# mobeets/classifying-vae-lstm

Hardware: AMD Instinct MI355X
Metric: piano-roll timesteps/sec (train) (higher is better)
Workload: dtype f32; 1 GPU; cfg3: cl_vrnn batch 256/GPU x seq_len 128, latent 2, 10 classes, 88-dim piano-roll, Adam-WN, hipGraph=True; global_batch=256, seq_len=128, parallelism=dp1

## Files before the change

### classifying-vae-lstm_amd/_lib.py

```python
import ctypes as C
import os

_HERE = os.path.dirname(os.path.abspath(__file__))
LIB_PATH = os.environ.get("CLV_LIB") or os.path.join(_HERE, "libclvae_hip.so")

ABI_VERSION = 600
ACT_NONE, ACT_RELU, ACT_SIGMOID, ACT_MASKPOS = 0, 1, 2, 3
GATE_HARD_SIGMOID, GATE_SIGMOID = 0, 1

_f = C.c_float
_i = C.c_int
_p = C.c_void_p
_sz = C.c_size_t
_i64 = C.c_int64
_u64 = C.c_uint64
_u32 = C.c_uint32
_d = C.c_double


class VaeStepOpts(C.Structure):
    _fields_ = [("draw", _i), ("stream_w", _u32), ("stream_z", _u32), ("step", _u32),
                ("noise_seed", _u64), ("first_w", _u64), ("first_z", _u64),
                ("step_dev", _p), ("loss_means", _p), ("bump_iterations", _p), ("bf16", _i)]



class NoiseDraw(C.Structure):
    _fields_ = [("seed", _u64), ("first", _u64), ("stream", _u32), ("step", _u32), ("step_dev", _p)]


class PairPackSrc(C.Structure):
    _fields_ = [("H", _i), ("L", _i), ("U_enc", _p), ("U_dec", _p), ("Kz", _p), ("Wz", _p), ("pack", _p)]


class AdamKnownSums(C.Structure):
    _fields_ = [("tensor", _i), ("use", _i), ("gdot", _p), ("vnorm2", _p)]


class BatchCursor(C.Structure):
    _fields_ = [("step_dev", _p), ("step0", C.c_int32), ("period", C.c_int32), ("stride", _i64), ("offset", _i64)]


class LabelStage(C.Structure):
    _fields_ = [("cur", _p), ("hist", _p),
                ("cur_stride", _i64), ("cur_offset", _i64), ("hist_stride", _i64), ("hist_offset", _i64), ("row0", _i64),
                ("cur_table", _p), ("hist_table", _p), ("idx", _p),
                ("cursor", BatchCursor),
                ("X", _p), ("Xh", _p), ("hist_chunk", C.c_int32), ("hist_ld", _i64),
                ("w_src", _p), ("w_out", _p), ("X8", _p), ("Xh8", _p)]


class FrameProj(C.Structure):
    _fields_ = [("T", C.c_int32), ("N", C.c_int32), ("ldo", C.c_int32), ("K_cur", _p), ("out_cur", _p), ("K_hist", _p), ("out_hist", _p)]


class WgradProblem(C.Structure):
    _fields_ = [("K", C.c_int32), ("N", C.c_int32),
                ("X", _p), ("ldx", C.c_int32), ("nx", C.c_int32), ("x_exact_bf16", C.c_int32),
                ("H", _p), ("ldh", C.c_int32), ("nh", C.c_int32), ("h_shift", C.c_int32), ("h_zero_period", C.c_int32),
                ("Z", _p), ("ldz", C.c_int32), ("nz", C.c_int32),
                ("dz", _p), ("lddz", C.c_int32),
                ("dKx", _p), ("ld_kx", C.c_int32),
                ("dU", _p), ("ld_u", C.c_int32),
                ("dKz", _p), ("ld_kz", C.c_int32),
                ("beta", C.c_float),
                ("ws", _p), ("ws_bytes", C.c_size_t)]


class ParamDesc(C.Structure):
    _fields_ = [("offset", C.c_int64), ("rows", C.c_int32), ("cols", C.c_int32),
                ("col_offset", C.c_int64), ("is_matrix", C.c_int32), ("pad_", C.c_int32)]


class GemmProb(C.Structure):
    _fields_ = [("A", C.c_void_p), ("lda", C.c_int32), ("M", C.c_int32), ("C", C.c_void_p), ("ldc", C.c_int32),
                ("a_shift", C.c_int32), ("a_zero_period", C.c_int32), ("ones", C.c_int32)]


class ReduceJob(C.Structure):
    _fields_ = [("opaque", C.c_ubyte * 160)]


class SkinnyProduct(C.Structure):
    _fields_ = [("A", C.c_void_p), ("lda", C.c_int), ("rows", C.c_int), ("B", C.c_void_p), ("ldb", C.c_int),
                ("N", C.c_int), ("K", C.c_int), ("C", C.c_void_p), ("ldc", C.c_int), ("bias_row", C.c_void_p)]


class LabelBwdRider(C.Structure):
    _fields_ = [("D", C.c_int), ("C", C.c_int), ("Kenc_w", C.c_void_p), ("Kdec_w", C.c_void_p), ("wargs", C.c_void_p),
                ("eps", C.c_void_p), ("onehot", C.c_void_p), ("W", C.c_void_p), ("hW", C.c_void_p), ("Ka", C.c_void_p),
                ("prior_logvar", C.c_float), ("class_weight", C.c_float), ("w_kl_weight", C.c_float), ("inv_b", C.c_float),
                ("dwargs", C.c_void_p), ("dhW", C.c_void_p), ("dKa", C.c_void_p), ("dba", C.c_void_p),
                ("ws", C.c_void_p), ("ws_bytes", C.c_size_t), ("job", C.c_void_p)]


class ProfRecord(C.Structure):
    _fields_ = [("name", C.c_char * 48), ("launches", C.c_int32), ("total_ms", C.c_float)]


def _args(kind, names):
    return [kind] * len(names.split())


_VRNN_GENERATE = _args(_i, "N S nsteps D H L C gate_act z_prior") + [_u64] + _args(_p, "x_seed w")
_VAE_GENERATE = _args(_i, "N nsteps D H L C use_x_prev z_prior") + [_u64] + _args(_p, "x_seed w")
_VARY = _args(_i, "N T D H L C gate_act|use_x_prev hist_source") + [_u64] + _args(_p, "sources x0 w_enc w_dec")
_DECODE = _args(_i, "N T D H L C gate_act|use_x_prev") + [_u64] + _args(_p, "z_in x0 history w_dec noise_rows")
_VRNN_ENC, _VRNN_DEC = _args(_p, "Kx_enc Kw_enc b_enc U_enc Wz bz"), _args(_p, "Kx_dec Kz Kw_dec b_dec U_dec Wo bo")
_VAE_ENC, _VAE_DEC = _args(_p, "Kh bh Kz bz"), _args(_p, "Kd bd Ko bo")
_TEMPER = [_p, _f, _f]
_OUT, _OUT_Z = _args(_p, "Xs xhat stream"), _args(_p, "Xs xhat zout stream")
_RESUME = [_u32] + _args(_p, "state_in state_out")

SIGNATURES = {
    "clv_version": (_i, []),
    "clv_device_count": (_i, []),
    "clv_error_string": (C.c_char_p, [_i]),
    "clv_gemm_auto_split": (_i, [_i, _i, _i]),
    "clv_gemm_workspace_bytes": (_sz, [_i, _i, _i]),
    "clv_gemm_f32": (_i, [_i, _i, _i, _i, _i, _f, _p, _i, _p, _i, _f, _p, _i, _p, _i, _p, _i, _p, _sz, _p, _p]),
    "clv_gemm_grouped_tn": (_i, [_p, _i, _i, _i, _p, _i, _f, _i, _p, _sz, _p, _p]),
    "clv_splitk_reduce_multi": (_i, [_p, _i, _p, _p, _p, _i, _p, _p, _i, _p]),
    "clv_splitk_reduce_multi_outer_supported": (_i, [_i, _i, _i, _i, _i]),
    "clv_splitk_reduce_multi_outer": (_i, [_p, _i, _p, _p, _p, _i, _p, _p, _i,
                                           _i, _i, _i, _p, _i, _i, _p, _i, _p, _i, _p, _p, _i, _p, _p, _p]),
    "clv_lstm_wgrad_supported": (_i, [_i, _i, _i, _i, _i]),
    "clv_lstm_wgrad_workspace_bytes": (_sz, [_i, _i, _i, _i, _i, _i]),
    "clv_lstm_wgrad_pair_supported": (_i, [_p, _p]),
    "clv_lstm_wgrad_pair_workspace_bytes": (_sz, [_i, _i, _i, _i, _i, _i]),
    "clv_lstm_wgrad_pair": (_i, [_p, _p, _i, _p, _p, _p]),
    "clv_lstm_wgrad": (_i, [_i, _i, _p, _i, _i, _i, _p, _i, _i, _i, _i, _p, _i, _i, _p, _i, _p, _i, _p, _i, _p, _i, _f,
                               _i, _p, _sz, _p, _p]),
    "clv_gemm_grouped_tn_small2": (_i, [_p, _i, _p, _p, _i, _p, _i, _i, _i, _p]),
    "clv_gemm_grouped_auto_split": (_i, [_p, _i, _i, _i]),
    "clv_gemm_grouped_workspace_bytes": (_sz, [_p, _i, _i, _i]),
    "clv_colsum_workspace_bytes": (_sz, [_i, _i]),
    "clv_colsum_f32": (_i, [_i, _i, _p, _i, _f, _p, _p, _sz, _p]),
    "clv_lstm_seq_fwd": (_i, [_i, _i, _i, _i, _p, _p, _p, _p, _p, _p, _p, _p, _p, _p, _p]),
    "clv_lstm_seq_bwd_z": (_i, [_i, _i, _i, _i, _p, _p, _p, _p, _p, _p, _p, _i, _p, _i, _p]),
    "clv_lstm_seq_bwd": (_i, [_i, _i, _i, _i, _p, _p, _p, _p, _p, _p, _p]),
    "clv_lstm_mx_supported": (_i, [_i, _i, _i, _i]),
    "clv_lstm_mx_fwd": (_i, [_i, _i, _i, _i, _p, _i, _i, _i, _p, _p, _i, _i, _p, _p, _p, _p, _p, _p, _p]),
    "clv_lstm_mx_bwd": (_i, [_i, _i, _i, _p, _p, _p, _p, _p, _p, _i, _p, _i, _p]),
    "clv_lstm_pair_supported": (_i, [_i, _i]),
    "clv_lstm_pair_pack_floats": (_sz, []),
    "clv_lstm_pair_pack": (_i, [_i, _i, _p, _p, _p, _p, _p, _p]),
    "clv_lstm_pair_fwd": (_i, [_i, _i, _i, _i, _i, _p, _p, _p, _i, _p, _p, _p, _p, _p, _p, _p, _p, _p, _p, _i, _p, _p, _p, _p, _p,
                               _p, _p]),
    "clv_lstm_pair_bwd": (_i, [_i, _i, _i, _i, _i, _f] + [_p] * 12 + [_p, _p, _p, _p, _sz, _p, _p, _p]),
    "clv_lstm_pair_bwd_workspace_bytes": (_sz, [_i, _i, _i]),
    "clv_sparse_proj_supported": (_i, [_i, _i]),
    "clv_sparse_proj_lds_bytes": (_sz, [_i, _i]),
    "clv_sparse_proj": (_i, [_i, _i, _i, _p, _i, _i, _p, _p, _i, _p]),
    "clv_sparse_proj2": (_i, [_i, _i, _i, _i, _i, _p, _i, _p, _p, _i, _p, _i, _p, _p, _p]),
    "clv_sparse_dense_supported": (_i, [_i]),
    "clv_sparse_dense": (_i, [_i, _i, _i, _p, _i, _p, _p, _i, _p, _i, _p]),
    "clv_sparse_outer": (_i, [_i, _i, _i, _p, _i, _p, _i, _p, _i, _p, _p, _i, _p, _p, _p]),
    "clv_dense_outer_bf16_supported": (_i, [_i, _i, _i, _i, _i]),
    "clv_dense_outer_bf16": (_i, [_i, _i, _i, _p, _i, _i, _p, _i, _p, _i, _p, _p, _i, _p, _p, _p]),
    "clv_gemm_bce_f32": (_i, [_i, _i, _i, _p, _i, _p, _i, _p, _p, _i, _f, _p, _p, _i, _p, _p]),
    "clv_out_head_train_supported": (_i, [_i, _i]),
    "clv_out_head_train_workspace_bytes": (_sz, [_i]),
    "clv_out_head_train": (_i, [_i, _i, _i, _p, _p, _p, _p, _i, _i, _f, _p, _p, _p, _p, _p, _p, _p, _sz, _p, _p]),
    "clv_latent_head_supported": (_i, [_i, _i]),
    "clv_latent_head_bwd_workspace_bytes": (_sz, [_i, _i]),
    "clv_latent_head_fwd": (_i, [_i, _i, _i, _p, _p, _p, _p, _p, _p, _i, _p, _p, _p]),
    "clv_latent_head_bwd": (_i, [_i, _i, _i, _p, _p, _p, _p, _p, _i, _f, _p, _p, _p, _p, _p, _sz, _p, _p]),
    "clv_vrnn_generate_supported": (_i, [_i, _i, _i, _i]),
    "clv_vrnn_generate": (_i, _VRNN_GENERATE + _VRNN_ENC + _VRNN_DEC + _OUT),
    "clv_vae_generate_supported": (_i, [_i, _i, _i, _i]),
    "clv_vae_generate": (_i, _VAE_GENERATE + _VAE_ENC + _VAE_DEC + _OUT),
    "clv_vrnn_generate_clamped": (_i, _VRNN_GENERATE + _VRNN_ENC + _VRNN_DEC + _args(_p, "clamp") + _OUT),
    "clv_vae_generate_clamped": (_i, _VAE_GENERATE + _VAE_ENC + _VAE_DEC + _args(_p, "clamp") + _OUT),
    "clv_vrnn_generate_tempered": (_i, _VRNN_GENERATE + _VRNN_ENC + _VRNN_DEC + _TEMPER + _OUT),
    "clv_vae_generate_tempered": (_i, _VAE_GENERATE + _VAE_ENC + _VAE_DEC + _TEMPER + _OUT),
    "clv_vrnn_vary": (_i, _VARY + _VRNN_ENC + _VRNN_DEC + _TEMPER + _OUT),
    "clv_vae_vary": (_i, _VARY + _VAE_ENC + _VAE_DEC + _TEMPER + _OUT),
    "clv_take_frame": (_i, [_i64, _i, _i, _p, _p, _p, _p]),
    "clv_vrnn_vary_latents": (_i, _VARY + _VRNN_ENC + _VRNN_DEC + _TEMPER + _OUT_Z),
    "clv_vae_vary_latents": (_i, _VARY + _VAE_ENC + _VAE_DEC + _TEMPER + _OUT_Z),
    "clv_vrnn_decode": (_i, _DECODE + _VRNN_DEC + _TEMPER[:2] + _OUT),
    "clv_vae_decode": (_i, _DECODE + _VAE_DEC + _TEMPER[:2] + _OUT),
    "clv_vrnn_generate_resume": (_i, _VRNN_GENERATE + _VRNN_ENC + _VRNN_DEC + _TEMPER + _RESUME + _OUT),
    "clv_vae_generate_resume": (_i, _VAE_GENERATE[:-2] + _args(_p, "w") + _VAE_ENC + _VAE_DEC + _TEMPER + _RESUME + _OUT),
    "clv_lerp_rows": (_i, [_i64, _i64] + [_p] * 7),
    "clv_sigmoid_temper": (_i, [_i64, _p, _f, _p]),
    "clv_scale_temper": (_i, [_i64, _p, _f, _p]),
    "clv_label_fwd": (_i, [_i, _i, _p, _p, _i, _p, _p, _f, _p, _p, _p]),
    "clv_label_bwd": (_i, [_i, _i, _p, _p, _i, _p, _p, _p, _p, _f, _f, _f, _f, _p, _p, _i, _p]),
    "clv_vae_fused_supported": (_i, [_i, _i, _i, _i, _i]),
    "clv_vae_fused_workspace_bytes": (_sz, [_i, _i, _i, _i, _i, _i, _i]),
    "clv_vae_fused_step": (_i, [_i, _i, _i, _i, _i, _i, _i, _p, _p, _p, _p, _p, _p, _p, _p, _p, C.c_long, _f, _f, _f, _f, _i,
                                _p, _p, _sz, _p, _p, _p, _p, _p, _p, _p, _p, _p]),
    "clv_vrnn_label_fwd": (_i, [_i, _i, _i, _i, _p, _p, _p, _p, _p, _f, _p, _p, _p, _p, _p, _p, _p, _p, _p, _p]),
    "clv_vrnn_label_fwd_x": (_i, [_i, _i, _i, _i, _p, _i, _i, _p, _p, _p, _p, _p, _p, _p, _p, _f, _p, _p, _p, _p, _p, _p, _p, _p, _p,
                                  _p, _p, _p, _p]),
    "clv_vrnn_label_fwd_x_proj_supported": (_i, [_i, _i, _i, _i, _i]),
    "clv_vrnn_label_fwd_parts": (_i, [_i, _i, _i, _i, _p, _i, _p, _p, _p, _p, _p, _p, _f, _p, _p, _p, _p, _p, _p, _p, _p, _p,
                                  _p, _p, _p]),
    "clv_dense_window_fwd_bf16_supported": (_i, [_i, _i, _i, _i, _i]),
    "clv_dense_window_fwd_bf16_splits": (_i, [_i, _i]),
    "clv_dense_window_fwd_bf16_workspace_bytes": (_sz, [_i, _i, _i]),
    "clv_dense_window_fwd_bf16": (_i, [_i, _i, _i, _p, _i, _i, _p, _i, _p, _sz, _p]),
    "clv_vrnn_label_bwd_workspace_bytes": (_sz, [_i, _i, _i]),
    "clv_vrnn_label_bwd": (_i, [_i, _i, _i, _i, _p, _p, _p, _p, _p, _p, _p, _p, _p, _p, _f, _f, _f, _f, _p, _p, _p, _p, _p, _sz,
                                   _p, _p]),
    "clv_gauss_fwd": (_i, [_i, _i, _p, _p, _p, _i, _p, _p]),
    "clv_gauss_bwd": (_i, [_i, _i, _p, _p, _p, _i, _f, _p, _p]),
    "clv_bernoulli_nll": (_i, [_i, _i, _p, _p, _i, _f, _p, _p, _p]),
    "clv_loss_sums": (_i, [_p, _i, _i, _p, _i, _i, _p, _i, _i, _p, _i, _i, _p, _i, _i, _p, _p]),
    "clv_sum_strided": (_i, [_i, _p, _i, _f, _p, _p]),
    "clv_act_grad": (_i, [_i64, _i, _p, _p, _p, _p]),
    "clv_axpy": (_i, [_i64, _f, _p, _p, _p]),
    "clv_gather_rows": (_i, [_i64, _i64, _p, _p, _p, _i64, _i64, _p]),
    "clv_adam_wn_plan_bytes": (_sz, [_p, _i]),
    "clv_adam_wn_plan_build": (_i, [_p, _i, _p]),
    "clv_adam_wn_workspace_bytes": (_sz, [_p, _i]),
    "clv_adam_wn_step": (_i, [_p, _i, _p, _p, _p, _p, _p, _p, _p, _p, _p, _i, _f, _f, _f, _f, _i, _p, _p, _sz, _p]),
    "clv_philox_normal2": (_i, [_p, _i64, _u32, _u64, _p, _i64, _u32, _u64, _u64, _u32, _p, _p]),
    "clv_gather_rows_multi": (_i, [_i64, _p, _i64, _i, _p, _p, _p, _p, _p, _p, _p, _p, _p, _p, _p, _p]),
    "clv_philox_normal": (_i, [_p, _i64, _u64, _u32, _p, _u32, _u64, _p]),
    "clv_philox_uniform": (_i, [_p, _i64, _u64, _u32, _p, _u32, _u64, _p]),
    "clv_i32_add": (_i, [_p, C.c_int32, _p]),
    "clv_iw_accumulate": (_i, [_i, _i, _i, _i, _p, _p, _p, _p, _p, _f, _i, _p, _p, _p]),
    "clv_iw_finish": (_i, [_i, _i, _i, _p, _p, _p, _p, _p]),
    "clv_smc_sample": (_i, [_i, _i, _i, _i, _i, _p, _p, _p, _p, _p, _p, _p, _p]),
    "clv_smc_resample": (_i, [_i, _i, _i, _i, _u64, _i64, _d] + [_p] * 9),
    "clv_smc_gather": (_i, [_i, _i, _i, _i, _i, _p, _p, _p, _p, _p, _p, _p]),
    "clv_smc_backtrack": (_i, [_i, _i, _i, _i, _i, _u64, _i64, _i, _p, _p, _p, _p, _p, _p]),
    "clv_smc_init_w": (_i, [_i, _i, _i, _i, _u64, _i64, _p, _p, _p, _p, _p]),
    "clv_smc_w_posterior": (_i, [_i, _i, _i, _i, _i, _p, _p, _p, _p, _p]),
    "clv_smc_take_w": (_i, [_i, _i, _i, _i, _p, _p, _p, _p]),
    "clv_key_track_windows": (_i, [_i, _i, _i, _i, _i, _i, _i, _p, _p, _p, _p, _p, _p, _p, _u64, _i64, _p, _p, _p]),
    "clv_key_track_smooth": (_i, [_i, _i, _p, _p, _p, _p, _d, _p, _p, _p, _p, _p]),
    "clv_bernoulli_sample": (_i, [_i64, _p, _p, _p, _p]),
    "clv_bernoulli_sample_clamped": (_i, [_i64, _i, _i, _i, _p, _p, _p, _p, _p, _p]),
    "clv_dropout_rows": (_i, [_i, _i, _i, _p, _i, _p, _i, _f, _f, _p, _i, _p]),
    "clv_graph_begin_capture": (_i, [_p]),
    "clv_graph_end_capture": (_i, [_p, C.POINTER(_p)]),
    "clv_graph_launch": (_i, [_p, _p]),
    "clv_graph_destroy": (_i, [_p]),
    "clv_prof_enable": (_i, [_i]),
    "clv_prof_collect": (_i, [C.POINTER(ProfRecord), _i]),
    "clv_prof_empty_scope": (_i, [_p]),
}

_lib = None


class ClvError(RuntimeError):
    pass


def lib():
    global _lib
    if _lib is None:
        if not os.path.exists(LIB_PATH):
            raise ClvError(
                "libclvae_hip.so is not built (%s). Run `python __graft_entry__.py` or "
                "`make -C classifying-vae-lstm_amd/csrc`. There is no CPU fallback." % LIB_PATH)
        import torch
        h = C.CDLL(LIB_PATH)
        for name, (res, args) in SIGNATURES.items():
            fn = getattr(h, name)
            fn.restype = res
            fn.argtypes = args
        if h.clv_version() != ABI_VERSION:
            raise ClvError("libclvae_hip.so has ABI version %d, this binding was written for %d (include/clvae.h: "
                           "CLV_ABI_VERSION); rebuild with `make -C classifying-vae-lstm_amd/csrc`"
                           % (h.clv_version(), ABI_VERSION))
        _lib = h
    return _lib


def require_gpu():
    n = lib().clv_device_count()
    if n <= 0:
        raise ClvError("no gfx950 (MI355X) device visible; the HIP path has no CPU fallback")
    return n


def check(code, what=""):
    if code != 0:
        msg = lib().clv_error_string(int(code))
        raise ClvError("%s failed: %s (%d)" % (what or "clv call", msg.decode() if msg else "?", code))
```

### classifying-vae-lstm_amd/csrc/optim.hip

```cpp
#include "common.h"

namespace clv {

#ifndef CLV_ADAM_UNIT_ROWS
#define CLV_ADAM_UNIT_ROWS 16
#endif
constexpr int UNIT_ROWS = CLV_ADAM_UNIT_ROWS;
constexpr int SM_RL = 16, SM_RMAX = 9;
constexpr int SM_ROWS = SM_RL * SM_RMAX;

struct AdamUnit {
  int64_t offset;
  int64_t col_offset;
  int32_t row0, nrows, cols;
  int32_t is_matrix;
  int32_t part_off;
  int32_t small;
};
struct AdamCol {
  int64_t col_global;
  int32_t part_base;
  int32_t nunits;
  int32_t cols;
  int32_t col_local;
};
struct AdamHyper {
  float lr, b1, b2, eps;
  int weightnorm;
  int step_t;
  const int32_t* iterations;
};

__device__ __forceinline__ float adam_lr_t(const AdamHyper& h) {
  const int t = h.iterations ? (*h.iterations + (h.step_t == CLV_STEP_ADVANCED ? 0 : 1)) : h.step_t;
  return h.lr * sqrtf(1.f - powf(h.b2, (float)t)) / (1.f - powf(h.b1, (float)t));
}

__global__ __launch_bounds__(256) void wn_stats_kernel(const AdamUnit* units, const float* params, const float* grads,
                                                       const float* s, float* partA, float* partB) {
  const AdamUnit un = units[blockIdx.x];
  if (!un.is_matrix || un.small) return;
  __shared__ float ra[4][64], rbb[4][64];
  const int cx = threadIdx.x & 63, ry = threadIdx.x >> 6;
  for (int c0 = 0; c0 < un.cols; c0 += 64) {
    const int col = c0 + cx;
    float a = 0.f, b = 0.f;
    if (col < un.cols) {
      const float inv_s = 1.f / s[un.col_offset + col];
      float pv[UNIT_ROWS / 4], gv[UNIT_ROWS / 4];
#pragma unroll
      for (int i = 0; i < UNIT_ROWS / 4; ++i) {
        const int r = ry + 4 * i;
        const size_t o = un.offset + (size_t)(un.row0 + min(r, un.nrows - 1)) * un.cols + col;
        pv[i] = params[o]; gv[i] = grads[o];
      }
#pragma unroll
      for (int i = 0; i < UNIT_ROWS / 4; ++i) {
        if (ry + 4 * i < un.nrows) {
          const float V = pv[i] * inv_s;
          a += V * V;
          b += gv[i] * V;
        }
      }
    }
    ra[ry][cx] = a; rbb[ry][cx] = b;
    __syncthreads();
    if (ry == 0 && col < un.cols) {
      partA[un.part_off + col] = ra[0][cx] + ra[1][cx] + ra[2][cx] + ra[3][cx];
      partB[un.part_off + col] = rbb[0][cx] + rbb[1][cx] + rbb[2][cx] + rbb[3][cx];
    }
    __syncthreads();
  }
}

constexpr int CL = 64;
constexpr int CPB = 4;
__device__ __forceinline__ void col_partial_sums(const AdamCol& c, const float* pa, const float* pb, int zy,
                                                 float& a, float& b) {
  const float* qa = pa + c.part_base + c.col_local;
  const float* qb = pb ? pb + c.part_base + c.col_local : nullptr;
  float a0 = 0.f, a1 = 0.f, a2 = 0.f, a3 = 0.f, b0 = 0.f, b1 = 0.f, b2 = 0.f, b3 = 0.f;
  int k = zy;
  for (; k + 11 * CL < c.nunits; k += 12 * CL) {
    float ta[12], tb[12];
#pragma unroll
    for (int i = 0; i < 12; ++i) {
      ta[i] = qa[(size_t)(k + i * CL) * c.cols];
      tb[i] = qb ? qb[(size_t)(k + i * CL) * c.cols] : 0.f;
    }
#pragma unroll
    for (int i = 0; i < 12; i += 4) {
      a0 += ta[i]; a1 += ta[i + 1]; a2 += ta[i + 2]; a3 += ta[i + 3];
      b0 += tb[i]; b1 += tb[i + 1]; b2 += tb[i + 2]; b3 += tb[i + 3];
    }
  }
  {
    float ta[12], tb[12];
    const int last = c.nunits - 1;
#pragma unroll
    for (int i = 0; i < 12; ++i) {
      const int kk = min(k + i * CL, last);
      ta[i] = qa[(size_t)kk * c.cols];
      tb[i] = qb ? qb[(size_t)kk * c.cols] : 0.f;
    }
#pragma unroll
    for (int i = 0; i < 12; i += 4) {
      a0 += (k + i * CL < c.nunits) ? ta[i] : 0.f;             a1 += (k + (i + 1) * CL < c.nunits) ? ta[i + 1] : 0.f;
      a2 += (k + (i + 2) * CL < c.nunits) ? ta[i + 2] : 0.f;   a3 += (k + (i + 3) * CL < c.nunits) ? ta[i + 3] : 0.f;
      b0 += (k + i * CL < c.nunits) ? tb[i] : 0.f;             b1 += (k + (i + 1) * CL < c.nunits) ? tb[i + 1] : 0.f;
      b2 += (k + (i + 2) * CL < c.nunits) ? tb[i + 2] : 0.f;   b3 += (k + (i + 3) * CL < c.nunits) ? tb[i + 3] : 0.f;
    }
  }
  a0 += a2; a1 += a3; b0 += b2; b1 += b3;
  a = a0 + a1; b = b0 + b1;
}
__device__ __forceinline__ float lanes16_sum(float (*red)[CPB], int zy, int cx, float v) {
  red[zy][cx] = v;
  __syncthreads();
  float t = 0.f;
  if (zy == 0)
#pragma unroll
    for (int i = 0; i < CL; ++i) t += red[i][cx];
  __syncthreads();
  return t;
}

__global__ __launch_bounds__(256) void wn_cols_kernel(int n_cols, const AdamCol* cols, const float* partA,
                                                      const float* partB, const float* s, float* mg, float* vg,
                                                      float* colscal, AdamHyper h) {
  __shared__ float red[CL][CPB];
  const int cx = threadIdx.x & (CPB - 1), zy = threadIdx.x / CPB;
  const int j = blockIdx.x * CPB + cx;
  float a = 0.f, b = 0.f;
  AdamCol c;
  bool skip = true;
  if (j < n_cols) { c = cols[j]; skip = c.nunits < 0; if (!skip) col_partial_sums(c, partA, partB, zy, a, b); }
  a = lanes16_sum(red, zy, cx, a);
  b = lanes16_sum(red, zy, cx, b);
  if (zy != 0 || j >= n_cols || skip) return;
  const float lr_t = adam_lr_t(h);
  const float sc = s[c.col_global];
  const float Vn = sqrtf(a);
  const float gparam = sc * Vn;
  const float grad_g = b / Vn;
  const float mgn = h.b1 * mg[c.col_global] + (1.f - h.b1) * grad_g;
  const float vgn = h.b2 * vg[c.col_global] + (1.f - h.b2) * grad_g * grad_g;
  mg[c.col_global] = mgn;
  vg[c.col_global] = vgn;
  colscal[4 * j + 0] = 1.f / sc;
  colscal[4 * j + 1] = grad_g / Vn;
  colscal[4 * j + 2] = sc;
  colscal[4 * j + 3] = gparam - lr_t * mgn / (sqrtf(vgn) + h.eps);
}

__global__ __launch_bounds__(256) void wn_cols2_kernel(int n_cols, const AdamCol* cols, const float* partC, float* s,
                                                       float* colscal, int32_t* iterations, float* vn2) {
  __shared__ float red[CL][CPB];
  if (blockIdx.x == 0 && threadIdx.x == 0 && iterations) *iterations += 1;
  const int cx = threadIdx.x & (CPB - 1), zy = threadIdx.x / CPB;
  const int j = blockIdx.x * CPB + cx;
  float a = 0.f, b = 0.f;
  AdamCol c;
  bool skip = true;
  if (j < n_cols) { c = cols[j]; skip = c.nunits < 0; if (!skip) col_partial_sums(c, partC, nullptr, zy, a, b); }
  a = lanes16_sum(red, zy, cx, a);
  if (zy != 0 || j >= n_cols || skip) return;
  const float snew = colscal[4 * j + 3] / sqrtf(a);
  colscal[4 * j + 0] = snew;
  s[c.col_global] = snew;
  if (vn2) vn2[c.col_global] = a;
}

__device__ __forceinline__ void wn_update_body(const AdamUnit& un, int unit_idx, float* params, const float* grads,
                                               float* m, float* v, const float* colscal,
                                               const int32_t* colidx0, float* partC, const AdamHyper& h) {
  if (un.small && h.weightnorm == CLV_OPT_ADAM_WN) return;
  const float lr_t = adam_lr_t(h);
  if (h.weightnorm == CLV_OPT_RMSPROP) {
    const int n = un.nrows * un.cols;
    const size_t base = un.offset + (size_t)un.row0 * un.cols;
    for (int i = threadIdx.x; i < n; i += 256) {
      const float g = grads[base + i];
      const float an = h.b2 * v[base + i] + (1.f - h.b2) * g * g;
      v[base + i] = an;
      params[base + i] -= h.lr * g / (sqrtf(an) + h.eps);
    }
    return;
  }
  if (!un.is_matrix || !h.weightnorm) {
    const int n = un.nrows * un.cols;
// ... 16 lines not shown
    if (col < un.cols) {
      const float inv_s = colscal[4 * (cbase + col) + 0], gov = colscal[4 * (cbase + col) + 1];
      const float sc = colscal[4 * (cbase + col) + 2];
      float pv[UNIT_ROWS / 4], gv[UNIT_ROWS / 4], mv[UNIT_ROWS / 4], vv[UNIT_ROWS / 4];
#pragma unroll
      for (int i = 0; i < UNIT_ROWS / 4; ++i) {
        const int r = ry + 4 * i;
        const size_t o = un.offset + (size_t)(un.row0 + min(r, un.nrows - 1)) * un.cols + col;
        pv[i] = params[o]; gv[i] = grads[o]; mv[i] = m[o]; vv[i] = v[o];
      }
#pragma unroll
      for (int i = 0; i < UNIT_ROWS / 4; ++i) {
        const int r = ry + 4 * i;
        if (r < un.nrows) {
          const size_t o = un.offset + (size_t)(un.row0 + r) * un.cols + col;
          const float V = pv[i] * inv_s;
          const float gV = sc * (gv[i] - gov * V);
          const float mn = h.b1 * mv[i] + (1.f - h.b1) * gV;
          const float vn = h.b2 * vv[i] + (1.f - h.b2) * gV * gV;
          m[o] = mn; v[o] = vn;
          const float Vp = V - lr_t * mn / (sqrtf(vn) + h.eps);
          params[o] = Vp;
          acc += Vp * Vp;
        }
      }
    }
    rc[ry][cx] = acc;
    __syncthreads();
    if (ry == 0 && col < un.cols) partC[un.part_off + col] = rc[0][cx] + rc[1][cx] + rc[2][cx] + rc[3][cx];
    __syncthreads();
  }
}

__global__ __launch_bounds__(256) void wn_rescale_kernel(const AdamUnit* units, float* params, const float* colscal,
                                                         const int32_t* colidx0) {
  const AdamUnit un = units[blockIdx.x];
  if (!un.is_matrix || un.small) return;
  const int cx = threadIdx.x & 63, ry = threadIdx.x >> 6;
  const int cbase = colidx0[blockIdx.x];
  for (int c0 = 0; c0 < un.cols; c0 += 64) {
    const int col = c0 + cx;
    if (col >= un.cols) continue;
    const float snew = colscal[4 * (cbase + col) + 0];
    for (int r = ry; r < un.nrows; r += 4) {
      const size_t o = un.offset + (size_t)(un.row0 + r) * un.cols + col;
      params[o] *= snew;
    }
  }
}

struct SmallItem {
  int64_t offset;
  int64_t col_offset;
  int32_t rows, cols, col0, is_matrix;
};
__device__ __forceinline__ void wn_small_body(const SmallItem& it, float* params, const float* grads, float* m,
                                              float* v, float* mg, float* vg, float* s, const AdamHyper& h) {
  const float lr_t = adam_lr_t(h);
  if (!it.is_matrix) {
    const int n = it.rows * it.cols;
    for (int i = threadIdx.x; i < n; i += 256) {
      const size_t o = it.offset + i;
      const float g = grads[o];
      const float mn = h.b1 * m[o] + (1.f - h.b1) * g;
      const float vn = h.b2 * v[o] + (1.f - h.b2) * g * g;
      m[o] = mn; v[o] = vn;
      params[o] -= lr_t * mn / (sqrtf(vn) + h.eps);
    }
    return;
  }
  __shared__ float red[SM_RL][16], tot[2][16];
  const int cx = threadIdx.x & 15, ry = threadIdx.x >> 4;
  const int col = it.col0 + cx;
  const bool live = col < it.cols;
  const int cc = min(col, it.cols - 1);
  const float sc = s[it.col_offset + cc];
  const float inv_s = 1.f / sc;
  float pv[SM_RMAX], gv[SM_RMAX], mv[SM_RMAX], vv[SM_RMAX];
#pragma unroll
  for (int i = 0; i < SM_RMAX; ++i) {
    const size_t o = it.offset + (size_t)min(ry + SM_RL * i, it.rows - 1) * it.cols + cc;
    pv[i] = params[o]; gv[i] = grads[o]; mv[i] = m[o]; vv[i] = v[o];
  }
  float a = 0.f, b = 0.f;
#pragma unroll
  for (int i = 0; i < SM_RMAX; ++i)
    if (ry + SM_RL * i < it.rows) {
      const float V = pv[i] * inv_s;
      pv[i] = V;
      a += V * V;
      b += gv[i] * V;
    }
  auto colsum = [&](float x, int slot) {
    red[ry][cx] = x;
    __syncthreads();
    if (ry == 0) {
      float t = 0.f;
#pragma unroll
      for (int i = 0; i < SM_RL; ++i) t += red[i][cx];
      tot[slot][cx] = t;
    }
    __syncthreads();
    return tot[slot][cx];
  };
  a = colsum(a, 0);
  b = colsum(b, 1);
  const float Vn = sqrtf(a);
  const float gparam = sc * Vn;
  const float grad_g = b / Vn;
  const size_t cg = it.col_offset + cc;
  const float mgn = h.b1 * mg[cg] + (1.f - h.b1) * grad_g;
  const float vgn = h.b2 * vg[cg] + (1.f - h.b2) * grad_g * grad_g;
  const float gnew = gparam - lr_t * mgn / (sqrtf(vgn) + h.eps);
  const float gov = grad_g / Vn;
  float c2 = 0.f;
#pragma unroll
  for (int i = 0; i < SM_RMAX; ++i)
    if (ry + SM_RL * i < it.rows) {
      const float gV = sc * (gv[i] - gov * pv[i]);
      const float mn = h.b1 * mv[i] + (1.f - h.b1) * gV;
      const float vn = h.b2 * vv[i] + (1.f - h.b2) * gV * gV;
      mv[i] = mn; vv[i] = vn;
      const float Vp = pv[i] - lr_t * mn / (sqrtf(vn) + h.eps);
      pv[i] = Vp;
      c2 += Vp * Vp;
    }
  c2 = colsum(c2, 0);
  const float snew = gnew / sqrtf(c2);
  if (live) {
#pragma unroll
    for (int i = 0; i < SM_RMAX; ++i)
      if (ry + SM_RL * i < it.rows) {
        const size_t o = it.offset + (size_t)(ry + SM_RL * i) * it.cols + col;
        m[o] = mv[i]; v[o] = vv[i];
        params[o] = snew * pv[i];
      }
    if (ry == 0) { mg[cg] = mgn; vg[cg] = vgn; s[cg] = snew; }
  }
}

__global__ __launch_bounds__(256) void wn_update_kernel(int n_units, const AdamUnit* units, const SmallItem* items,
                                                        float* params, const float* grads, float* m, float* v,
                                                        float* mg, float* vg, float* s, const float* colscal,
                                                        const int32_t* colidx0, float* partC, AdamHyper h) {
  if ((int)blockIdx.x >= n_units) {
    wn_small_body(items[blockIdx.x - n_units], params, grads, m, v, mg, vg, s, h);
    return;
  }
  wn_update_body(units[blockIdx.x], (int)blockIdx.x, params, grads, m, v, colscal, colidx0, partC, h);
}

__global__ void adam_bump_kernel(int32_t* iterations) { *iterations += 1; }

#ifndef CLV_FAST_ROWS
#define CLV_FAST_ROWS 64
#endif
constexpr int FAST_ROWS = CLV_FAST_ROWS;
constexpr int FAST_NT = 1024;
struct AdamFast {
  int64_t offset, col_offset;
  int rows, cols, nunits;
  const float* gdot;
  float* vn2;
  float* gnew;
  float* partC;
};

__device__ __forceinline__ void wn_fast_update_body(const AdamFast& f, int unit, float* params, const float* grads, float* m,
                                                    float* v, float* mg, float* vg, const float* s, const AdamHyper& h) {
  __shared__ float cs[3][128];
  __shared__ float2 red[16][64];
  const int tid = threadIdx.x, cx = tid & 63, ry = tid >> 6;
  const float lr_t = adam_lr_t(h);
  for (int c = tid; c < f.cols; c += FAST_NT) {
    const size_t cg = f.col_offset + c;
    const float sc = s[cg], a = f.vn2[cg];
    const float Vn = sqrtf(a), inv_s = 1.f / sc;
    const float grad_g = f.gdot[c] * inv_s / Vn;
    cs[0][c] = inv_s; cs[1][c] = grad_g / Vn; cs[2][c] = sc;
    if (unit == 0) {
      const float mgn = h.b1 * mg[cg] + (1.f - h.b1) * grad_g;
      const float vgn = h.b2 * vg[cg] + (1.f - h.b2) * grad_g * grad_g;
      mg[cg] = mgn; vg[cg] = vgn;
      f.gnew[c] = sc * Vn - lr_t * mgn / (sqrtf(vgn) + h.eps);
    }
  }
  __syncthreads();
  const int row0 = unit * FAST_ROWS, nrows = min(FAST_ROWS, f.rows - row0), n2 = f.cols / 2;
  float2 acc = make_float2(0.f, 0.f);
  if (cx < n2) {
    const float2 inv_s = make_float2(cs[0][2 * cx], cs[0][2 * cx + 1]), gov = make_float2(cs[1][2 * cx], cs[1][2 * cx + 1]);
    const float2 sc = make_float2(cs[2][2 * cx], cs[2][2 * cx + 1]);
    float2 pv[FAST_ROWS / 16], gv[FAST_ROWS / 16], mv[FAST_ROWS / 16], vv[FAST_ROWS / 16];
#pragma unroll
    for (int i = 0; i < FAST_ROWS / 16; ++i) {
      const size_t o = f.offset + (size_t)(row0 + min(ry + 16 * i, nrows - 1)) * f.cols + 2 * cx;
      pv[i] = *reinterpret_cast<const float2*>(params + o); gv[i] = *reinterpret_cast<const float2*>(grads + o);
      mv[i] = *reinterpret_cast<const float2*>(m + o); vv[i] = *reinterpret_cast<const float2*>(v + o);
    }
    auto one = [&](float p, float g, float m0, float v0, float is, float go, float s0, float& mo, float& vo, float& a2) {
      const float V = p * is;
      const float gV = s0 * (g - go * V);
      mo = h.b1 * m0 + (1.f - h.b1) * gV;
      vo = h.b2 * v0 + (1.f - h.b2) * gV * gV;
      const float Vp = V - lr_t * mo / (sqrtf(vo) + h.eps);
      a2 += Vp * Vp;
      return Vp;
    };
#pragma unroll
    for (int i = 0; i < FAST_ROWS / 16; ++i) {
      const int r = ry + 16 * i;
      if (r < nrows) {
        const size_t o = f.offset + (size_t)(row0 + r) * f.cols + 2 * cx;
        float2 mo, vo, po;
        po.x = one(pv[i].x, gv[i].x, mv[i].x, vv[i].x, inv_s.x, gov.x, sc.x, mo.x, vo.x, acc.x);
        po.y = one(pv[i].y, gv[i].y, mv[i].y, vv[i].y, inv_s.y, gov.y, sc.y, mo.y, vo.y, acc.y);
        *reinterpret_cast<float2*>(m + o) = mo;
        *reinterpret_cast<float2*>(v + o) = vo;
        *reinterpret_cast<float2*>(params + o) = po;
      }
    }
  }
  red[ry][cx] = acc;
  __syncthreads();
  if (ry == 0 && cx < n2) {
    float2 t = make_float2(0.f, 0.f);
#pragma unroll
    for (int w = 0; w < 16; ++w) { t.x += red[w][cx].x; t.y += red[w][cx].y; }
    *reinterpret_cast<float2*>(f.partC + (size_t)unit * f.cols + 2 * cx) = t;
  }
}

#ifndef CLV_ADAM_FLAT
#define CLV_ADAM_FLAT 1
#endif
__device__ __forceinline__ void wn_fast_update_body_flat(const AdamFast& f, int unit, float* params, const float* grads, float* m,
                                                         float* v, float* mg, float* vg, const float* s, const AdamHyper& h) {
  __shared__ __attribute__((aligned(16))) float cs[3][128];
  __shared__ __attribute__((aligned(16))) float sq[FAST_ROWS * 128];
  const int tid = threadIdx.x;
  const float lr_t = adam_lr_t(h);
  for (int c = tid; c < f.cols; c += FAST_NT) {
    const size_t cg = f.col_offset + c;
    const float sc = s[cg], a = f.vn2[cg];
    const float Vn = sqrtf(a), inv_s = 1.f / sc;
    const float grad_g = f.gdot[c] * inv_s / Vn;
    cs[0][c] = inv_s; cs[1][c] = grad_g / Vn; cs[2][c] = sc;
    if (unit == 0) {
      const float mgn = h.b1 * mg[cg] + (1.f - h.b1) * grad_g;
      const float vgn = h.b2 * vg[cg] + (1.f - h.b2) * grad_g * grad_g;
      mg[cg] = mgn; vg[cg] = vgn;
      f.gnew[c] = sc * Vn - lr_t * mgn / (sqrtf(vgn) + h.eps);
    }
  }
  const int row0 = unit * FAST_ROWS, nrows = min(FAST_ROWS, f.rows - row0);
  const int n4 = nrows * f.cols / 4;
  const size_t o0 = f.offset + (size_t)row0 * f.cols;
#ifndef CLV_ADAM_FLAT_PT
#define CLV_ADAM_FLAT_PT 2
#endif
  constexpr int PT = CLV_ADAM_FLAT_PT;
  constexpr int NTA = (FAST_ROWS * 128 / 4 + PT - 1) / PT < FAST_NT ? (FAST_ROWS * 128 / 4 + PT - 1) / PT : FAST_NT;
  float4 pv[PT], gv[PT], mv[PT], vv[PT];
#pragma unroll
  for (int k = 0; k < PT; ++k) {
    const size_t o = o0 + 4 * (size_t)min(tid + NTA * k, n4 - 1);
    pv[k] = *reinterpret_cast<const float4*>(params + o); gv[k] = *reinterpret_cast<const float4*>(grads + o);
    mv[k] = *reinterpret_cast<const float4*>(m + o); vv[k] = *reinterpret_cast<const float4*>(v + o);
  }
  __syncthreads();
#pragma unroll
  for (int k = 0; k < PT; ++k) {
    const int i = tid + NTA * k;
    if (tid < NTA && i < n4) {
      const int c0 = (4 * i) % f.cols;
      const float pin[4] = {pv[k].x, pv[k].y, pv[k].z, pv[k].w}, gin[4] = {gv[k].x, gv[k].y, gv[k].z, gv[k].w};
      const float min_[4] = {mv[k].x, mv[k].y, mv[k].z, mv[k].w}, vin[4] = {vv[k].x, vv[k].y, vv[k].z, vv[k].w};
      const float4 c_is = *reinterpret_cast<const float4*>(&cs[0][c0]), c_gg = *reinterpret_cast<const float4*>(&cs[1][c0]),
                   c_sc = *reinterpret_cast<const float4*>(&cs[2][c0]);
      const float is4[4] = {c_is.x, c_is.y, c_is.z, c_is.w}, gg4[4] = {c_gg.x, c_gg.y, c_gg.z, c_gg.w}, sc4[4] = {c_sc.x, c_sc.y, c_sc.z, c_sc.w};
      float po[4], mo[4], vo[4];
#pragma unroll
      for (int c = 0; c < 4; ++c) {
        const float V = pin[c] * is4[c];
        const float gV = sc4[c] * (gin[c] - gg4[c] * V);
        mo[c] = h.b1 * min_[c] + (1.f - h.b1) * gV;
        vo[c] = h.b2 * vin[c] + (1.f - h.b2) * gV * gV;
        po[c] = V - lr_t * mo[c] / (sqrtf(vo[c]) + h.eps);
      }
      const size_t o = o0 + 4 * (size_t)i;
      *reinterpret_cast<float4*>(m + o) = make_float4(mo[0], mo[1], mo[2], mo[3]);
      *reinterpret_cast<float4*>(v + o) = make_float4(vo[0], vo[1], vo[2], vo[3]);
      *reinterpret_cast<float4*>(params + o) = make_float4(po[0], po[1], po[2], po[3]);
      *reinterpret_cast<float4*>(sq + 4 * i) = make_float4(po[0] * po[0], po[1] * po[1], po[2] * po[2], po[3] * po[3]);
    }
  }
  __syncthreads();
  const int cx = tid % f.cols, rl = tid / f.cols;
  float part = 0.f;
  if (rl < 8)
    for (int r = rl; r < nrows; r += 8) part += sq[r * f.cols + cx];
  __syncthreads();
  if (rl < 8) sq[rl * f.cols + cx] = part;
  __syncthreads();
  if (tid < f.cols) {
    float t = 0.f;
#pragma unroll
    for (int w = 0; w < 8; ++w) t += sq[w * f.cols + tid];
    f.partC[(size_t)unit * f.cols + tid] = t;
  }
}

__global__ __launch_bounds__(FAST_NT) void wn_fast_update_kernel(AdamFast f, const SmallItem* items, float* params,
                                                                 const float* grads, float* m, float* v, float* mg, float* vg,
                                                                 float* s, AdamHyper h) {
  if ((int)blockIdx.x >= f.nunits) {
    if (threadIdx.x >= 256) return;
    wn_small_body(items[blockIdx.x - f.nunits], params, grads, m, v, mg, vg, s, h);
    return;
  }
#if CLV_ADAM_FLAT
  if (f.cols % 4 == 0 && f.offset % 4 == 0 && 8 * f.cols <= FAST_NT) {
    wn_fast_update_body_flat(f, (int)blockIdx.x, params, grads, m, v, mg, vg, s, h);
    return;
  }
#endif
  wn_fast_update_body(f, (int)blockIdx.x, params, grads, m, v, mg, vg, s, h);
}

__global__ __launch_bounds__(FAST_NT) void wn_fast_rescale_kernel(AdamFast f, float* params, float* s, int32_t* iterations) {
  __shared__ __attribute__((aligned(16))) float2 red[16][64], snew[64];
  const int tid = threadIdx.x, cx = tid & 63, ry = tid >> 6, unit = blockIdx.x, n2 = f.cols / 2;
  if (unit == 0 && tid == 0 && iterations) *iterations += 1;
#if CLV_ADAM_FLAT
  const bool flat = f.cols % 4 == 0 && f.offset % 4 == 0;
  const int frow0 = unit * FAST_ROWS, fn4 = min(FAST_ROWS, f.rows - frow0) * f.cols / 4;
  float* ftile = params + f.offset + (size_t)frow0 * f.cols;
  float4 fpv[2];
  if (flat) {
#pragma unroll
    for (int k = 0; k < 2; ++k) fpv[k] = *reinterpret_cast<const float4*>(ftile + 4 * (size_t)min(tid + FAST_NT * k, fn4 - 1));
  }
#endif
  float2 a = make_float2(0.f, 0.f);
  if (cx < n2)
    for (int k = ry; k < f.nunits; k += 16) {
      const float2 t = *reinterpret_cast<const float2*>(f.partC + (size_t)k * f.cols + 2 * cx);
      a.x += t.x; a.y += t.y;
    }
  red[ry][cx] = a;
  __syncthreads();
  if (ry == 0 && cx < n2) {
    float2 t = make_float2(0.f, 0.f);
#pragma unroll
    for (int w = 0; w < 16; ++w) { t.x += red[w][cx].x; t.y += red[w][cx].y; }
    const float2 sn = make_float2(f.gnew[2 * cx] / sqrtf(t.x), f.gnew[2 * cx + 1] / sqrtf(t.y));
    snew[cx] = sn;
    if (unit == 0) {
      *reinterpret_cast<float2*>(s + f.col_offset + 2 * cx) = sn;
      *reinterpret_cast<float2*>(f.vn2 + f.col_offset + 2 * cx) = t;
    }
  }
  __syncthreads();
#if CLV_ADAM_FLAT
  if (flat) {
    const float* sf = reinterpret_cast<const float*>(snew);
#pragma unroll
    for (int k = 0; k < 2; ++k) {
      const int i = tid + FAST_NT * k;
      if (i < fn4) {
        const int c0 = (4 * i) % f.cols;
        const float4 sn4 = *reinterpret_cast<const float4*>(sf + c0);
        *reinterpret_cast<float4*>(ftile + 4 * (size_t)i) = make_float4(fpv[k].x * sn4.x, fpv[k].y * sn4.y, fpv[k].z * sn4.z, fpv[k].w * sn4.w);
      }
    }
    return;
  }
#endif
  const int row0 = unit * FAST_ROWS, nrows = min(FAST_ROWS, f.rows - row0);
  if (cx < n2) {
    const float2 sn = snew[cx];
    float2 pv[FAST_ROWS / 16];
#pragma unroll
    for (int i = 0; i < FAST_ROWS / 16; ++i)
      pv[i] = *reinterpret_cast<const float2*>(params + f.offset + (size_t)(row0 + min(ry + 16 * i, nrows - 1)) * f.cols + 2 * cx);
#pragma unroll
    for (int i = 0; i < FAST_ROWS / 16; ++i)
      if (ry + 16 * i < nrows)
        *reinterpret_cast<float2*>(params + f.offset + (size_t)(row0 + ry + 16 * i) * f.cols + 2 * cx) =
            make_float2(pv[i].x * sn.x, pv[i].y * sn.y);
  }
}

struct PlanCounts { int n_units, n_cols, n_part, n_small, n_big; };

static bool is_small(const clv_param_desc& t) { return !t.is_matrix || t.rows <= SM_ROWS; }
static PlanCounts plan_counts(const clv_param_desc* t, int n) {
  PlanCounts c{0, 0, 0, 0, 0};
  for (int i = 0; i < n; ++i) {
    const int units = (t[i].rows + UNIT_ROWS - 1) / UNIT_ROWS;
    c.n_units += units;
    if (t[i].is_matrix) { c.n_cols += t[i].cols; c.n_part += units * t[i].cols; }
    if (is_small(t[i])) c.n_small += t[i].is_matrix ? (t[i].cols + 15) / 16 : 1;
    else c.n_big += 1;
  }
  return c;
}

}

using namespace clv;

extern "C" size_t clv_adam_wn_plan_bytes(const clv_param_desc* host_table, int n_tensors) {
  if (!host_table || n_tensors <= 0) return 0;
  PlanCounts c = plan_counts(host_table, n_tensors);
  return align_up(sizeof(AdamUnit) * c.n_units, 16) + align_up(sizeof(AdamCol) * (c.n_cols > 0 ? c.n_cols : 1), 16) +
         align_up(sizeof(int32_t) * c.n_units, 16) + align_up(sizeof(SmallItem) * (c.n_small > 0 ? c.n_small : 1), 16);
}

extern "C" int clv_adam_wn_plan_build(const clv_param_desc* host_table, int n_tensors, void* host_blob) {
  if (!host_table || n_tensors <= 0 || !host_blob) return CLV_EINVAL;
  PlanCounts c = plan_counts(host_table, n_tensors);
  char* p = (char*)host_blob;
  AdamUnit* units = (AdamUnit*)p;
  p += align_up(sizeof(AdamUnit) * c.n_units, 16);
  AdamCol* cols = (AdamCol*)p;
  p += align_up(sizeof(AdamCol) * (c.n_cols > 0 ? c.n_cols : 1), 16);
  int32_t* colidx0 = (int32_t*)p;
  p += align_up(sizeof(int32_t) * c.n_units, 16);
  SmallItem* small = (SmallItem*)p;
  int ui = 0, ci = 0, part = 0, si = 0;
  for (int i = 0; i < n_tensors; ++i) {
    const clv_param_desc& t = host_table[i];
    if (t.rows <= 0 || t.cols <= 0) return CLV_EINVAL;
    if (is_small(t)) {
      if (t.is_matrix)
        for (int c0 = 0; c0 < t.cols; c0 += 16) small[si++] = SmallItem{t.offset, t.col_offset, t.rows, t.cols, c0, 1};
      else small[si++] = SmallItem{t.offset, 0, t.rows, t.cols, 0, 0};
    }
    const int nun = (t.rows + UNIT_ROWS - 1) / UNIT_ROWS;
    const int part_base = part;
    for (int k = 0; k < nun; ++k) {
      AdamUnit& u = units[ui];
      u.offset = t.offset; u.col_offset = t.col_offset;
      u.row0 = k * UNIT_ROWS;
      u.nrows = (t.rows - u.row0) < UNIT_ROWS ? (t.rows - u.row0) : UNIT_ROWS;
      u.cols = t.cols; u.is_matrix = t.is_matrix;
      u.part_off = t.is_matrix ? part : 0;
      u.small = is_small(t) ? 1 : 0;
      colidx0[ui] = t.is_matrix ? ci : 0;
      if (t.is_matrix) part += t.cols;
      ++ui;
    }
    if (t.is_matrix) {
      for (int cidx = 0; cidx < t.cols; ++cidx) {
        AdamCol& c2 = cols[ci + cidx];
        c2.col_global = t.col_offset + cidx;
        c2.part_base = part_base; c2.nunits = is_small(t) ? -1 : nun; c2.cols = t.cols; c2.col_local = cidx;
      }
      ci += t.cols;
    }
  }
  return CLV_OK;
}

extern "C" size_t clv_adam_wn_workspace_bytes(const clv_param_desc* host_table, int n_tensors) {
  if (!host_table || n_tensors <= 0) return 0;
  PlanCounts c = plan_counts(host_table, n_tensors);
  return (size_t)(3 * c.n_part + 4 * c.n_cols + 16) * sizeof(float);
}

extern "C" int clv_adam_wn_step(const clv_param_desc* host_table, int n_tensors, const void* plan_dev,
                                   float* params, const float* grads, float* m, float* v,
                                   float* mg, float* vg, float* s,
                                   int32_t* iterations_dev, int step_t, float lr, float beta1, float beta2, float eps,
                                   int weightnorm, const clv_adam_known_sums* known, void* ws, size_t ws_bytes, void* stream) {
  if (!host_table || n_tensors <= 0 || !plan_dev || !params || !grads || !m || !v) return CLV_EINVAL;
  float* vn2 = known ? known->vnorm2 : nullptr;
  if (weightnorm < 0 || weightnorm > CLV_OPT_RMSPROP) return CLV_EINVAL;
  if (weightnorm == CLV_OPT_ADAM_WN && (!mg || !vg || !s)) return CLV_EINVAL;
  PlanCounts c = plan_counts(host_table, n_tensors);
  if (!ws || ws_bytes < clv_adam_wn_workspace_bytes(host_table, n_tensors)) return CLV_EWORKSPACE;
  hipStream_t st = (hipStream_t)stream;
  const char* p = (const char*)plan_dev;
  const AdamUnit* units = (const AdamUnit*)p;
  p += align_up(sizeof(AdamUnit) * c.n_units, 16);
  const AdamCol* cols = (const AdamCol*)p;
  p += align_up(sizeof(AdamCol) * (c.n_cols > 0 ? c.n_cols : 1), 16);
  const int32_t* colidx0 = (const int32_t*)p;
  p += align_up(sizeof(int32_t) * c.n_units, 16);
  const SmallItem* small = (const SmallItem*)p;
  float* partA = (float*)ws;
  float* partB = partA + c.n_part;
  float* partC = partB + c.n_part;
  float* colscal = partC + c.n_part;
  AdamHyper h{lr, beta1, beta2, eps, weightnorm, step_t, iterations_dev};
  int32_t* bump = (iterations_dev && (step_t == -1 || step_t == CLV_STEP_ADVANCED)) ? nullptr : iterations_dev;
  const bool wn = weightnorm == CLV_OPT_ADAM_WN && c.n_cols > 0;
  const bool fast = known && known->use && wn;
  int nunits = 0;
  if (fast) {
    const int ti = known->tensor;
    if (ti < 0 || ti >= n_tensors || c.n_big != 1 || is_small(host_table[ti]) || !known->gdot || !vn2) return CLV_EINVAL;
    const clv_param_desc& t = host_table[ti];
    if (t.cols > 128 || t.cols % 2 || t.offset % 2 || t.col_offset % 2) return CLV_EINVAL;
    nunits = (t.rows + FAST_ROWS - 1) / FAST_ROWS;
    if ((size_t)nunits * t.cols > (size_t)c.n_part) return CLV_EWORKSPACE;
  }
  ProfScope pr("adam_wn_step", st);
  if (fast) {
    const clv_param_desc& t = host_table[known->tensor];
    AdamFast f{t.offset, t.col_offset, t.rows, t.cols, nunits, known->gdot, vn2, colscal, partC};
    hipLaunchKernelGGL(wn_fast_update_kernel, dim3(nunits + c.n_small), dim3(FAST_NT), 0, st, f, small, params, grads, m, v, mg,
                       vg, s, h);
    hipLaunchKernelGGL(wn_fast_rescale_kernel, dim3(nunits), dim3(FAST_NT), 0, st, f, params, s, bump);
    return launch_status();
  }
  const bool chain = !wn || c.n_big > 0;
  const int n_small = wn ? c.n_small : 0;
  if (wn && chain) {
    hipLaunchKernelGGL(wn_stats_kernel, dim3(c.n_units), dim3(256), 0, st, units, params, grads, s, partA, partB);
    hipLaunchKernelGGL(wn_cols_kernel, dim3((c.n_cols + CPB - 1) / CPB), dim3(256), 0, st, c.n_cols, cols, partA, partB, s,
                       mg, vg, colscal, h);
  }
  {
    const int n_units = chain ? c.n_units : 0;
    if (n_units + n_small > 0)
      hipLaunchKernelGGL(wn_update_kernel, dim3(n_units + n_small), dim3(256), 0, st, n_units, units, small, params, grads, m,
                         v, mg, vg, s, colscal, colidx0, partC, h);
  }
  if (wn && chain) {
    hipLaunchKernelGGL(wn_cols2_kernel, dim3((c.n_cols + CPB - 1) / CPB), dim3(256), 0, st, c.n_cols, cols, partC, s, colscal,
                       bump, vn2);
    hipLaunchKernelGGL(wn_rescale_kernel, dim3(c.n_units), dim3(256), 0, st, units, params, colscal, colidx0);
  } else if (bump) {
    hipLaunchKernelGGL(adam_bump_kernel, dim3(1), dim3(1), 0, st, bump);
  }
  return launch_status();
}
```

### classifying-vae-lstm_amd/csrc/outer_bf16_body.h

```cpp
#pragma once
#include "bf16_images.h"

namespace clv {


typedef float od_f32x4 __attribute__((ext_vector_type(4)));
typedef unsigned od_u32x4 __attribute__((ext_vector_type(4)));

constexpr int OD_KS = 32;
constexpr int OD_P = 192;
constexpr int OD_IMG = OD_KS * OD_P;
constexpr int OD_BUF = 4 * OD_IMG;
constexpr int OD_LDS = 2 * OD_BUF;

struct OuterBf16Args {
  int Bn, nx, N, ldx, ldg, ldo;
  const void* X;
  const float* G;
  float* out;
  float* colsum;
  const float* Hact; const float* hbias; float* gdot; int ldh;
};

typedef __amdgpu_buffer_rsrc_t od_rsrc_t;
constexpr unsigned OD_OOB = 0x80000000u;
__device__ __forceinline__ float od_u2f(unsigned u) { return __builtin_bit_cast(float, u); }
__device__ __forceinline__ float4 od_load4(od_rsrc_t r, unsigned voff) {
  const od_u32x4 x = __builtin_amdgcn_raw_buffer_load_b128(r, (int)voff, 0, 0);
  return make_float4(od_u2f(x[0]), od_u2f(x[1]), od_u2f(x[2]), od_u2f(x[3]));
}
__device__ __forceinline__ float4 od_load_u8x4(od_rsrc_t r, unsigned voff) {
  return make_float4(od_u2f((unsigned)__builtin_amdgcn_raw_buffer_load_b32(r, (int)voff, 0, 0)), 0.f, 0.f, 0.f);
}
__device__ __forceinline__ float4 od_widen(const float4& raw) {
  const float r0 = raw.x;
  const unsigned v = __builtin_bit_cast(unsigned, r0);
  return make_float4((float)(v & 0xffu), (float)((v >> 8) & 0xffu), (float)((v >> 16) & 0xffu), (float)(v >> 24));
}

inline int od_own_launch_waves(int nx) { return (nx + 95) / 96 >= 100 ? 6 : 3; }

template <int OD_NW, bool XU8>
__device__ __forceinline__ void dense_outer_block(const OuterBf16Args& a, char* od_lds, int blk, int vw) {
  constexpr int OD_NT = 64 * OD_NW, OD_JT = 16 * OD_NW;
  const int tid = threadIdx.x, lane = tid & 63;
  const int wave = __builtin_amdgcn_readfirstlane(tid >> 6);
  const int ntile = (a.nx + OD_JT - 1) / OD_JT;
  if (blk >= ntile) {
    float2* red = reinterpret_cast<float2*>(od_lds);
    const int n2 = a.N / 2;
    for (int w = wave; w < vw; w += OD_NW) {
      float2 cs = make_float2(0.f, 0.f), gd = make_float2(0.f, 0.f);
      if (lane < n2) {
        const float2 hb = a.gdot ? make_float2(a.hbias[2 * lane], a.hbias[2 * lane + 1]) : make_float2(0.f, 0.f);
        for (int b0 = w; b0 < a.Bn; b0 += 8 * vw) {
          float2 hv[8], gv[8];
#pragma unroll
          for (int i = 0; i < 8; ++i) {
            const int bb = min(b0 + i * vw, a.Bn - 1);
            gv[i] = *reinterpret_cast<const float2*>(a.G + (size_t)bb * a.ldg + 2 * lane);
            hv[i] = a.gdot ? *reinterpret_cast<const float2*>(a.Hact + (size_t)bb * a.ldh + 2 * lane) : make_float2(0.f, 0.f);
          }
#pragma unroll
          for (int i = 0; i < 8; ++i) {
            const float mk = b0 + i * vw < a.Bn ? 1.f : 0.f;
            cs.x += gv[i].x * mk; cs.y += gv[i].y * mk;
            gd.x = fmaf((hv[i].x - hb.x) * mk, gv[i].x, gd.x);
            gd.y = fmaf((hv[i].y - hb.y) * mk, gv[i].y, gd.y);
          }
        }
      }
      red[w * 64 + lane] = cs;
      red[(vw + w) * 64 + lane] = gd;
    }
    __syncthreads();
    if (wave == 0 && lane < n2) {
      float2 t = make_float2(0.f, 0.f), u = make_float2(0.f, 0.f);
      for (int w = 0; w < vw; ++w) {
        t.x += red[w * 64 + lane].x; t.y += red[w * 64 + lane].y;
        u.x += red[(vw + w) * 64 + lane].x; u.y += red[(vw + w) * 64 + lane].y;
      }
      if (a.colsum) { a.colsum[2 * lane] = t.x; a.colsum[2 * lane + 1] = t.y; }
      if (a.gdot) { a.gdot[2 * lane] = u.x; a.gdot[2 * lane + 1] = u.y; }
    }
    return;
  }

  for (int i = tid; i < OD_LDS / 16; i += OD_NT) reinterpret_cast<float4*>(od_lds)[i] = make_float4(0.f, 0.f, 0.f, 0.f);
  const int j0 = blk * OD_JT;
  const int n4 = a.N / 4;
  constexpr unsigned XE = XU8 ? 1u : 4u;
  const od_rsrc_t r_x = (od_rsrc_t)__builtin_amdgcn_make_buffer_rsrc(const_cast<void*>(a.X), 0, (int)(unsigned)((size_t)a.Bn * a.ldx * XE), 0x00020000);
  const od_rsrc_t r_g = (od_rsrc_t)__builtin_amdgcn_make_buffer_rsrc(const_cast<float*>(a.G), 0, (int)(unsigned)((size_t)a.Bn * a.ldg * 4), 0x00020000);
  constexpr int XC4 = OD_JT / 4;
  constexpr int XS = OD_KS * XC4 / OD_NT, GS = (OD_KS * 24 + OD_NT - 1) / OD_NT;
  static_assert(XS * OD_NT == OD_KS * XC4, "X slots");
  unsigned xg[XS], gg[GS];
  int xl[XS], gl[GS];
  bool gok[GS];
#pragma unroll
  for (int i = 0; i < XS; ++i) {
    const int e = tid + OD_NT * i;
    const int rx = e / XC4, cx = e - XC4 * rx;
    xg[i] = j0 + 4 * cx < a.nx ? XE * (unsigned)(rx * a.ldx + j0 + 4 * cx) : OD_OOB;
    xl[i] = rx * OD_P + 8 * cx;
  }
#pragma unroll
  for (int i = 0; i < GS; ++i) {
    const int e = tid + OD_NT * i;
    gok[i] = e < OD_KS * n4;
    const int eg = gok[i] ? e : 0, rg = eg / n4, cg = eg - n4 * rg;
    gg[i] = gok[i] ? 4u * (unsigned)(rg * a.ldg + 4 * cg) : OD_OOB;
    gl[i] = rg * OD_P + 8 * cg;
  }
  const int nst = (a.Bn + OD_KS - 1) / OD_KS;
  constexpr int DEPTH = 4;
  float4 xr[DEPTH][XS], gr[DEPTH][GS];
  auto load_stage = [&](float4 (&xq)[XS], float4 (&gq)[GS], int s) {
    const unsigned kx = XE * (unsigned)(s * OD_KS * a.ldx), kg = 4u * (unsigned)(s * OD_KS * a.ldg);
#pragma unroll
    for (int i = 0; i < XS; ++i) {
      const unsigned xo = xg[i] == OD_OOB ? OD_OOB : xg[i] + kx;
      xq[i] = XU8 ? od_load_u8x4(r_x, xo) : od_load4(r_x, xo);
    }
#pragma unroll
    for (int i = 0; i < GS; ++i) gq[i] = od_load4(r_g, gg[i] == OD_OOB ? OD_OOB : gg[i] + kg);
  };
  auto store_stage = [&](const float4 (&xq)[XS], const float4 (&gq)[GS], int s) {
    char* buf = od_lds + (s & 1) * OD_BUF;
#pragma unroll
    for (int i = 0; i < XS; ++i) img_put4<1>(buf + xl[i], 0, XU8 ? od_widen(xq[i]) : xq[i]);
#pragma unroll
    for (int i = 0; i < GS; ++i)
      if (gok[i]) img_put4<3>(buf + OD_IMG + gl[i], OD_IMG, gq[i]);
  };
  __syncthreads();
#pragma unroll
  for (int d = 0; d < DEPTH; ++d) load_stage(xr[d], gr[d], d);
  store_stage(xr[0], gr[0], 0);
  load_stage(xr[0], gr[0], DEPTH);
  asm volatile("s_waitcnt lgkmcnt(0)\n\ts_barrier" ::: "memory");

  od_f32x4 acc[6];
#pragma unroll
  for (int n = 0; n < 6; ++n) acc[n] = od_f32x4{0.f, 0.f, 0.f, 0.f};
  const int fo = img_frag_lane_offset(OD_P, lane);
  auto stage = [&](int s, float4 (&xq)[XS], float4 (&gq)[GS]) {
    const char* buf = od_lds + (s & 1) * OD_BUF;
    const img_bf16x8 ax = img_frag(buf, OD_P, 16 * wave, fo);
#pragma unroll
    for (int n = 0; n < 6; ++n) {
      img_bf16x8 b[3];
#pragma unroll
      for (int p = 0; p < 3; ++p) b[p] = img_frag(buf + (1 + p) * OD_IMG, OD_P, 16 * n, fo);
#pragma unroll
      for (int p = 2; p >= 0; --p) acc[n] = __builtin_amdgcn_mfma_f32_16x16x32_bf16(ax, b[p], acc[n], 0, 0, 0);
    }
    store_stage(xq, gq, s + 1);
    load_stage(xq, gq, s + 1 + DEPTH);
    asm volatile("s_waitcnt lgkmcnt(0)\n\ts_barrier" ::: "memory");
  };
  for (int s = 0; s < nst; s += DEPTH) {
    stage(s, xr[1], gr[1]);
    stage(s + 1, xr[2], gr[2]);
    stage(s + 2, xr[3], gr[3]);
    stage(s + 3, xr[0], gr[0]);
  }
#pragma unroll
  for (int n = 0; n < 6; ++n)
#pragma unroll
    for (int r = 0; r < 4; ++r) {
      const int j = j0 + 16 * wave + 4 * (lane >> 4) + r, c = 16 * n + (lane & 15);
      if (j < a.nx && c < a.N) a.out[(size_t)j * a.ldo + c] = acc[n][r];
    }
}

}
```

### classifying-vae-lstm_amd/csrc/tail_launch.hip

```cpp
#include "outer_bf16_body.h"
#include "reduce_body.h"

namespace clv {

constexpr int TL_NW = 4;
static_assert(SR_LDS_FLOATS * 4 <= OD_LDS, "the reduce roles' scratch overlays the product's images");

template <bool XU8>
__global__ __launch_bounds__(64 * TL_NW, XU8 ? 4 : 3) void tail_launch_kernel(ReduceTable t, MeanTerms m, SkinnyRider sr, OuterBf16Args a,
                                                                unsigned n_outer, int vw) {
  extern __shared__ __attribute__((aligned(16))) char tl_lds[];
  if (blockIdx.x < n_outer) { dense_outer_block<TL_NW, XU8>(a, tl_lds, (int)blockIdx.x, vw); return; }
  reduce_launch_block<true>(t, m, sr, blockIdx.x - n_outer, reinterpret_cast<float*>(tl_lds));
}

}

extern "C" int clv_splitk_reduce_multi_outer_supported(int Bn, int nx, int N, int ldx, int ldg) {
  return clv_dense_outer_bf16_supported(Bn, nx, N, ldx, ldg);
}

extern "C" int clv_splitk_reduce_multi_outer(const clv_reduce_job* jobs, int njobs, const float* const* x, const int* n,
                                             const int* stride, int n_terms, float* means_out,
                                             const clv_skinny_product* riders, int n_riders,
                                             int Bn, int nx, int N, const void* X, int x_u8, int ldx, const float* G, int ldg,
                                             float* out, int ldo, float* colsum, const float* Hact, int ldh, const float* hbias,
                                             float* gdot, void* stream) {
  using namespace clv;
  ReduceTable t;
  MeanTerms m;
  SkinnyRider sr;
  unsigned blocks = 0;
  if (int e = reduce_launch_tables(jobs, njobs, x, n, stride, n_terms, means_out, riders, n_riders, t, m, sr, &blocks)) return e;
  const bool product = Bn != 0 || nx != 0 || N != 0 || X || G || out;
  OuterBf16Args a{};
  unsigned n_outer = 0;
  if (product) {
    if (!clv_dense_outer_bf16_supported(Bn, nx, N, ldx, ldg) || !X || !G || !out || ldo < N) return CLV_EINVAL;
    if (((uintptr_t)X) % (x_u8 ? 4 : 16) != 0 || ((uintptr_t)G) % 16 != 0) return CLV_EINVAL;
    if (gdot && (!Hact || !hbias || ldh < N || ldh % 2 != 0 || ((uintptr_t)Hact) % 8 != 0)) return CLV_EINVAL;
    a = OuterBf16Args{Bn, nx, N, ldx, ldg, ldo, X, G, out, colsum, Hact, hbias, gdot, ldh};
    n_outer = (unsigned)((nx + 16 * TL_NW - 1) / (16 * TL_NW)) + ((colsum || gdot) ? 1u : 0u);
  }
  if (blocks + n_outer == 0) return CLV_OK;
  hipStream_t s = (hipStream_t)stream;
  const int lds = product ? OD_LDS : SR_LDS_FLOATS * 4 + reduce_pad_lds();
  ProfScope p("tail_launch", s);
  auto go = [&](auto kern) -> int {
    if (int e = allow_dynamic_lds(reinterpret_cast<const void*>(kern), OD_LDS)) return e;
    hipLaunchKernelGGL(kern, dim3(n_outer + blocks), dim3(64 * TL_NW), lds, s, t, m, sr, a, n_outer, od_own_launch_waves(nx));
    return launch_status();
  };
  return x_u8 ? go(tail_launch_kernel<true>) : go(tail_launch_kernel<false>);
}
```

### classifying-vae-lstm_amd/engine.py

```python
import contextlib
import ctypes as C
import os
import warnings

import numpy as np
import torch

from . import _lib, ops
from .engine_dropout import VrnnDropout
from .engine_generate import VaeGenerate, VrnnGenerate
from .ops import ACT_MASKPOS, ACT_NONE, ACT_RELU, ACT_SIGMOID
from .params import FlatParams, fuse_heads


def vae_param_shapes(cfg):
    D, H, L, Hc, Cn = cfg['D'], cfg['H'], cfg['L'], cfg['Hc'], cfg['C']
    dec_in = Cn + (D if cfg['use_x_prev'] else 0) + L
    head = [('h_w/kernel', (D, Hc)), ('h_w/bias', (Hc,)),
            ('w_mean/kernel', (Hc, Cn - 1)), ('w_mean/bias', (Cn - 1,)),
            ('w_log_var/kernel', (Hc, Cn - 1)), ('w_log_var/bias', (Cn - 1,))]
    if H > 0:
        return head + [('h/kernel', (D + Cn, H)), ('h/bias', (H,)),
                       ('z_mean/kernel', (H, L)), ('z_mean/bias', (L,)),
                       ('z_log_var/kernel', (H, L)), ('z_log_var/bias', (L,)),
                       ('decoder_h/kernel', (dec_in, H)), ('decoder_h/bias', (H,)),
                       ('x_decoded_mean/kernel', (H, D)), ('x_decoded_mean/bias', (D,))]
    return head + [('z_mean/kernel', (D + Cn, L)), ('z_mean/bias', (L,)),
                   ('z_log_var/kernel', (D + Cn, L)), ('z_log_var/bias', (L,)),
                   ('x_decoded_mean/kernel', (dec_in, D)), ('x_decoded_mean/bias', (D,))]


def vrnn_param_shapes(cfg):
    D, H, L, T, Cn = cfg['D'], cfg['H'], cfg['L'], cfg['T'], cfg['C']
    dec_in = (D if cfg['use_x_prev'] else 0) + L + Cn
    return [('hW/kernel', (T * D, D)), ('hW/bias', (D,)),
            ('Wargs/kernel', (D, 2 * (Cn - 1))), ('Wargs/bias', (2 * (Cn - 1),)),
            ('encoder_h/kernel', (D + Cn, 4 * H)), ('encoder_h/recurrent_kernel', (H, 4 * H)),
            ('encoder_h/bias', (4 * H,)),
            ('Z_mean/kernel', (H, L)), ('Z_mean/bias', (L,)),
            ('Z_log_var/kernel', (H, L)), ('Z_log_var/bias', (L,)),
            ('decoder_h/kernel', (dec_in, 4 * H)), ('decoder_h/recurrent_kernel', (H, 4 * H)),
            ('decoder_h/bias', (4 * H,)),
            ('X_decoded_mean/kernel', (H, D)), ('X_decoded_mean/bias', (D,))]


SWITCHES = {
    'fuse_pair':      (None,                   True,  "the separate sequence kernels (csrc/lstm.hip) instead of encoder + latent head + decoder as one launch"),
    'sparse_inputs':  (None,                   True,  "dense GEMM input projections instead of row gathers of the notes that are on"),
    'keep_logits':    (None,                   True,  "the fused output head does not store its logits (what a replayed training step does: 11.5 / 92 MB per step)"),
    'fuse_head':      ('CLV_FUSE_HEAD',        True,  "output head as GEMM + NLL + three backward GEMMs instead of one launch"),
    'bf16_wgrad':     ('CLV_BF16_WGRAD',       True,  "the LSTM kernel gradients on the f32 MFMA GEMM instead of split-bf16 products"),
    'wgrad_pair':     ('CLV_WGRAD_PAIR',       True,  "one kernel-gradient launch per LSTM instead of both in one"),
    'dense_hw_grad':  ('CLV_DENSE_HW_GRAD',    True,  "the hW kernel gradient by walking the notes instead of dense on the bf16 matrix cores"),
    'dense_hw_fwd':   ('CLV_DENSE_HW_FWD',     True,  "the hW forward product by walking the notes at every batch size"),
    'label_in_pair':  ('CLV_LABEL_IN_PAIR',    True,  "the label path's backward as a launch of its own instead of the pair backward kernel's epilogue"),
    'fuse_latent':    ('CLV_FUSE_LATENT',      True,  "the latent head as GEMM + pointwise launches instead of csrc/latent_head.hip"),
    'lstm_mx':        ('CLV_USE_MX',           True,  "large batches on the generic chain instead of csrc/lstm_mx.hip"),
    'frames_u8':      ('CLV_FRAMES_U8',        True,  "the large-batch step widens its byte batch to float (rounds 4-5) instead of reading bytes"),
    'front_fused':    ('CLV_FRONT_FUSED',      True,  "the frame projections as a launch of their own behind the label launch instead of workgroups of it (csrc/label_head.hip: vrnn_front_kernel)"),
    'tail_launch':    ('CLV_TAIL_LAUNCH',      True,  "the hW kernel gradient as a launch of its own in front of grads_tail() instead of workgroups of the reduction launch that ends it (csrc/tail_launch.hip)"),
    'fine_grid':      ('CLV_FINE_GRID',        False, "twice the workgroups, half the rows each, for the LSTM kernel gradients (what tune_dp_schedule may pick next to an all-reduce)"),
    'fuse_notes':     ('CLV_FUSE_NOTES',       False, "input projections gathered inside the pair forward from note lists (+48 us on MI355X: profiles/r03_notes_fusion_ab.txt)"),
}


def switch(cfg, key):
    env, default, _ = SWITCHES[key]
    if key in cfg:
        return bool(cfg[key])
    if env is not None and env in os.environ:
        return os.environ[env] != '0'
    return default


def _f(device, *shape):
    return torch.empty(*shape, dtype=torch.float32, device=device)


class _EngineBase:
    def __init__(self, cfg, batch_size, shapes, device, head_pairs=(), grads_pre=0):
        _lib.require_gpu()
        self.cfg = dict(cfg)
        self.B = int(batch_size)
        self.device = torch.device(device)
        phys, aliases = fuse_heads(shapes, head_pairs)
        self.P = FlatParams(shapes, self.device, phys, aliases, pre=grads_pre)
        self.ws = ops.Workspace(self.device, 8 << 20)
        self.ws2 = ops.Workspace(self.device, 8 << 20)
        self.rq = ops.ReduceQueue(self.device)
        self.side = torch.cuda.Stream(device=self.device) if cfg.get('two_streams', False) else None
        self.scal = torch.zeros(8, dtype=torch.float32, device=self.device)
        self.kl_weight = float(cfg.get('kl_weight', 1.0))
        self.w_kl_weight = float(cfg.get('w_kl_weight', 1.0))
        self.class_weight = float(cfg.get('class_weight', 1.0))

    def losses(self):
        s = self.scal.detach().cpu().numpy().astype(np.float64)
        out = dict(vae=s[0], kl_z=s[1], kl_w=s[2], w_rec=s[3], acc=s[4])
        out['total'] = (out['vae'] + self.w_kl_weight * out['kl_w'] + self.class_weight * out['w_rec']
                        + self.kl_weight * out['kl_z'])
        out['elbo'] = -(out['vae'] + out['kl_z'] + out['kl_w'] + out['w_rec'])
        return out

    def _mean_into(self, n, x, stride, slot):
        ops.sum_strided(n, x, stride, 1.0 / n, self.scal[slot:])

    def _side(self):
        if self.side is None:
            return contextlib.nullcontext()
        self.side.wait_stream(torch.cuda.current_stream())
        return torch.cuda.stream(self.side)

    def _side_more(self):
        return contextlib.nullcontext() if self.side is None else torch.cuda.stream(self.side)

    def _join(self):
        if self.side is not None:
            torch.cuda.current_stream().wait_stream(self.side)


class VaeEngine(VaeGenerate, _EngineBase):

    def __init__(self, cfg, batch_size, device='cuda:0'):
        super().__init__(cfg, batch_size, vae_param_shapes(cfg), device,
                         head_pairs=[('w_mean', 'w_log_var', 'wargs'), ('z_mean', 'z_log_var', 'zargs')])
        B, D, H, L, Hc, Cn = self.B, cfg['D'], cfg['H'], cfg['L'], cfg['Hc'], cfg['C']
        d = self.device
        self.xoff = D if cfg['use_x_prev'] else 0
        L_ = _lib.lib()
        self.fused = H > 0 and bool(cfg.get('fused_step', True)) and bool(L_.clv_vae_fused_supported(D, H, Hc, Cn, L))
        self.stage_spec = None
        names = ['h_w', 'wargs', 'h', 'zargs', 'decoder_h', 'x_decoded_mean']
        self._offs = (C.c_int64 * 12)(*[self.P.offsets.get('%s/%s' % (n, w), 0) for n in names for w in ('kernel', 'bias')])
        ws_bytes = L_.clv_vae_fused_workspace_bytes(B, D, H, Hc, Cn, L, int(cfg['use_x_prev'])) if self.fused else 0
        self._fused_ws = torch.empty(max(ws_bytes, 16), dtype=torch.uint8, device=self.device) if self.fused else None
        self.h_w = _f(d, B, Hc)
        self.wargs = _f(d, B, 2 * (Cn - 1))
        self.w = _f(d, B, Cn)
        self.rowloss = _f(d, B, 3)
        self.h = _f(d, B, max(H, 1))
        self.zargs = _f(d, B, 2 * L)
        self.z = _f(d, B, L)
        self.h_dec = _f(d, B, max(H, 1))
        self.logits = _f(d, B, D)
        self.dlogits = _f(d, B, D)
        self.rownll = _f(d, B)
        self.rowkl = _f(d, B)
        self.d_hdec = _f(d, B, max(H, 1))
        self.dz = _f(d, B, L)
        self.dzargs = _f(d, B, 2 * L)
        self.d_h = _f(d, B, max(H, 1))
        self.dw = _f(d, B, Cn)
        self.dwargs = _f(d, B, 2 * (Cn - 1))
        self.d_hw = _f(d, B, Hc)

    def encode_w(self, x, B=None):
        cfg, P = self.cfg, self.P
        B = self.B if B is None else B
        D, Hc, C1 = cfg['D'], cfg['Hc'], cfg['C'] - 1
        g = ops.gemm
        g(x, P.p('h_w/kernel'), self.h_w, B, Hc, D, bias=P.p('h_w/bias'), act=ACT_RELU, ws=self.ws)
        g(self.h_w, P.p('wargs/kernel'), self.wargs, B, 2 * C1, Hc, bias=P.p('wargs/bias'), ws=self.ws)

    def encode_z(self, x, w, B=None):
        cfg, P = self.cfg, self.P
        B = self.B if B is None else B
        D, H, L, Cn = cfg['D'], cfg['H'], cfg['L'], cfg['C']
        g = ops.gemm
        if H == 0:
            g(x, P.p('zargs/kernel'), self.zargs, B, 2 * L, D, ws=self.ws)
            g(w, P.rows(P.params, 'zargs/kernel', D), self.zargs, B, 2 * L, Cn, beta=1.0, bias=P.p('zargs/bias'), ws=self.ws)
            return
        g(x, P.p('h/kernel'), self.h, B, H, D, ws=self.ws)
        g(w, P.rows(P.params, 'h/kernel', D), self.h, B, H, Cn, beta=1.0, bias=P.p('h/bias'), act=ACT_RELU,
          ws=self.ws)
        g(self.h, P.p('zargs/kernel'), self.zargs, B, 2 * L, H, bias=P.p('zargs/bias'), ws=self.ws)

    def decode(self, w, z, xp, B=None, act=ACT_NONE):
        cfg, P = self.cfg, self.P
        B = self.B if B is None else B
        D, H, L, Cn = cfg['D'], cfg['H'], cfg['L'], cfg['C']
        g = ops.gemm
        if H == 0:
            K = 'x_decoded_mean/kernel'
            g(w, P.p(K), self.logits, B, D, Cn, ws=self.ws)
            if cfg['use_x_prev']:
                g(xp, P.rows(P.params, K, Cn), self.logits, B, D, D, beta=1.0, ws=self.ws)
            g(z, P.rows(P.params, K, Cn + self.xoff), self.logits, B, D, L, beta=1.0, bias=P.p('x_decoded_mean/bias'),
              act=act, ws=self.ws)
            return
        g(w, P.p('decoder_h/kernel'), self.h_dec, B, H, Cn, ws=self.ws)
        if cfg['use_x_prev']:
            g(xp, P.rows(P.params, 'decoder_h/kernel', Cn), self.h_dec, B, H, D, beta=1.0, ws=self.ws)
        g(z, P.rows(P.params, 'decoder_h/kernel', Cn + self.xoff), self.h_dec, B, H, L, beta=1.0,
          bias=P.p('decoder_h/bias'), act=ACT_RELU, ws=self.ws)
        g(self.h_dec, P.p('x_decoded_mean/kernel'), self.logits, B, D, H, bias=P.p('x_decoded_mean/bias'), act=act,
          ws=self.ws)

    def x_hat(self):
        cfg, P, B = self.cfg, self.P, self.B
        if cfg['H'] == 0:
            self.decode(self.w, self.z, self._last_xp, act=ACT_SIGMOID)
            return self.logits
        ops.gemm(self.h_dec, P.p('x_decoded_mean/kernel'), self.dlogits, B, cfg['D'], cfg['H'],
                 bias=P.p('x_decoded_mean/bias'), act=ACT_SIGMOID, ws=self.ws)
        return self.dlogits

    def forward(self, x, xp, eps_w, eps_z, w_true=None):
        cfg, B = self.cfg, self.B
        self._last_xp = xp
        L, Cn = cfg['L'], cfg['C']
        C1 = Cn - 1
        self.encode_w(x)
        ops.label_fwd(B, Cn, self.wargs, self.wargs[:, C1:], 2 * C1, eps_w, w_true, cfg['w_log_var_prior'],
                      self.w, self.rowloss)
        self.encode_z(x, self.w)
        ops.gauss_fwd(B, L, self.zargs, eps_z, self.z, L, self.rowkl)
        self.decode(self.w, self.z, xp)

    def _fused_step(self, x, xp, w_true, eps_w, eps_z, need_grads, target=None, noise=None, bump=False):
        cfg, P, B = self.cfg, self.P, self.B
        p_ = ops._ptr
        opts = _lib.VaeStepOpts()
        opts.loss_means = p_(self.scal)
        opts.bf16 = int(bool(cfg.get('bf16', False)))
        if noise is not None:
            (opts.noise_seed, opts.stream_w, opts.stream_z, opts.first_w, opts.first_z, opts.step), step_dev = noise[:6], noise[6]
            opts.draw, opts.step_dev = 1, p_(step_dev)
        if bump and need_grads:
            opts.bump_iterations = p_(P.iterations)
        tail = (p_(eps_w), p_(eps_z), p_(P.params), self._offs, P.n, float(cfg['w_log_var_prior']), self.class_weight,
                self.kl_weight, self.w_kl_weight, int(need_grads), p_(P.grads), p_(self._fused_ws), self._fused_ws.numel(),
                p_(self.logits), p_(self.w), p_(self.wargs), p_(self.zargs), p_(self.rownll), p_(self.rowkl),
                p_(self.rowloss), C.byref(opts), ops._stream())
        stage, self.stage_spec = self.stage_spec, None
        staged = stage is not None and target is None
        _lib.check(_lib.lib().clv_vae_fused_step(
            B, cfg['D'], cfg['H'], cfg['Hc'], cfg['C'], cfg['L'], int(cfg['use_x_prev']), p_(x), p_(xp), p_(target), p_(w_true),
            C.byref(stage) if staged else None, *tail), "clv_vae_fused_step")

    def can_stage_in_label(self):
        return bool(self.fused)

    def folds_step(self, w_true):
        return bool(self.fused and w_true is not None)

    def loss_and_grads(self, x, xp, w_true, eps_w, eps_z, need_grads=True, target=None, noise=None, bump=False):
        cfg, P, B = self.cfg, self.P, self.B
        D, H, L, Hc, Cn = cfg['D'], cfg['H'], cfg['L'], cfg['Hc'], cfg['C']
        C1 = Cn - 1
        inv = 1.0 / B
        if self.fused and w_true is not None:
            return self._fused_step(x, xp, w_true, eps_w, eps_z, need_grads, target, noise, bump)
        if noise is not None:
            ops.philox_normal2(eps_w, B * C1, noise[1], noise[3], eps_z, B * L, noise[2], noise[4], noise[0], noise[5],
                               step_dev=noise[6])
        self.forward(x, xp, eps_w, eps_z, w_true)
        ops.bernoulli_nll(B, D, self.logits, x if target is None else target, D, inv, self.rownll,
                          self.dlogits if need_grads else None)
        ops.loss_sums([(self.rownll, B, 1), (self.rowkl, B, 1), (self.rowloss, B, 3), (self.rowloss[:, 1:], B, 3),
                       (self.rowloss[:, 2:], B, 3)], self.scal)
        if not need_grads:
            return
        g, ws, xo = ops.gemm, self.ws, self.xoff
        if H == 0:
            return self._grads_without_hidden_layers(x, xp, w_true, eps_w, eps_z, inv)
        g(self.h_dec, self.dlogits, P.g('x_decoded_mean/kernel'), H, D, B, ta=True, ws=ws)
        ops.colsum(self.dlogits, B, D, P.g('x_decoded_mean/bias'), ws)
        g(self.dlogits, P.p('x_decoded_mean/kernel'), self.d_hdec, B, H, D, tb=True, act=ACT_MASKPOS, aux=self.h_dec,
          ws=ws)
        g(self.w, self.d_hdec, P.g('decoder_h/kernel'), Cn, H, B, ta=True, ws=ws)
        if cfg['use_x_prev']:
            g(xp, self.d_hdec, P.rows(P.grads, 'decoder_h/kernel', Cn), D, H, B, ta=True, ws=ws)
        g(self.z, self.d_hdec, P.rows(P.grads, 'decoder_h/kernel', Cn + xo), L, H, B, ta=True, ws=ws)
        ops.colsum(self.d_hdec, B, H, P.g('decoder_h/bias'), ws)
        g(self.d_hdec, P.p('decoder_h/kernel'), self.dw, B, Cn, H, tb=True, ws=ws)
        g(self.d_hdec, P.rows(P.params, 'decoder_h/kernel', Cn + xo), self.dz, B, L, H, tb=True, ws=ws)
        ops.gauss_bwd(B, L, self.zargs, eps_z, self.dz, L, self.kl_weight * inv, self.dzargs)
        g(self.h, self.dzargs, P.g('zargs/kernel'), H, 2 * L, B, ta=True, ws=ws)
        ops.colsum(self.dzargs, B, 2 * L, P.g('zargs/bias'), ws)
        g(self.dzargs, P.p('zargs/kernel'), self.d_h, B, H, 2 * L, tb=True, act=ACT_MASKPOS, aux=self.h, ws=ws)
        g(x, self.d_h, P.g('h/kernel'), D, H, B, ta=True, ws=ws)
        g(self.w, self.d_h, P.rows(P.grads, 'h/kernel', D), Cn, H, B, ta=True, ws=ws)
        ops.colsum(self.d_h, B, H, P.g('h/bias'), ws)
        g(self.d_h, P.rows(P.params, 'h/kernel', D), self.dw, B, Cn, H, tb=True, beta=1.0, ws=ws)
        self._label_head_grads(x, w_true, eps_w, inv)


    def _label_head_grads(self, x, w_true, eps_w, inv):
        cfg, P, B = self.cfg, self.P, self.B
        D, Hc, Cn = cfg['D'], cfg['Hc'], cfg['C']
        C1, g, ws = Cn - 1, ops.gemm, self.ws
        ops.label_bwd(B, Cn, self.wargs, self.wargs[:, C1:], 2 * C1, eps_w, w_true, self.w, self.dw,
                      cfg['w_log_var_prior'], self.class_weight, self.w_kl_weight, inv,
                      self.dwargs, self.dwargs[:, C1:], 2 * C1)
        g(self.h_w, self.dwargs, P.g('wargs/kernel'), Hc, 2 * C1, B, ta=True, ws=ws)
        ops.colsum(self.dwargs, B, 2 * C1, P.g('wargs/bias'), ws)
        g(self.dwargs, P.p('wargs/kernel'), self.d_hw, B, Hc, 2 * C1, tb=True, act=ACT_MASKPOS, aux=self.h_w, ws=ws)
        g(x, self.d_hw, P.g('h_w/kernel'), D, Hc, B, ta=True, ws=ws)
        ops.colsum(self.d_hw, B, Hc, P.g('h_w/bias'), ws)

    def _grads_without_hidden_layers(self, x, xp, w_true, eps_w, eps_z, inv):
        cfg, P, B = self.cfg, self.P, self.B
        D, L, Cn = cfg['D'], cfg['L'], cfg['C']
        g, ws, xo, K = ops.gemm, self.ws, self.xoff, 'x_decoded_mean/kernel'
        g(self.w, self.dlogits, P.g(K), Cn, D, B, ta=True, ws=ws)
        if cfg['use_x_prev']:
            g(xp, self.dlogits, P.rows(P.grads, K, Cn), D, D, B, ta=True, ws=ws)
        g(self.z, self.dlogits, P.rows(P.grads, K, Cn + xo), L, D, B, ta=True, ws=ws)
        ops.colsum(self.dlogits, B, D, P.g('x_decoded_mean/bias'), ws)
        g(self.dlogits, P.p(K), self.dw, B, Cn, D, tb=True, ws=ws)
        g(self.dlogits, P.rows(P.params, K, Cn + xo), self.dz, B, L, D, tb=True, ws=ws)
        ops.gauss_bwd(B, L, self.zargs, eps_z, self.dz, L, self.kl_weight * inv, self.dzargs)
        g(x, self.dzargs, P.g('zargs/kernel'), D, 2 * L, B, ta=True, ws=ws)
        g(self.w, self.dzargs, P.rows(P.grads, 'zargs/kernel', D), Cn, 2 * L, B, ta=True, ws=ws)
        ops.colsum(self.dzargs, B, 2 * L, P.g('zargs/bias'), ws)
        g(self.dzargs, P.rows(P.params, 'zargs/kernel', D), self.dw, B, Cn, 2 * L, tb=True, beta=1.0, ws=ws)
        self._label_head_grads(x, w_true, eps_w, inv)


class VrnnEngine(VrnnDropout, VrnnGenerate, _EngineBase):

    def __init__(self, cfg, batch_size, device='cuda:0'):
        super().__init__(cfg, batch_size, vrnn_param_shapes(cfg), device,
                         head_pairs=[('Z_mean', 'Z_log_var', 'Zargs')], grads_pre=cfg['D'])
        B, D, H, L, T, Cn = self.B, cfg['D'], cfg['H'], cfg['L'], cfg['T'], cfg['C']
        d = self.device
        BT = B * T
        if H != 88:
            warnings.warn("cl_vrnn with %d LSTM units runs on the generic kernels (csrc/lstm_any.hip, GEMM heads): several times "
                          "slower per step than the default 88 units, which the fused kernels are laid out for" % H, stacklevel=2)
        self.gate_act = _lib.GATE_HARD_SIGMOID if cfg.get('gate_act', 'hard_sigmoid') == 'hard_sigmoid' \
            else _lib.GATE_SIGMOID
        self.off = D if cfg['use_x_prev'] else 0
        self.dropout = float(cfg.get('dropout', 0.0) or 0.0)
        if not 0.0 <= self.dropout < 1.0:
            raise ValueError("dropout must be in [0, 1)")
        self._train_pass = False
        sw = lambda key: switch(cfg, key)
        self.fuse_pair = sw('fuse_pair') and ops.lstm_pair_supported(L, H) and not self.dropout
        self.fine_grid = sw('fine_grid')
        self.pair_pack = _f(d, ops.lstm_pair_pack_floats()) if self.fuse_pair else None
        self.sparse_inputs = sw('sparse_inputs') and ops.sparse_proj_supported(D, 4 * H)
        self.fuse_head = sw('fuse_head') and ops.out_head_train_supported(H, D)
        self._head_done = False
        self.keep_logits = sw('keep_logits')
        self.bf16_wgrad = sw('bf16_wgrad')
        self.frames_exact_bf16 = bool(cfg.get('frames_exact_bf16', False))
        self.wgrad_pair = sw('wgrad_pair')
        self.dense_hw_grad = sw('dense_hw_grad')
        self.dense_hw_fwd = sw('dense_hw_fwd') and B >= int(os.environ.get('CLV_DENSE_HW_FWD_ROWS', '512'))
        self.ws_hw = None
        self.stage_spec = None
        self._f8 = None
        self.ws_b = None
        self.label_in_pair = sw('label_in_pair') and self.fuse_pair
        self.fuse_latent = sw('fuse_latent') and ops.latent_head_supported(H, L)
        self.use_mx = sw('lstm_mx') and not self.fuse_pair and not self.dropout and self.sparse_inputs \
            and ops.lstm_mx_supported(B, D, L, H)
        self.frames_u8 = sw('frames_u8')
        self.front_fused = sw('front_fused')
        self.tail_launch = sw('tail_launch')
        self.halves_adjacent = False
        self._hw_outer = None
        self.fuse_notes = sw('fuse_notes') and self.fuse_pair and self.sparse_inputs and D == ops.NOTE_NONE
        self.notes_valid = False
        if self.fuse_notes:
            self.notes_enc = torch.full((BT, ops.NOTE_ROW), ops.NOTE_NONE, dtype=torch.uint8, device=d)
            self.notes_dec = torch.full((BT, ops.NOTE_ROW), ops.NOTE_NONE, dtype=torch.uint8, device=d)
        self.hW = _f(d, B, D)
        self.wargs = _f(d, B, 2 * (Cn - 1))
        self.W = _f(d, B, Cn)
        self.rowloss = _f(d, B, 3)
        self.wk_enc = _f(d, B, 4 * H)
        self.wk_dec = _f(d, B, 4 * H)
        self.gates_enc = _f(d, BT, 4 * H)
        self.gates_dec = _f(d, BT, 4 * H)
        aux2 = self.fuse_pair or self.use_mx
        self.hs_enc, self.cs_enc = _f(d, BT, H), _f(d, BT, 2 * H if aux2 else H)
        self.hs_dec, self.cs_dec = _f(d, BT, H), _f(d, BT, 2 * H if aux2 else H)
        self.zargs = _f(d, BT, 2 * L)
        self.xz_ld = (self.off + L + 3) // 4 * 4
        self.XZ = torch.zeros(BT, self.xz_ld, dtype=torch.float32, device=d)
        self.Z = self.XZ[:, self.off:self.off + L]
        self.rowkl = _f(d, BT)
        self.klterm = _f(d, BT, L)
        self.logits = _f(d, BT, D)
        self.dlogits = _f(d, BT, D)
        self.rownll = _f(d, BT)
        self.dhs = _f(d, BT, H)
        self.dzsum_enc, self.dzsum_dec = _f(d, B, 4 * H), _f(d, B, 4 * H)
        self.dZ = _f(d, BT, L)
        self.dzargs = _f(d, BT, 2 * L)
        self.dW = _f(d, B, Cn)
        self.dwargs = _f(d, B, 2 * (Cn - 1))
        self.dhW = _f(d, B, D)
        self.gdot = self.P.grads_pre[:D] if (self.P.grads_pre.numel() >= D and self.P.offsets['hW/kernel'] == 0) else _f(d, D)
        self.gdot_fresh = False
        if self.dropout:
            in_e, in_d = D + Cn, self.off + L + Cn
            self.u_enc, self.u_dec = _f(d, B, 4, in_e), _f(d, B, 4, in_d)
            self._masks_given = False
            self.xm_e = _f(d, 4, BT, D)
            self.xm_d = torch.zeros(4, BT, self.xz_ld, dtype=torch.float32, device=d)
            self.wm_e, self.wm_d = _f(d, 4, B, Cn), _f(d, 4, B, Cn)
            self.dxg, self.dwg = _f(d, BT, self.xz_ld), _f(d, B, Cn)

    def folds_noise(self):
        return bool((self.fuse_pair or (self.use_mx and self.fuse_latent)) and self.sparse_inputs and self.cfg['D'] % 2 == 0)

    def frames_u8_route(self):
        cfg, B = self.cfg, self.B
        D, H, L, T = cfg['D'], cfg['H'], cfg['L'], cfg['T']
        if not (self.frames_u8 and self.fuse_head and self.bf16_wgrad and self.dense_hw_grad and D % 4 == 0 and self.sparse_inputs
                and ops.dense_outer_bf16_supported(B, T * D, D, T * D, D) and ops.sparse_dense_supported(D)
                and ops.lstm_wgrad_supported(4 * H, D, H, 0, 2) and (not self.off or ops.lstm_wgrad_supported(4 * H, D, H, L, 2))):
            return None
        if self.use_mx:
            return 'gather' if (self.dense_hw_fwd and ops.dense_window_fwd_bf16_supported(B, T * D, D, T * D, D)) else None
        if self.fuse_pair and self.can_stage_in_label():
            return 'label'
        return None

    def frames_u8_supported(self):
        return self.frames_u8_route() is not None

    def forward(self, X, Xp, eps_W, eps_Z, w_true=None, keep_gates=True, nll=None, target=None, noise=None, frames8=None):
        if frames8 is not None and (target is not None or not self.frames_exact_bf16 or not self.frames_u8_supported()):
            raise ValueError("frames8 needs the large-batch path (frames_u8_supported()), frames_exact_bf16 and the input frames as "
                             "the target")
        self._f8 = frames8
        target = X if target is None else target
        cfg, P, B = self.cfg, self.P, self.B
        self._nll_done = False
        self._noise = None
        if noise is not None:
            if self.folds_noise():
                seed, sw, sz, fw, fz, step, step_dev = noise
                self._noise = (ops.noise_draw(seed, sw, fw, step, step_dev), ops.noise_draw(seed, sz, fz, step, step_dev))
            else:
                ops.philox_normal2(eps_W, B * (cfg['C'] - 1), noise[1], noise[3], eps_Z, B * cfg['T'] * cfg['L'], noise[2],
                                   noise[4], noise[0], noise[5], step_dev=noise[6])
        D, H, L, T, Cn = cfg['D'], cfg['H'], cfg['L'], cfg['T'], cfg['C']
        C1, BT, G4 = Cn - 1, B * T, 4 * H
        g, ws = ops.gemm, self.ws
        if cfg['use_x_prev'] and frames8 is None and Xp.data_ptr() != self.XZ.data_ptr():
            self.XZ.view(B, T, self.xz_ld)[:, :, :D].copy_(Xp.view(B, T, D))
        if self.fuse_pair:
            return self._forward_pair(X, eps_W, eps_Z, w_true, nll, target)
        if self.use_mx:
            return self._forward_mx(X, eps_W, eps_Z, w_true, nll, target)
        if self.dropout and self._train_pass:
            if noise is not None:
                row0 = int(noise[3]) // max(cfg['C'] - 1, 1)
                for u, sid in ((self.u_enc, 2), (self.u_dec, 3)):
                    per_row = u.shape[1] * u.shape[2]
                    ops.philox_uniform(u, B * per_row, noise[0], noise[5], sid, row0 * per_row, step_dev=noise[6])
                self._masks_given = True
            elif not self._masks_given:
                raise RuntimeError("training pass with dropout=%g and neither noise=... nor set_dropout_uniforms(): the masks "
                                   "would come from uninitialised memory" % self.dropout)
            return self._forward_dropout(X, eps_W, eps_Z, w_true, nll, target)
        if self.sparse_inputs:
            ops.sparse_proj(BT, D, G4, X, D, P.p('encoder_h/kernel'), self.gates_enc)
        else:
            with self._side():
                g(X, P.p('encoder_h/kernel'), self.gates_enc, BT, G4, D, ws=self.ws2)
        off = self.off
        self._label_forward(X, eps_W, w_true)
        self._join()
        ops.lstm_seq_fwd(B, T, self.gates_enc, self.wk_enc, P.p('encoder_h/recurrent_kernel'), self.hs_enc,
                         self.cs_enc, self.gates_enc, gate_act=self.gate_act, H=H)
        if self.fuse_latent:
            ops.latent_head_fwd(BT, H, L, self.hs_enc, P.p('Zargs/kernel'), P.p('Zargs/bias'), eps_Z, self.zargs, self.Z,
                                self.xz_ld, self.rowkl)
        else:
            g(self.hs_enc, P.p('Zargs/kernel'), self.zargs, BT, 2 * L, H, bias=P.p('Zargs/bias'), ws=ws)
            ops.gauss_fwd(BT, L, self.zargs, eps_Z, self.Z, self.xz_ld, self.rowkl)
        self._join()
        g(self.XZ, P.p('decoder_h/kernel'), self.gates_dec, BT, G4, off + L, lda=self.xz_ld, ws=ws)
        ops.lstm_seq_fwd(B, T, self.gates_dec, self.wk_dec, P.p('decoder_h/recurrent_kernel'), self.hs_dec,
                         self.cs_dec, self.gates_dec, gate_act=self.gate_act, H=H)
        self._output_head(target, nll)

    def _forward_mx(self, X, eps_W, eps_Z, w_true, nll, target):
        cfg, P, B = self.cfg, self.P, self.B
        D, H, L, T = cfg['D'], cfg['H'], cfg['L'], cfg['T']
        BT, off = B * T, self.off
        f8 = self._f8
        if f8 is not None:
            X = f8[0]
        self._label_forward(X, eps_W, w_true)
        ops.lstm_mx_fwd(B, T, X, D, D, P.p('encoder_h/kernel'), None, 0, 0, None, self.wk_enc,
                        P.p('encoder_h/recurrent_kernel'), self.hs_enc, self.gates_enc, self.cs_enc, gate_act=self.gate_act)
        if self.fuse_latent:
            nz = getattr(self, '_noise', None)
            ops.latent_head_fwd(BT, H, L, self.hs_enc, P.p('Zargs/kernel'), P.p('Zargs/bias'), eps_Z, self.zargs, self.Z,
                                self.xz_ld, self.rowkl, noise=nz[1] if nz else None)
        else:
            ops.gemm(self.hs_enc, P.p('Zargs/kernel'), self.zargs, BT, 2 * L, H, bias=P.p('Zargs/bias'), ws=self.ws)
            ops.gauss_fwd(BT, L, self.zargs, eps_Z, self.Z, self.xz_ld, self.rowkl)
        hist, hist_ld = (f8[1], D) if (f8 is not None and off) else (self.XZ if off else None, self.xz_ld)
        ops.lstm_mx_fwd(B, T, hist, hist_ld, off, P.p('decoder_h/kernel') if off else None,
                        self.Z, self.xz_ld, L, P.rows(P.params, 'decoder_h/kernel', off), self.wk_dec,
                        P.p('decoder_h/recurrent_kernel'), self.hs_dec, self.gates_dec, self.cs_dec, gate_act=self.gate_act)
        self._output_head(X if f8 is not None else target, nll)

    def _dense_hw_fwd_now(self):
        cfg = self.cfg
        return self.dense_hw_fwd and self.frames_exact_bf16 and \
            ops.dense_window_fwd_bf16_supported(self.B, cfg['T'] * cfg['D'], cfg['D'], cfg['T'] * cfg['D'], cfg['D'])

    def can_stage_in_label(self):
        return self.fuse_pair and self.sparse_inputs and self.cfg['D'] % 2 == 0 and not self.fuse_notes and \
            not (self.dense_hw_fwd and ops.dense_window_fwd_bf16_supported(self.B, self.cfg['T'] * self.cfg['D'], self.cfg['D'],
                                                                         self.cfg['T'] * self.cfg['D'], self.cfg['D']))

# ... 32 lines not shown
            else:
                ops.gemm_bce(self.hs_dec, P.p('X_decoded_mean/kernel'), P.p('X_decoded_mean/bias'), X, scale, self.logits,
                             self.dlogits if need_grads else None, self.rownll, BT, D, H)
            self._nll_done = True
        else:
            ops.gemm(self.hs_dec, P.p('X_decoded_mean/kernel'), self.logits, BT, D, H, bias=P.p('X_decoded_mean/bias'),
                     ws=self.ws)

    def _forward_pair(self, X, eps_W, eps_Z, w_true, nll=None, target=None):
        cfg, P, B = self.cfg, self.P, self.B
        D, H, L, T, Cn = cfg['D'], cfg['H'], cfg['L'], cfg['T'], cfg['C']
        BT, G4, off = B * T, 4 * H, self.off
        g, ws = ops.gemm, self.ws
        pack = (L, P.p('encoder_h/recurrent_kernel'), P.p('decoder_h/recurrent_kernel'),
                P.rows(P.params, 'decoder_h/kernel', off), P.p('Zargs/kernel'), self.pair_pack)
        pack_in_label = self.sparse_inputs and D % 2 == 0
        if not pack_in_label:
            ops.lstm_pair_pack(*pack)
        stage = self.stage_spec if pack_in_label else None
        self.stage_spec = None
        f8 = self._f8
        if f8 is not None and stage is None:
            raise ValueError("frames8 on the pair path: the byte batch is what the label launch's own stage leaves (ops.label_stage)")
        proj = None
        if stage is not None and f8 is not None and self.front_fused and self.sparse_inputs and not self.fuse_notes and \
                ops.vrnn_label_fwd_x_proj_supported(B, D, T * D, T, G4):
            proj = (T, G4, P.p('encoder_h/kernel'), self.gates_enc, P.p('decoder_h/kernel') if off else None,
                    self.gates_dec if off else None)
        if stage is not None:
            self._label_forward(X, eps_W, w_true, pack=pack, stage=stage, proj=proj)
        notes = None
        if proj is not None:
            pass
        elif self.fuse_notes and self.notes_valid:
            notes = (self.notes_enc, P.p('encoder_h/kernel'), self.notes_dec if off else None,
                     P.p('decoder_h/kernel') if off else None)
        elif self.sparse_inputs:
            cur, hist, hist_ld = (X, self.XZ, self.xz_ld) if f8 is None else (f8[0], f8[1], D)
            if off:
                ops.sparse_proj2(BT, G4, (D, cur, D, P.p('encoder_h/kernel'), self.gates_enc),
                                 (off, hist, hist_ld, P.p('decoder_h/kernel'), self.gates_dec))
            else:
                ops.sparse_proj(BT, D, G4, cur, D, P.p('encoder_h/kernel'), self.gates_enc)
        else:
            g(X, P.p('encoder_h/kernel'), self.gates_enc, BT, G4, D, ws=ws)
            if off:
                g(self.XZ, P.p('decoder_h/kernel'), self.gates_dec, BT, G4, off, lda=self.xz_ld, ws=ws)
        if stage is None:
            self._label_forward(X, eps_W, w_true, pack=pack if pack_in_label else None)
        nz = getattr(self, '_noise', None)
        ops.lstm_pair_fwd(B, T, L, self.gates_enc, self.wk_enc, self.gates_dec, off > 0, self.wk_dec, self.pair_pack,
                          P.p('Zargs/bias'), eps_Z, self.hs_enc, self.cs_enc, self.hs_dec, self.cs_dec, self.zargs, self.Z,
                          self.xz_ld, self.klterm, gate_act=self.gate_act, noise=nz[1] if nz else None, notes=notes)
        self._output_head(f8[0] if f8 is not None else (X if target is None else target), nll)

    def xp_view(self):
        return self.XZ.view(self.B, self.cfg['T'], self.xz_ld)[:, :, :self.cfg['D']]

    def x_hat(self):
        cfg, P = self.cfg, self.P
        ops.gemm(self.hs_dec, P.p('X_decoded_mean/kernel'), self.dlogits, self.B * cfg['T'], cfg['D'], cfg['H'],
                 bias=P.p('X_decoded_mean/bias'), act=ACT_SIGMOID, ws=self.ws)
        return self.dlogits

    def _wgrad_args(self, name, X_in, x_ld, x_rows, hs, dz, x8=None):
        cfg, P = self.cfg, self.P
        H, T, L = cfg['H'], cfg['T'], cfg['L']
        nz = L if name == 'decoder_h' else 0
        nx = x_rows - nz
        if not (self.bf16_wgrad and nx > 0 and ops.lstm_wgrad_supported(4 * H, nx, H, nz, self.frames_exact_bf16)):
            return None
        xs, xs_ld = (X_in, x_ld) if (x8 is None or nx == 0) else (x8, nx)
        return (self.B * T, 4 * H, xs, xs_ld, nx, self.frames_exact_bf16, hs, H, H, T, X_in[:, nx:] if nz else None, x_ld, nz,
                dz, P.g(name + '/kernel'), P.g(name + '/recurrent_kernel'),
                P.rows(P.grads, name + '/kernel', nx) if nz else None)

    def _lstm_wgrads(self, name, X_in, x_ld, x_rows, hs, dz, dzsum, w_row, ws, products=True, x8=None):
        cfg, P, B = self.cfg, self.P, self.B
        H, Cn = cfg['H'], cfg['C']
        G4 = 4 * H
        rq = self._rq()
        if products:
            args = self._wgrad_args(name, X_in, x_ld, x_rows, hs, dz, x8)
            if args is None and x8 is not None:
                raise RuntimeError("frames8: the %s kernel gradients have no byte-reading kernel at these shapes" % name)
            if args is not None:
                ops.lstm_wgrad(*args, ws, defer=rq, split_scale=2 if self.fine_grid else 1)
            else:
                self._lstm_wgrads_f32(name, X_in, x_ld, x_rows, hs, dz, ws, rq)
        if not (Cn + 1 <= 16 and B <= 4096):
            ops.gemm_grouped_tn([dict(A=self.W, lda=Cn, M=Cn, C=P.rows(P.grads, name + '/kernel', w_row)),
                                 dict(A=None, M=1, C=P.g(name + '/bias'), ones=1)], G4, B, dzsum, ws, defer=rq)

    def _lstm_wgrads_f32(self, name, X_in, x_ld, x_rows, hs, dz, ws, rq):
        cfg, P = self.cfg, self.P
        H, T = cfg['H'], cfg['T']
        BT, G4 = self.B * T, 4 * H
        ops.gemm_grouped_tn([dict(A=X_in, lda=x_ld, M=x_rows, C=P.g(name + '/kernel')),
                             dict(A=hs, lda=H, M=H, C=P.g(name + '/recurrent_kernel'), shift=1, zero_period=T)],
                            G4, BT, dz, ws, defer=rq, split_scale=2 if self.fine_grid else 1)

    def _dense_wgrad(self, name, A, lda, rows, N, K, Bm, ws, rq):
        P = self.P
        gk, gb = P.g(name + '/kernel'), P.g(name + '/bias')
        if gb.data_ptr() == gk.data_ptr() + 4 * rows * N and lda % 4 == 0 and A.data_ptr() % 16 == 0:
            probs = [dict(A=A, lda=lda, M=rows + 1, C=gk, ldc=N, ones=2)]
        else:
            probs = [dict(A=A, lda=lda, M=rows, C=gk), dict(A=None, M=1, C=gb, ones=1)]
        ops.gemm_grouped_tn(probs, N, K, Bm, ws, defer=rq)

    def _rq(self):
        return self.rq if self.side is None else None

    def tail_range(self):
        D, T = self.cfg['D'], self.cfg['T']
        return self.P.offsets['hW/kernel'], T * D * D

    def _bptt_separate(self, eps_Z, ws):
        cfg, P, B = self.cfg, self.P, self.B
        H, L, T = cfg['H'], cfg['L'], cfg['T']
        BT, G4, off = B * T, 4 * H, self.off
        g = ops.gemm
        if self.use_mx:
            ops.lstm_mx_bwd(B, T, P.p('decoder_h/recurrent_kernel'), self.dhs, self.cs_dec, self.gates_dec, self.dzsum_dec,
                            Kz=P.rows(P.params, 'decoder_h/kernel', off), nz=L, dZ=self.dZ, lddz=L)
        elif H == 88 and L <= 40:
            ops.lstm_seq_bwd_z(B, T, P.p('decoder_h/recurrent_kernel'), self.dhs, self.cs_dec, self.gates_dec,
                               self.dzsum_dec, P.rows(P.params, 'decoder_h/kernel', off), L, self.dZ, L,
                               gate_act=self.gate_act)
        else:
            ops.lstm_seq_bwd(B, T, P.p('decoder_h/recurrent_kernel'), self.dhs, self.cs_dec, self.gates_dec,
                             self.dzsum_dec, gate_act=self.gate_act, H=H)
            g(self.gates_dec, P.rows(P.params, 'decoder_h/kernel', off), self.dZ, BT, L, G4, tb=True, ws=ws)
        if self.fuse_latent:
            ops.latent_head_bwd(BT, H, L, self.hs_enc, P.p('Zargs/kernel'), self.zargs, eps_Z, self.dZ, L,
                                self.kl_weight / BT, self.dhs, P.g('Zargs/kernel'), P.g('Zargs/bias'), ws, defer=self._rq())
            self._head_grad_done = True
        else:
            ops.gauss_bwd(BT, L, self.zargs, eps_Z, self.dZ, L, self.kl_weight / BT, self.dzargs)
            g(self.dzargs, P.p('Zargs/kernel'), self.dhs, BT, H, 2 * L, tb=True, ws=ws)
        if self.use_mx:
            ops.lstm_mx_bwd(B, T, P.p('encoder_h/recurrent_kernel'), self.dhs, self.cs_enc, self.gates_enc, self.dzsum_enc)
        else:
            ops.lstm_seq_bwd(B, T, P.p('encoder_h/recurrent_kernel'), self.dhs, self.cs_enc, self.gates_enc,
                             self.dzsum_enc, gate_act=self.gate_act, H=H)

    def loss_and_grads(self, X, Xp, w_true, eps_W, eps_Z, need_grads=True, do_tail=True, target=None, noise=None, frames8=None):
        cfg, P, B = self.cfg, self.P, self.B
        D, H, L, T, Cn = cfg['D'], cfg['H'], cfg['L'], cfg['T'], cfg['C']
        C1, BT, G4 = Cn - 1, B * T, 4 * H
        inv_bt, inv_b = 1.0 / BT, 1.0 / B
        g, ws, off = ops.gemm, self.ws, self.off
        adjacent, self.halves_adjacent = bool(do_tail or self.halves_adjacent), False
        self._hw_outer = None
        self._train_pass = bool(need_grads)
        try:
            self.forward(X, Xp, eps_W, eps_Z, w_true, nll=(inv_bt, need_grads), target=target, noise=noise, frames8=frames8)
        finally:
            self._train_pass = False
        if not self._nll_done:
            ops.bernoulli_nll(BT, D, self.logits, X if target is None else target, D, inv_bt, self.rownll,
                              self.dlogits if need_grads else None)
        kl = (self.klterm, BT * L, 1) if self.fuse_pair else (self.rowkl, BT, 1)
        terms = [(self.rownll, BT, 1), kl, (self.rowloss, B, 3), (self.rowloss[:, 1:], B, 3), (self.rowloss[:, 2:], B, 3)]
        self._loss_terms = terms if (need_grads and self._rq() is not None) else None
        if self._loss_terms is None:
            ops.loss_sums(terms, self.scal)
        if not need_grads:
            self._join()
            return
        if not self._head_done:
            g(self.dlogits, P.p('X_decoded_mean/kernel'), self.dhs, BT, H, D, tb=True, ws=ws)
        if self.dropout:
            self._backward_dropout(X, w_true, eps_W, eps_Z)
            return
        if self.fuse_pair:
            label = None
            if self.label_in_pair:
                label = dict(D=D, C=Cn, Kenc_w=P.rows(P.params, 'encoder_h/kernel', D),
                             Kdec_w=P.rows(P.params, 'decoder_h/kernel', off + L), wargs=self.wargs, eps=eps_W, onehot=w_true,
                             W=self.W, hW=self.hW, Ka=P.p('Wargs/kernel'), prior=cfg['w_log_var_prior'],
                             class_weight=self.class_weight, w_kl_weight=self.w_kl_weight, inv_b=inv_b, dwargs=self.dwargs,
                             dhW=self.dhW, layer_grad=(P.g('Wargs/kernel'), P.g('Wargs/bias')))
            ops.lstm_pair_bwd(B, T, L, self.kl_weight * inv_bt, self.pair_pack, P.p('Zargs/kernel'), self.dhs,
                              self.cs_dec, self.cs_enc, self.gates_dec, self.gates_enc, self.dzsum_dec, self.dzsum_enc,
                              self.zargs, eps_Z, self.dzargs, gate_act=self.gate_act,
                              head_grad=(self.hs_enc, P.g('Zargs/kernel'), P.g('Zargs/bias')), ws=ws, defer=self._rq(),
                              label=label)
            self._head_grad_done = True
        else:
            self._bptt_separate(eps_Z, ws)
        if not (self.fuse_pair and self.label_in_pair):
            ops.vrnn_label_bwd(B, D, Cn, G4, self.dzsum_enc, self.dzsum_dec, P.rows(P.params, 'encoder_h/kernel', D),
                               P.rows(P.params, 'decoder_h/kernel', off + L), self.wargs, eps_W, w_true, self.W, self.hW,
                               P.p('Wargs/kernel'), cfg['w_log_var_prior'], self.class_weight, self.w_kl_weight, inv_b,
                               self.dwargs, self.dhW, layer_grad=(P.g('Wargs/kernel'), P.g('Wargs/bias')), ws=ws,
                               defer=self._rq())
        if self.sparse_inputs and ops.sparse_dense_supported(D):
            outer = ops.dense_outer_bf16 if (self.dense_hw_grad and self.frames_exact_bf16 and
                                             ops.dense_outer_bf16_supported(B, T * D, D, T * D, D)) else ops.sparse_outer
            frames = X if frames8 is None else frames8[0]
            gdot = (self.hW, D, P.p('hW/bias'), self.gdot)
            if (outer is ops.dense_outer_bf16 and self.tail_launch and adjacent and self._rq() is not None
                    and ops.reduce_outer_supported(B, T * D, D, T * D, D)):
                self._hw_outer = dict(Bn=B, nx=T * D, N=D, X=frames, ldx=T * D, G=self.dhW, ldg=D, out=P.g('hW/kernel'),
                                      colsum=P.g('hW/bias'), gdot=gdot)
            else:
                outer(B, T * D, D, frames, T * D, self.dhW, D, P.g('hW/kernel'), colsum=P.g('hW/bias'), gdot=gdot)
            self.gdot_fresh = True
        else:
            g(X, self.dhW, P.g('hW/kernel'), T * D, D, B, ta=True, ws=ws)
            ops.colsum(self.dhW, B, D, P.g('hW/bias'), ws)
        if do_tail:
            self.grads_tail(X, frames8=frames8)

    def grads_tail(self, X, frames8=None):
        cfg, P, B = self.cfg, self.P, self.B
        D, H, L, T, Cn = cfg['D'], cfg['H'], cfg['L'], cfg['T'], cfg['C']
        C1, BT, off = Cn - 1, B * T, self.off
        ws, rq = self.ws, self._rq()
        if self.dropout:
            return
        if not self._head_done:
            self._dense_wgrad('X_decoded_mean', self.hs_dec, H, H, D, BT, self.dlogits, ws, rq)
        dec = ('decoder_h', self.XZ, self.xz_ld, off + L, self.hs_dec, self.gates_dec)
        enc = ('encoder_h', X, D, D, self.hs_enc, self.gates_enc)
        if frames8 is not None:
            dec, enc = dec + (frames8[1],), enc + (frames8[0],)
        paired = False
        if self.wgrad_pair:
            pd, pe = self._wgrad_args(*dec), self._wgrad_args(*enc)
            if pd is not None and pe is not None and ops.lstm_wgrad_pair_supported(pd, pe):
                if rq is None and self.ws_b is None:
                    self.ws_b = ops.Workspace(self.device)
                ops.lstm_wgrad_pair(pd, pe, (ws, self.ws_b), defer=rq, split_scale=2 if self.fine_grid else 1)
                paired = True
        self._lstm_wgrads(*dec[:6], self.dzsum_dec, off + L, ws, products=not paired, x8=dec[6] if len(dec) > 6 else None)
        if not getattr(self, '_head_grad_done', False):
            self._dense_wgrad('Zargs', self.hs_enc, H, H, 2 * L, BT, self.dzargs, ws, rq)
        self._head_grad_done = False
        self._lstm_wgrads(*enc[:6], self.dzsum_enc, D, ws, products=not paired, x8=enc[6] if len(enc) > 6 else None)
        skinny = None
        if Cn + 1 <= 16 and B <= 4096:
            if rq is not None:
                skinny = [dict(A=self.W, lda=Cn, rows=Cn, B=dzs, ldb=4 * H, N=4 * H, K=B,
                               C=P.rows(P.grads, name + '/kernel', w_row), ldc=4 * H, bias_row=P.g(name + '/bias'))
                          for name, w_row, dzs in (('encoder_h', D, self.dzsum_enc), ('decoder_h', off + L, self.dzsum_dec))]
            else:
                wprobs = lambda name, w_row: [dict(A=self.W, lda=Cn, M=Cn, C=P.rows(P.grads, name + '/kernel', w_row)),
                                              dict(A=None, M=1, C=P.g(name + '/bias'), ones=1)]
                ops.gemm_grouped_tn_small2(wprobs('encoder_h', D), self.dzsum_enc, wprobs('decoder_h', off + L),
                                           self.dzsum_dec, 4 * H, B)
        if rq is not None:
            rq.flush(means=getattr(self, '_loss_terms', None), out=self.scal, skinny=skinny, outer=self._hw_outer)
            self._loss_terms = None
            self._hw_outer = None
```

### classifying-vae-lstm_amd/ops.py

```python
import ctypes as C

import torch

from . import _lib
from ._lib import ACT_NONE, ACT_RELU, ACT_SIGMOID, ACT_MASKPOS, check


def _ptr(t):
    return None if t is None else C.c_void_p(t.data_ptr())


def _stream():
    return C.c_void_p(torch.cuda.current_stream().cuda_stream)


class Workspace:

    def __init__(self, device, nbytes=1 << 20):
        self.device = device
        self.buf = torch.empty(int(nbytes), dtype=torch.uint8, device=device)

    def ensure(self, nbytes):
        if self.buf.numel() < nbytes:
            self.buf = torch.empty(int(nbytes * 1.25) + 256, dtype=torch.uint8, device=self.device)
        return self.buf


class ReduceQueue:
    MAX_JOBS = 16

    def __init__(self, device):
        self.device = device
        self.jobs = (_lib.ReduceJob * self.MAX_JOBS)()
        self.slots = [None] * self.MAX_JOBS
        self.n = 0

    def scratch(self, nbytes):
        if self.n >= self.MAX_JOBS:
            raise _lib.ClvError("ReduceQueue: more than %d pending reductions" % self.MAX_JOBS)
        buf = self.slots[self.n]
        if buf is None or buf.numel() < nbytes:
            buf = self.slots[self.n] = torch.empty(int(nbytes) + 256, dtype=torch.uint8, device=self.device)
        return buf

    def next_job(self):
        j = C.byref(self.jobs, self.n * C.sizeof(_lib.ReduceJob))
        self.n += 1
        return j

    def next_job_addr(self):
        a = C.addressof(self.jobs) + self.n * C.sizeof(_lib.ReduceJob)
        self.n += 1
        return a

    def flush(self, means=None, out=None, skinny=None, outer=None):
        if means or skinny or self.n or outer is not None:
            means = means or []
            k = len(means)
            xs = (C.c_void_p * max(k, 1))(*[_ptr(t) for t, _, _ in means])
            ns = (C.c_int * max(k, 1))(*[int(n) for _, n, _ in means])
            st = (C.c_int * max(k, 1))(*[int(s) for _, _, s in means])
            skinny = skinny or []
            riders = (_lib.SkinnyProduct * max(len(skinny), 1))()
            for i, p in enumerate(skinny):
                riders[i] = _lib.SkinnyProduct(_ptr(p['A']), p['lda'], p['rows'], _ptr(p['B']), p['ldb'], p['N'], p['K'],
                                               _ptr(p['C']), p['ldc'], _ptr(p.get('bias_row')))
            args = (self.jobs, self.n, xs if k else None, ns if k else None, st if k else None, k,
                    _ptr(out) if k else None, riders if skinny else None, len(skinny))
            if outer is None:
                check(_lib.lib().clv_splitk_reduce_multi(*args, _stream()), "clv_splitk_reduce_multi")
            else:
                o = outer
                h, ldh, hb, go = o['gdot'] if o.get('gdot') is not None else (None, 0, None, None)
                ldo = o['ldo'] if o.get('ldo') is not None else o['N']
                check(_lib.lib().clv_splitk_reduce_multi_outer(
                    *args, o['Bn'], o['nx'], o['N'], _ptr(o['X']), _is_u8(o['X']), o['ldx'], _ptr(o['G']), o['ldg'], _ptr(o['out']),
                    ldo, _ptr(o.get('colsum')), _ptr(h), int(ldh), _ptr(hb), _ptr(go), _stream()), "clv_splitk_reduce_multi_outer")
        self.n = 0


def reduce_outer_supported(Bn, nx, N, ldx, ldg):
    return bool(_lib.lib().clv_splitk_reduce_multi_outer_supported(Bn, nx, N, ldx, ldg))


def gemm(A, B, C_out, M, N, K, ta=False, tb=False, lda=None, ldb=None, ldc=None, alpha=1.0, beta=0.0,
         bias=None, act=ACT_NONE, aux=None, split_k=None, ws=None, defer=None):
    L = _lib.lib()
    lda = lda if lda is not None else (M if ta else K)
    ldb = ldb if ldb is not None else (K if tb else N)
    ldc = ldc if ldc is not None else N
    if split_k is None:
        split_k = L.clv_gemm_auto_split(M, N, K)
    wsp, wsb, job = None, 0, None
    if split_k > 1:
        need = L.clv_gemm_workspace_bytes(M, N, split_k)
        buf = defer.scratch(need) if defer is not None else ws.ensure(need)
        wsp, wsb = _ptr(buf), buf.numel()
        job = defer.next_job() if defer is not None else None
    check(L.clv_gemm_f32(int(ta), int(tb), M, N, K, float(alpha), _ptr(A), lda, _ptr(B), ldb, float(beta),
                                  _ptr(C_out), ldc, _ptr(bias), act, _ptr(aux), split_k, wsp, wsb, job, _stream()),
          "clv_gemm_f32")


def gemm_grouped_tn(probs, N, K, B, ws, ldb=None, beta=0.0, split_k=None, defer=None, split_scale=1):
    L = _lib.lib()
    arr = (_lib.GemmProb * len(probs))()
    for i, p in enumerate(probs):
        A = p.get('A')
        arr[i] = _lib.GemmProb(A.data_ptr() if A is not None else None, p.get('lda', p['M']), p['M'],
                               p['C'].data_ptr(), p.get('ldc', N), p.get('shift', 0), p.get('zero_period', 0),
                               int(p.get('ones', 0)))
    n = len(probs)
    if split_k is None:
        split_k = L.clv_gemm_grouped_auto_split(arr, n, N, K)
        if split_k > 1:
            split_k *= int(split_scale)
    wsp, wsb, job = None, 0, None
    if split_k > 1:
        need = L.clv_gemm_grouped_workspace_bytes(arr, n, N, split_k)
        buf = defer.scratch(need) if defer is not None else ws.ensure(need)
        wsp, wsb = _ptr(buf), buf.numel()
        job = defer.next_job() if defer is not None else None
    check(L.clv_gemm_grouped_tn(arr, n, N, K, _ptr(B), ldb if ldb is not None else N, float(beta), split_k,
                                         wsp, wsb, job, _stream()), "clv_gemm_grouped_tn")


def lstm_wgrad_supported(N, nx, nh, nz, x_exact_bf16):
    return bool(_lib.lib().clv_lstm_wgrad_supported(N, nx, nh, nz, int(bool(x_exact_bf16))))


def lstm_wgrad(K, N, X, ldx, nx, x_exact_bf16, H, ldh, nh, T, Z, ldz, nz, dz, dKx, dU, dKz, ws, defer=None, beta=0.0,
               split_scale=1):
    L = _lib.lib()
    need = L.clv_lstm_wgrad_workspace_bytes(K, N, nx, nh, nz, int(split_scale))
    buf = defer.scratch(need) if defer is not None else ws.ensure(need)
    job = defer.next_job() if defer is not None else None
    check(L.clv_lstm_wgrad(K, N, _ptr(X), ldx, nx, _frames_mode(X, x_exact_bf16), _ptr(H), ldh, nh, 1, T,
                              _ptr(Z), ldz, nz, _ptr(dz), N, _ptr(dKx), N, _ptr(dU), N, _ptr(dKz), N, float(beta),
                              int(split_scale), _ptr(buf), buf.numel(), job, _stream()), "clv_lstm_wgrad")


def _wgrad_problem(K, N, X, ldx, nx, x_exact_bf16, H, ldh, nh, T, Z, ldz, nz, dz, dKx, dU, dKz, beta=0.0):
    w = _lib.WgradProblem()
    w.K, w.N = K, N
    w.X, w.ldx, w.nx, w.x_exact_bf16 = _ptr(X), ldx, nx, _frames_mode(X, x_exact_bf16)
    w.H, w.ldh, w.nh, w.h_shift, w.h_zero_period = _ptr(H), ldh, nh, 1, T
    w.Z, w.ldz, w.nz = _ptr(Z), ldz, nz
    w.dz, w.lddz = _ptr(dz), N
    w.dKx, w.ld_kx, w.dU, w.ld_u, w.dKz, w.ld_kz = _ptr(dKx), N, _ptr(dU), N, _ptr(dKz), N
    w.beta = float(beta)
    return w


def lstm_wgrad_pair_supported(p, q):
    a, b = _wgrad_problem(*p), _wgrad_problem(*q)
    return bool(_lib.lib().clv_lstm_wgrad_pair_supported(C.byref(a), C.byref(b)))


def lstm_wgrad_pair(p, q, ws, defer=None, split_scale=1):
    L = _lib.lib()
    probs, jobs = [], []
    for i, t in enumerate((p, q)):
        w = _wgrad_problem(*t)
        need = L.clv_lstm_wgrad_pair_workspace_bytes(w.K, w.N, w.nx, w.nh, w.nz, int(split_scale))
        buf = defer.scratch(need) if defer is not None else ws[i].ensure(need)
        jobs.append(defer.next_job() if defer is not None else None)
        w.ws, w.ws_bytes = _ptr(buf), buf.numel()
        probs.append(w)
    check(L.clv_lstm_wgrad_pair(C.byref(probs[0]), C.byref(probs[1]), int(split_scale), jobs[0], jobs[1], _stream()),
          "clv_lstm_wgrad_pair")


def gemm_bce(A, B, bias, Y, scale, logits, dlogits, rownll, M, N, K, lda=None, ldb=None, ldy=None, ldc=None):
    check(_lib.lib().clv_gemm_bce_f32(M, N, K, _ptr(A), lda if lda is not None else K, _ptr(B),
                                      ldb if ldb is not None else N, _ptr(bias), _ptr(Y), ldy if ldy is not None else N,
                                      float(scale), _ptr(logits), _ptr(dlogits), ldc if ldc is not None else N,
                                      _ptr(rownll), _stream()), "clv_gemm_bce_f32")


def out_head_train_supported(H, D):
    return bool(_lib.lib().clv_out_head_train_supported(H, D))


def out_head_train(R, H, D, hs, Wo, bo, Y, scale, rownll, dhs, dWo, dbo, ws, logits=None, dlogits=None, ldy=None,
                   defer=None):
    L = _lib.lib()
    need = L.clv_out_head_train_workspace_bytes(R)
    buf = defer.scratch(need) if defer is not None else ws.ensure(need)
    job = defer.next_job() if defer is not None else None
    check(L.clv_out_head_train(R, H, D, _ptr(hs), _ptr(Wo), _ptr(bo), _ptr(Y), _is_u8(Y), ldy if ldy is not None else D,
                               float(scale), _ptr(logits), _ptr(rownll), _ptr(dlogits), _ptr(dhs), _ptr(dWo), _ptr(dbo),
                               _ptr(buf), buf.numel(), job, _stream()), "clv_out_head_train")


def latent_head_supported(H, L):
    return bool(_lib.lib().clv_latent_head_supported(H, L))


def latent_head_fwd(R, H, L, hs, Wz, bz, eps, zargs, Z, ldz, rowkl=None, noise=None):
    check(_lib.lib().clv_latent_head_fwd(R, H, L, _ptr(hs), _ptr(Wz), _ptr(bz), _ptr(eps), _ptr(zargs), _ptr(Z), ldz,
                                         _ptr(rowkl), _noise_ref(noise), _stream()), "clv_latent_head_fwd")


def latent_head_bwd(R, H, L, hs, Wz, zargs, eps, dZ, lddz, kl_scale, dhs, dWz, dbz, ws, dzargs=None, defer=None):
    Lb = _lib.lib()
    need = Lb.clv_latent_head_bwd_workspace_bytes(R, L)
    buf = defer.scratch(need) if defer is not None else ws.ensure(need)
    job = defer.next_job() if defer is not None else None
    check(Lb.clv_latent_head_bwd(R, H, L, _ptr(hs), _ptr(Wz), _ptr(zargs), _ptr(eps), _ptr(dZ), lddz, float(kl_scale),
                                 _ptr(dzargs), _ptr(dhs), _ptr(dWz), _ptr(dbz), _ptr(buf), buf.numel(), job, _stream()),
          "clv_latent_head_bwd")


def _prob_array(probs, N):
    arr = (_lib.GemmProb * len(probs))()
    for i, p in enumerate(probs):
        A = p.get('A')
        arr[i] = _lib.GemmProb(A.data_ptr() if A is not None else None, p.get('lda', p['M']), p['M'],
                               p['C'].data_ptr(), p.get('ldc', N), p.get('shift', 0), p.get('zero_period', 0),
                               int(p.get('ones', 0)))
    return arr


def gemm_grouped_tn_small2(probs0, B0, probs1, B1, N, K, ldb=None):
    a0, a1 = _prob_array(probs0, N), _prob_array(probs1, N)
    check(_lib.lib().clv_gemm_grouped_tn_small2(a0, len(probs0), _ptr(B0), a1, len(probs1), _ptr(B1), N, K,
                                                ldb if ldb is not None else N, _stream()), "clv_gemm_grouped_tn_small2")


def loss_sums(terms, out):
    a = []
    for t, n, st in terms:
        a += [_ptr(t), n, st]
    check(_lib.lib().clv_loss_sums(*a, _ptr(out), _stream()), "clv_loss_sums")

# ... 580 lines not shown
```

### classifying-vae-lstm_amd/params.py

```python
import ctypes as C

import numpy as np
import torch

from . import _lib, ops


def fuse_heads(shapes, pairs):
    d = dict(shapes)
    phys, aliases, done = [], {}, set()
    for name, shp in shapes:
        layer, w = name.split('/')
        hit = [pr for pr in pairs if layer in pr[:2]]
        if not hit:
            phys.append((name, shp))
            continue
        a, b, fused = hit[0]
        na, nb = d[a + '/kernel'][1], d[b + '/kernel'][1]
        for wn in ('kernel', 'bias'):
            aliases[a + '/' + wn] = (fused + '/' + wn, 0, na)
            aliases[b + '/' + wn] = (fused + '/' + wn, na, nb)
        if fused not in done:
            done.add(fused)
            phys.append((fused + '/kernel', (d[a + '/kernel'][0], na + nb)))
            phys.append((fused + '/bias', (na + nb,)))
    return phys, aliases


class FlatParams:

    def __init__(self, shapes, device, phys=None, aliases=None, pre=0):
        self.logical = list(shapes)
        self.aliases = dict(aliases or {})
        self.shapes = list(phys) if phys is not None else list(shapes)
        self.device = device
        self.offsets, self.col_offsets = {}, {}
        off = col = 0
        table = (_lib.ParamDesc * len(self.shapes))()
        for i, (name, shp) in enumerate(self.shapes):
            n = int(np.prod(shp))
            self.offsets[name] = off
            is_mat = len(shp) > 1
            rows = int(np.prod(shp[:-1])) if is_mat else 1
            table[i] = _lib.ParamDesc(off, rows, int(shp[-1]), col if is_mat else 0, int(is_mat), 0)
            if is_mat:
                self.col_offsets[name] = col
                col += (int(shp[-1]) + 3) // 4 * 4
            off += (n + 3) // 4 * 4
        self.n, self.n_cols, self.table = off, max(col, 4), table
        self._subplans = {}
        f = dict(dtype=torch.float32, device=device)
        self.params = torch.zeros(self.n, **f)
        pre = (int(pre) + 3) // 4 * 4
        self.grads_store = torch.zeros(pre + self.n, **f)
        self.grads_pre, self.grads = self.grads_store[:pre], self.grads_store[pre:]
        self.m = torch.zeros(self.n, **f)
        self.v = torch.zeros(self.n, **f)
        self.mg = torch.zeros(self.n_cols, **f)
        self.vg = torch.zeros(self.n_cols, **f)
        self.s = torch.ones(self.n_cols, **f)
        self.vn2 = torch.zeros(self.n_cols, **f)
        self.norms_valid = False
        self.iterations = torch.zeros(1, dtype=torch.int32, device=device)
        L = _lib.lib()
        nb = L.clv_adam_wn_plan_bytes(table, len(self.shapes))
        blob = (C.c_uint8 * nb)()
        _lib.check(L.clv_adam_wn_plan_build(table, len(self.shapes), blob), "adam plan")
        self.plan = torch.from_numpy(np.frombuffer(blob, dtype=np.uint8).copy()).to(device)
        self.adam_ws = torch.empty(L.clv_adam_wn_workspace_bytes(table, len(self.shapes)), dtype=torch.uint8,
                                   device=device)

    def view(self, buf, name):
        if name in self.aliases:
            phys, c0, nc = self.aliases[name]
            return self.view(buf, phys)[..., c0:c0 + nc]
        shp = dict(self.shapes)[name]
        o = self.offsets[name]
        return buf[o:o + int(np.prod(shp))].view(*shp)

    def p(self, name):
        return self.view(self.params, name)

    def g(self, name):
        return self.view(self.grads, name)

    def rows(self, buf, name, r0):
        shp = dict(self.shapes)[name]
        o = self.offsets[name] + r0 * int(shp[-1])
        return buf[o:]

    def set_weights(self, weights):
        for name, _ in self.logical:
            self.p(name).copy_(torch.as_tensor(np.asarray(weights[name], dtype=np.float32)))
        self.norms_valid = False

    def get_weights(self, buf=None):
        buf = self.params if buf is None else buf
        return {name: self.view(buf, name).detach().cpu().numpy().copy() for name, _ in self.logical}

    def state_tensors(self):
        return [self.params, self.m, self.v, self.mg, self.vg, self.s, self.vn2, self.iterations]

    def reset_optimizer(self):
        for t in (self.m, self.v, self.mg, self.vg):
            t.zero_()
        self.s.fill_(1.0)
        self.iterations.zero_()
        self.norms_valid = False

    def _subplan(self, names):
        key = tuple(names)
        if key not in self._subplans:
            idx = [i for i, (name, _) in enumerate(self.shapes) if name in names]
            table = (_lib.ParamDesc * len(idx))(*[self.table[i] for i in idx])
            L = _lib.lib()
            blob = (C.c_uint8 * L.clv_adam_wn_plan_bytes(table, len(idx)))()
            _lib.check(L.clv_adam_wn_plan_build(table, len(idx), blob), "adam plan")
            plan = torch.from_numpy(np.frombuffer(blob, dtype=np.uint8).copy()).to(self.device)
            self._subplans[key] = (table, len(idx), plan)
        return self._subplans[key]

    def tall_tensor(self):
        tall = [(i, name) for i, (name, shp) in enumerate(self.shapes) if len(shp) > 1 and int(np.prod(shp[:-1])) > 144]
        return tall[0] if len(tall) == 1 else None

    def adam_step(self, lr=1e-3, b1=0.9, b2=0.999, eps=1e-8, weightnorm=True, only=None, advance=True, advanced=False,
                  gdot=None):
        table, n, plan = (self.table, len(self.shapes), self.plan) if only is None else self._subplan(only)
        known, tall = None, self.tall_tensor()
        if int(weightnorm) == 1 and tall is not None and (only is None or tall[1] in only):
            use = gdot is not None and self.norms_valid
            pos = tall[0] if only is None else [name for name, _ in self.shapes if name in only].index(tall[1])
            known = _lib.AdamKnownSums(pos, int(use), ops._ptr(gdot) if use else None, ops._ptr(self.vn2))
        _lib.check(_lib.lib().clv_adam_wn_step(
            table, n, ops._ptr(plan), ops._ptr(self.params), ops._ptr(self.grads),
            ops._ptr(self.m), ops._ptr(self.v), ops._ptr(self.mg), ops._ptr(self.vg), ops._ptr(self.s),
            ops._ptr(self.iterations), -2 if advanced else (0 if advance else -1), lr, b1, b2, eps, int(weightnorm),
            C.byref(known) if known is not None else None, ops._ptr(self.adam_ws),
            self.adam_ws.numel(), ops._stream()), "clv_adam_wn_step")
        self.norms_valid = known is not None or (self.norms_valid and tall is not None and only is not None
                                                 and tall[1] not in only)
```

### classifying-vae-lstm_amd/trainer.py

```python
import os

import numpy as np

import torch

from . import ops
from .parallel import GradAllReduce, eps_first_index, meta_device


IW_STREAM_W, IW_STREAM_Z = 0xFFFFFFFE, 0xFFFFFFFF
SMC_STREAM = 0xFFFFFFFD
SMC_W_STREAM = 0xFFFFFFFC
KEY_STREAM = 0xFFFFFFFB


class DevWindows:

    def __init__(self, store, starts, t0):
        self.store, self.starts, self.t0 = store, starts, int(t0)
        self.shape = (int(starts.shape[0]),)


class TrainStep:
    def __init__(self, engine, seed=1234, rank=0, world=1, group=None, optimizer='adam-wn',
# ... 21 lines not shown
            self.xp_ld = engine.xz_ld
        else:
            self.Xp = torch.zeros(*shp, **f)
        self.Y = None
        self.X8 = self.Xp8 = None
        self._f8 = None
        self.w_true = torch.zeros(B, cfg['C'], **f)
        self.eps_w = torch.zeros(B, C1, **f)
        self.eps_z = torch.zeros(B * T, L, **f)
        tail = engine.tail_range() if self.is_vrnn else (0, 0)
        force = os.environ.get('CLV_FORCE_DP_GRAPHS') == '1'
        P = engine.P
        self.pre_in_tail = bool(self.is_vrnn and tail[1] and tail[0] == 0 and P.grads_pre.numel() > 0
                                and getattr(engine, 'gdot', None) is not None
                                and engine.gdot.data_ptr() == P.grads_pre.data_ptr())
        real = os.environ.get('CLV_DP_REAL_COLLECTIVES') == '1'
        if self.pre_in_tail:
            self.ar = GradAllReduce(P.grads_store, 0, P.grads_pre.numel() + tail[1], group, always=real) \
                if (world > 1 or force) else None
        else:
            self.ar = GradAllReduce(P.grads, tail[0], tail[1], group, always=real) if (world > 1 or force) else None
        self.tail_names = [n for n, _ in engine.P.shapes if tail[1] and engine.P.offsets[n] == tail[0]
                           and int(np.prod(dict(engine.P.shapes)[n])) == tail[1]]
        self.rest_names = [n for n, _ in engine.P.shapes if n not in self.tail_names]
        self.split_update = self.ar is not None and len(self.tail_names) == 1
        self.dp_trials = None
        self.capture_collectives = os.environ.get('CLV_CAPTURE_COLLECTIVES', '1') != '0'
        self.capture_note = None
        self._graphs = None
        self._warm = False
        self._bound = None
        self.loss_acc = None

    def noise_spec(self, stream_offset=0, row0=None):
        eng, B = self.eng, self.eng.B
        C1, L = eng.cfg['C'] - 1, eng.cfg['L']
        T = eng.cfg['T'] if self.is_vrnn else 1
        row0 = self.rank * B if row0 is None else int(row0)
        return (self.seed, 2 * stream_offset, 2 * stream_offset + 1, eps_first_index(row0, C1),
                eps_first_index(row0, T * L), 0, eng.P.iterations)

    def draw_noise(self, stream_offset=0, row0=None):
        eng, B = self.eng, self.eng.B
        T = eng.cfg['T'] if self.is_vrnn else 1
        seed, sw, sz, fw, fz, step, it = self.noise_spec(stream_offset, row0)
        ops.philox_normal2(self.eps_w, B * (eng.cfg['C'] - 1), sw, fw, self.eps_z, B * T * eng.cfg['L'], sz, fz, seed, step,
                           step_dev=it)

    def _folded(self):
        return (not self.is_vrnn) and self.eng.folds_step(self.w_true)

    def set_target(self, on):
        if bool(on) != (self.Y is not None):
            self.Y = torch.zeros_like(self.X) if on else None
            self.recapture()

    def bind_batches(self, d_cur, d_hist, d_w, idx=None, period=1, stride=None, offset=0, d_target=None):
        self.set_target(d_target is not None)
        self._bound = dict(cur=d_cur, hist=d_hist, w=d_w, idx=idx, period=int(period),
                           stride=int(self.eng.B if stride is None else stride), offset=int(offset), target=d_target,
                           step0=int(self.eng.P.iterations.item()))
        self.recapture()

    def unbind_batches(self):
        if self._bound is not None:
            self._bound = None
            self.recapture()

    def _bytes_batch(self, b):
        eng = self.eng
        if not (self.is_vrnn and b['target'] is None and getattr(eng, 'frames_u8_route', lambda: None)() == 'gather'):
            return None
        need_hist = eng.off > 0
        if need_hist != (b['hist'] is not None):
            return None
        for x in ((b['cur'], b['hist']) if need_hist else (b['cur'],)):
            t = x.store if isinstance(x, DevWindows) else x
            if t.dtype != torch.uint8 or not t.is_contiguous():
                return None
        if self.X8 is None:
            shp = tuple(self.X.shape)
            self.X8 = torch.zeros(*shp, dtype=torch.uint8, device=self.X.device)
            self.Xp8 = torch.zeros(*shp, dtype=torch.uint8, device=self.X.device) if need_hist else None
        return (self.X8, self.Xp8)

    def _stage_bound(self):
        b = self._bound
        self._f8 = self._bytes_batch(b)
        segs = self._segments(b['cur'], b['hist'], b['w'], b['target'], bytes_out=self._f8)
        ops.gather_rows_multi(self.eng.B, b['idx'], segs, notes=self._note_outputs(b['cur'], b['hist'], len(segs)),
                              cursor=(self.eng.P.iterations, b['step0'], b['period'], b['stride'], b['offset']))

    def _label_stage(self):
        b, eng = self._bound, self.eng
        if os.environ.get('CLV_STAGE_IN_LABEL', '1') == '0' or b['target'] is not None:
            return None
        if not getattr(eng, 'can_stage_in_label', lambda: False)():
            return None
        if not self.is_vrnn and not (self._folded() and b['w'] is not None):
            return None
        need_hist = (eng.off > 0) if self.is_vrnn else bool(eng.cfg['use_x_prev'])
        if need_hist != (b['hist'] is not None):
            return None
        D, row = eng.cfg['D'], int(self.X[0].numel())

        def src(x):
            if isinstance(x, DevWindows):
                return (x.store, D, x.t0 * D, x.starts)
            return (x, row, 0, None)
        cur = src(b['cur'])
        hist = src(b['hist']) if need_hist else None
        if any(t is not None and (t[0].dtype != torch.uint8 or not t[0].is_contiguous()) for t in (cur, hist)):
            return None
        if b['w'].dtype != torch.float32 or not b['w'].is_contiguous():
            return None
        if hasattr(eng, 'frames_exact_bf16') and not eng.frames_exact_bf16:
            eng.frames_exact_bf16 = True
            self.recapture()
        hist_chunk, hist_ld = (D, self.xp_ld) if self.xp_ld else (row, row)
        f8 = None
        if self.is_vrnn and getattr(eng, 'frames_u8_route', lambda: None)() == 'label':
            if self.X8 is None:
                self.X8 = torch.zeros(tuple(self.X.shape), dtype=torch.uint8, device=self.X.device)
                self.Xp8 = torch.zeros(tuple(self.X.shape), dtype=torch.uint8, device=self.X.device) if need_hist else None
            f8 = (self.X8, self.Xp8)
        self._f8 = f8
        return ops.label_stage(cur, hist, b['idx'], 0, (eng.P.iterations, b['step0'], b['period'], b['stride'], b['offset']),
                               self.X, self.Xp if need_hist else None, hist_chunk, hist_ld, b['w'], self.w_true, bytes_out=f8)

    def _main(self):
        if not self._drop_logits:
            return self._main_pass()
        keep, self.eng.keep_logits = self.eng.keep_logits, False
        try:
            return self._main_pass()
        finally:
            self.eng.keep_logits = keep

    def _main_pass(self):
        self._f8 = None
        if self._bound is not None:
            st = self._label_stage()
            if st is None:
                self._stage_bound()
            elif hasattr(self.eng, 'stage_spec'):
                self.eng.stage_spec = st
        if self._folded():
            self.eng.loss_and_grads(self.X, self.Xp, self.w_true, self.eps_w, self.eps_z, target=self.Y,
                                    noise=self.noise_spec(), bump=True)
            return
        if self.is_vrnn:
            if hasattr(self.eng, 'halves_adjacent'):
                self.eng.halves_adjacent = self.ar is None
            self.eng.loss_and_grads(self.X, self.Xp, self.w_true, self.eps_w, self.eps_z, do_tail=False, target=self.Y,
                                    noise=self.noise_spec(), frames8=self._f8)
            return
        self.draw_noise()
        self.eng.loss_and_grads(self.X, self.Xp, self.w_true, self.eps_w, self.eps_z, target=self.Y)

    def _tail(self):
        if self.is_vrnn:
            self.eng.grads_tail(self.X, frames8=self._f8)

    def _update(self):
        eng = self.eng
        eng.P.adam_step(lr=self.lr, b2=self.b2, weightnorm=self.weightnorm, advanced=self._folded(), gdot=self._gdot())

    def _gdot(self):
        eng = self.eng
        ok = self.fast_adam and getattr(eng, 'gdot_fresh', False) and (self.ar is None or self.pre_in_tail)
        if hasattr(eng, 'gdot_fresh'):
            eng.gdot_fresh = False
        return eng.gdot if ok else None

    def _update_tail(self):
        self.eng.P.adam_step(lr=self.lr, b2=self.b2, weightnorm=self.weightnorm, only=self.tail_names, advance=False,
                             advanced=self._folded(), gdot=self._gdot())

    def _update_rest(self):
        self.eng.P.adam_step(lr=self.lr, b2=self.b2, weightnorm=self.weightnorm, only=self.rest_names,
                             advanced=self._folded())

    def _segments(self, cur, hist, w, target=None, bytes_out=None):
        row, D = int(self.X[0].numel()), self.eng.cfg['D']

        def src(x):
            return (x.store, (D, x.t0 * D, x.starts)) if isinstance(x, DevWindows) else (x, ())
        exact = all(src(x)[0].dtype == torch.uint8 for x in (cur, hist) if x is not None)
        if hasattr(self.eng, 'frames_exact_bf16') and self.eng.frames_exact_bf16 != exact:
            self.eng.frames_exact_bf16 = exact
            self.recapture()
        c, cx = src(cur)
        if bytes_out is not None:
            segs = [(c, bytes_out[0], row, D, D) + cx]
            if hist is not None:
                h, hx = src(hist)
                segs.append((h, bytes_out[1], row, D, D) + hx)
            segs.append((w, self.w_true, int(self.w_true.shape[1]), 0, 0))
            return segs
        segs = [(c, self.X, row, D, D) + cx]
        if hist is not None:
            h, hx = src(hist)
            if self.xp_ld:
                segs.append((h, self.Xp, row, D, self.xp_ld) + hx)
            else:
                segs.append((h, self.Xp, row, 0, 0) + hx)
        segs.append((w, self.w_true, int(self.w_true.shape[1]), 0, 0))
        if target is not None:
            t, tx = src(target)
            segs.append((t, self.Y, row, 0, 0) + tx)
        return segs

    def _note_outputs(self, cur, hist, nseg):
        eng = self.eng
        if not getattr(eng, 'fuse_notes', False):
            return None
        need = [cur, hist] if eng.off else [cur]
        ok = all(x is not None and self._is_binary_u8(x.store if isinstance(x, DevWindows) else x) for x in need)
        if eng.notes_valid != ok:
            eng.notes_valid = ok
            self.recapture()
        if not ok:
            return None
        out = [None] * nseg
        out[0] = eng.notes_enc
        if eng.off:
            out[1] = eng.notes_dec
        return out

    def _is_binary_u8(self, t):
        if t.dtype != torch.uint8:
            return False
        key = (t.untyped_storage().data_ptr(), t.untyped_storage().nbytes())
        cache = self.__dict__.setdefault('_binary_stores', {})
        if key not in cache:
            whole = torch.empty(0, dtype=torch.uint8, device=t.device).set_(t.untyped_storage())
            cache[key] = bool((whole <= 1).all().item())
        return cache[key]

    def stage_batch(self, X, Xp, w_true, target=None):
        self.set_target(target is not None)
        segs = self._segments(X, Xp, w_true, target)
        ops.gather_rows_multi(self.eng.B, None, segs, notes=self._note_outputs(X, Xp, len(segs)))

    def gather_batch(self, d_cur, d_hist, d_w, ib, row0=0, d_target=None):
        self.set_target(d_target is not None)
        segs = self._segments(d_cur, d_hist, d_w, d_target)
        ops.gather_rows_multi(self.eng.B, ib, segs, row0=row0, notes=self._note_outputs(d_cur, d_hist, len(segs)))

    def _accumulate(self):
        if self.loss_acc is not None:
            ops.axpy(5, 1.0, self.eng.scal, self.loss_acc)

    def _single(self):
        self._main()
        self._tail()
        self._update()
        self._accumulate()

    def _eager(self):
        if self.ar is None:
            return self._single()
        self._main()
        if self.ar is not None:
            self.ar.reduce_tail()
        self._tail()
        if self.ar is not None:
            self.ar.reduce_main()
            if self.split_update:
                self.ar.wait_tail()
                self._update_tail()
                self.ar.wait()
                self._update_rest()
                self._accumulate()
                return
            self.ar.wait()
        self._update()
        self._accumulate()

    def tune_dp_schedule(self, steps=20, warm=3):
        import time
        eng = self.eng
        if self.ar is None or not hasattr(eng, 'fine_grid') or 'fine_grid' in eng.cfg:
            return None
        import torch.distributed as dist
        saved = [t.clone() for t in eng.P.state_tensors()]
        flags = (eng.P.norms_valid, getattr(eng, 'gdot_fresh', False))
        res = {}
        for name, fine in (('coarse_ms', False), ('fine_ms', True)):
            eng.fine_grid = fine
            self.recapture()
            self._warm = False
            for _ in range(warm):
                self.step()
            torch.cuda.synchronize()
            if self.ar.world > 1:
                dist.barrier()
            t0 = time.perf_counter()
            for _ in range(steps):
                self.step()
            torch.cuda.synchronize()
            ms = torch.tensor([1e3 * (time.perf_counter() - t0) / steps], dtype=torch.float64, device=meta_device(eng.device))
            if self.ar.world > 1:
                dist.all_reduce(ms, op=dist.ReduceOp.MAX)
            res[name] = round(float(ms.item()), 4)
            for t, sv in zip(eng.P.state_tensors(), saved):
                t.copy_(sv)
            eng.P.norms_valid = flags[0]
            if hasattr(eng, 'gdot_fresh'):
                eng.gdot_fresh = flags[1]
        eng.fine_grid = res['fine_ms'] < res['coarse_ms']
        res['chosen'] = 'fine' if eng.fine_grid else 'coarse'
        self.recapture()
        self._warm = False
        self.dp_trials = res
        return res

    def recapture(self):
        self._graphs = None
# ... 97 lines not shown
```

### include/clvae.h

```cpp
#ifndef CLVAE_H
#define CLVAE_H

#include <stddef.h>
#include <stdint.h>

#ifdef __cplusplus
extern "C" {
#endif

#define CLV_OK          0
#define CLV_EINVAL     (-1)
#define CLV_EWORKSPACE (-2)
#define CLV_ENOGPU     (-3)

#define CLV_ACT_NONE     0
#define CLV_ACT_RELU     1
#define CLV_ACT_SIGMOID  2
#define CLV_ACT_MASKPOS  3

#define CLV_GATE_HARD_SIGMOID 0
#define CLV_GATE_SIGMOID      1

typedef struct clv_pair_pack_src {
  int H, L;
// ... 255 lines not shown
int clv_lerp_rows(int64_t R, int64_t n, const float* a, const int32_t* ia, const float* b, const int32_t* ib,
                  const float* alpha, float* out, void* stream);

int clv_label_fwd(int B, int C, const float* mean, const float* logvar, int ld_in,
                  const float* eps, const float* onehot, float prior_logvar,
                  float* w, float* rowloss, void* stream);
int clv_label_bwd(int B, int C, const float* mean, const float* logvar, int ld_in,
                  const float* eps, const float* onehot, const float* w, const float* dw,
                  float prior_logvar, float class_weight, float w_kl_weight, float inv_b,
                  float* dmean, float* dlogvar, int ld_out, void* stream);

int clv_vae_fused_supported(int D, int H, int Hc, int C, int L);
size_t clv_vae_fused_workspace_bytes(int B, int D, int H, int Hc, int C, int L, int use_x_prev);

typedef struct clv_vae_step_opts {
  int draw;
  uint32_t stream_w, stream_z, step;
  uint64_t noise_seed, first_w, first_z;
  const int32_t* step_dev;
  float* loss_means;
  int32_t* bump_iterations;
  int bf16;
} clv_vae_step_opts;

int clv_vrnn_label_fwd(int B, int D, int C, int G4, const float* hW, const float* Ka, const float* ba,
                       const float* eps, const float* onehot, float prior_logvar,
                       const float* Kenc_w, const float* benc, const float* Kdec_w, const float* bdec,
                       float* wargs, float* W, float* rowloss, float* rb_enc, float* rb_dec, void* stream);
int clv_vrnn_label_fwd_x(int B, int D, int C, int G4, const float* X, int ldx, int nx, const float* Kh,
                         const clv_label_stage* stage,
                         const float* bh, float* hW_out, const float* Ka, const float* ba,
                         float* eps, const float* onehot, float prior_logvar,
                         const float* Kenc_w, const float* benc, const float* Kdec_w, const float* bdec,
                         float* wargs, float* W, float* rowloss, float* rb_enc, float* rb_dec,
                         const clv_noise_draw* noise, const clv_pair_pack_src* pack,
                         const clv_frame_proj* proj,
                         void* stream);
int clv_vrnn_label_fwd_x_proj_supported(int B, int D, int nx, int T, int N);
int clv_dense_window_fwd_bf16_supported(int Bn, int nx, int N, int ldx, int ldk);
int clv_dense_window_fwd_bf16_splits(int Bn, int nx);
size_t clv_dense_window_fwd_bf16_workspace_bytes(int Bn, int nx, int N);
int clv_dense_window_fwd_bf16(int Bn, int nx, int N, const void* X, int x_u8, int ldx, const float* K, int ldk, float* part,
                              size_t part_bytes, void* stream);
int clv_vrnn_label_fwd_parts(int B, int D, int C, int G4, const float* part, int splits,
                             const float* bh, float* hW_out, const float* Ka, const float* ba,
                             float* eps, const float* onehot, float prior_logvar,
                             const float* Kenc_w, const float* benc, const float* Kdec_w, const float* bdec,
                             float* wargs, float* W, float* rowloss, float* rb_enc, float* rb_dec,
                             const clv_noise_draw* noise, const clv_pair_pack_src* pack, void* stream);
int clv_vae_fused_step(int B, int D, int H, int Hc, int C, int L, int use_x_prev,
                       const float* x, const float* xp, const float* target, const float* onehot,
                       const clv_label_stage* stage, float* eps_w, float* eps_z,
                       const float* params, const int64_t* host_offsets12, long n_params,
                       float prior_logvar, float class_weight, float kl_weight, float w_kl_weight,
                       int need_grads, float* grads, void* ws, size_t ws_bytes,
                       float* logits, float* w_out, float* wargs_out, float* zargs_out,
                       float* rownll, float* rowkl, float* rowloss, const clv_vae_step_opts* opts, void* stream);
size_t clv_vrnn_label_bwd_workspace_bytes(int B, int D, int C);
int clv_vrnn_label_bwd(int B, int D, int C, int G4, const float* dzsum_enc, const float* dzsum_dec,
                          const float* Kenc_w, const float* Kdec_w, const float* wargs, const float* eps,
                          const float* onehot, const float* W, const float* hW, const float* Ka,
                          float prior_logvar, float class_weight, float w_kl_weight, float inv_b,
                          float* dwargs, float* dhW, float* dKa, float* dba, void* ws, size_t ws_bytes,
                          clv_reduce_job* job, void* stream);

int clv_gauss_fwd(int R, int L, const float* zargs, const float* eps, float* z, int ldz,
                  float* rowkl, void* stream);
int clv_gauss_bwd(int R, int L, const float* zargs, const float* eps, const float* dz, int lddz,
                  float kl_scale, float* dzargs, void* stream);

int clv_bernoulli_nll(int R, int D, const float* logits, const float* y, int ldy, float scale,
                      float* rownll, float* dlogits, void* stream);
int clv_gemm_bce_f32(int M, int N, int K, const float* A, int lda, const float* B, int ldb, const float* bias,
                     const float* Y, int ldy, float scale, float* logits, float* dlogits, int ldc,
                     float* rownll, void* stream);

int clv_out_head_train_supported(int H, int D);
size_t clv_out_head_train_workspace_bytes(int R);
int clv_out_head_train(int R, int H, int D, const float* hs, const float* Wo, const float* bo,
                       const void* Y, int y_u8, int ldy, float scale, float* logits, float* rownll, float* dlogits,
                       float* dhs, float* dWo, float* dbo, void* ws, size_t ws_bytes, clv_reduce_job* job,
                       void* stream);

int clv_latent_head_supported(int H, int L);
size_t clv_latent_head_bwd_workspace_bytes(int R, int L);
int clv_latent_head_fwd(int R, int H, int L, const float* hs, const float* Wz, const float* bz, float* eps,
                        float* zargs, float* Z, int ldz, float* rowkl, const clv_noise_draw* noise, void* stream);
int clv_latent_head_bwd(int R, int H, int L, const float* hs, const float* Wz, const float* zargs, const float* eps,
                        const float* dZ, int lddz, float kl_scale, float* dzargs, float* dhs, float* dWz, float* dbz,
                        void* ws, size_t ws_bytes, clv_reduce_job* job, void* stream);

int clv_act_grad(int64_t n, int act, const float* y, const float* dy, float* dpre, void* stream);
int clv_axpy(int64_t n, float alpha, const float* x, float* y, void* stream);

int clv_sparse_proj_supported(int nx, int N);
size_t clv_sparse_proj_lds_bytes(int nx, int N);
int clv_sparse_proj(int R, int nx, int N, const void* X, int x_u8, int ldx, const float* K, float* out, int ldo, void* stream);
int clv_sparse_proj2(int R, int N, int ldo, int x_u8, int nx0, const void* X0, int ldx0, const float* K0, float* out0,
                     int nx1, const void* X1, int ldx1, const float* K1, float* out1, void* stream);

int clv_sparse_dense_supported(int N);
int clv_sparse_dense(int R, int nx, int N, const float* X, int ldx, const float* K, const float* bias, int act,
                     float* out, int ldo, void* stream);
int clv_sparse_outer(int Bn, int nx, int N, const float* X, int ldx, const float* G, int ldg, float* out, int ldo,
                        float* colsum, const float* Hact, int ldh, const float* hbias, float* gdot, void* stream);

int clv_dense_outer_bf16_supported(int Bn, int nx, int N, int ldx, int ldg);
int clv_dense_outer_bf16(int Bn, int nx, int N, const void* X, int x_u8, int ldx, const float* G, int ldg, float* out, int ldo,
                         float* colsum, const float* Hact, int ldh, const float* hbias, float* gdot, void* stream);

int clv_gather_rows(int64_t rows, int64_t row_elems, const float* src, const int64_t* idx, float* out,
                    int64_t chunk, int64_t out_ld, void* stream);
#define CLV_NOTE_ROW 96
#define CLV_NOTE_NONE 88
int clv_gather_rows_multi(int64_t rows, const int64_t* idx, int64_t row0, int nseg,
                                 const void* const* src, const int32_t* src_u8, float* const* out,
                                 const int64_t* row_elems, const int64_t* chunk, const int64_t* out_ld,
                                 const int64_t* src_stride, const int64_t* src_offset,
                                 const int64_t* const* src_table, unsigned char* const* notes_out,
                                 const clv_batch_cursor* cursor, void* stream);

int clv_loss_sums(const float* x0, int n0, int s0, const float* x1, int n1, int s1, const float* x2, int n2, int s2,
                  const float* x3, int n3, int s3, const float* x4, int n4, int s4, float* out, void* stream);

int clv_sum_strided(int n, const float* x, int stride, float scale, float* out, void* stream);

typedef struct clv_param_desc {
  int64_t offset;
  int32_t rows;
  int32_t cols;
  int64_t col_offset;
  int32_t is_matrix;
  int32_t pad_;
} clv_param_desc;
size_t clv_adam_wn_plan_bytes(const clv_param_desc* host_table, int n_tensors);
int clv_adam_wn_plan_build(const clv_param_desc* host_table, int n_tensors, void* host_blob);
size_t clv_adam_wn_workspace_bytes(const clv_param_desc* host_table, int n_tensors);
#define CLV_STEP_ADVANCED (-2)
#define CLV_OPT_ADAM     0
#define CLV_OPT_ADAM_WN  1
#define CLV_OPT_RMSPROP  2
typedef struct clv_adam_known_sums {
  int tensor;
  int use;
  const float* gdot;
  float* vnorm2;
} clv_adam_known_sums;
int clv_adam_wn_step(const clv_param_desc* host_table, int n_tensors, const void* plan_dev,
                        float* params, const float* grads, float* m, float* v,
                        float* mg, float* vg, float* s,
                        int32_t* iterations_dev, int step_t, float lr, float beta1, float beta2, float eps,
                        int weightnorm, const clv_adam_known_sums* known, void* ws, size_t ws_bytes, void* stream);

int clv_philox_normal(float* out, int64_t n, uint64_t seed, uint32_t step, const int32_t* step_dev,
                      uint32_t stream_id, uint64_t first_index, void* stream);
int clv_philox_uniform(float* out, int64_t n, uint64_t seed, uint32_t step, const int32_t* step_dev,
                       uint32_t stream_id, uint64_t first_index, void* stream);
int clv_philox_normal2(float* out0, int64_t n0, uint32_t stream_id0, uint64_t first_index0,
                       float* out1, int64_t n1, uint32_t stream_id1, uint64_t first_index1,
                       uint64_t seed, uint32_t step, const int32_t* step_dev, void* stream);
int clv_i32_add(int32_t* counter, int32_t v, void* stream);
int clv_bernoulli_sample(int64_t n, const float* p, const float* u, float* x, void* stream);
int clv_bernoulli_sample_clamped(int64_t n, int D, int nsteps, int S, const float* p, const float* u, const uint8_t* clamp,
                                 const int32_t* step_dev, float* x, void* stream);
int clv_dropout_rows(int R, int T, int n, const float* X, int ldx, const float* U, int ldu, float rate, float beta,
                     float* out, int ldo, void* stream);

int clv_iw_accumulate(int R, int T, int L, int C1, const float* rownll, const float* zargs, const float* eps_z,
                      const float* wargs, const float* eps_w, float w_log_var_prior, int nvalid, double* state,
                      int32_t* step_dev, void* stream);
int clv_iw_finish(int R, int nvalid, int K, const double* state, double* log_p, double* elbo, double* ess, void* stream);

int clv_smc_sample(int R, int D, int P, int nsteps, int S, const float* p, const float* u, const uint8_t* clamp,
                   const int32_t* step_dev, float* x, double* ell, uint8_t* hist, void* stream);
int clv_smc_resample(int G, int P, int nsteps, int S, uint64_t seed, int64_t m0, double tau, const double* ell, double* logW,
                     double* logZ, double* ess, int32_t* nres, int32_t* flag, int32_t* anc, const int32_t* step_dev,
                     void* stream);
int clv_smc_gather(int R, int P, int nsteps, int S, int nbuf, float* const* bufs, const int* widths, float* scratch,
                   const int32_t* anc, const int32_t* flag, const int32_t* step_dev, void* stream);
int clv_smc_backtrack(int G, int P, int nsteps, int D, int n_out, uint64_t seed, int64_t m0, int step, const double* logW,
                      const int32_t* anc, const uint8_t* hist, float* Xs, int32_t* picks, void* stream);
int clv_smc_init_w(int G, int P, int C, int mode, uint64_t seed, int64_t m0, const double* probs, const float* mean,
                   const float* log_var, float* wr, void* stream);
int clv_smc_w_posterior(int G, int P, int C, int nsteps, int S, const double* logW, const float* wr, const int32_t* step_dev,
                        double* out, void* stream);
int clv_smc_take_w(int G, int P, int C, int n_out, const int32_t* picks, const float* wr, float* w_out, void* stream);

int clv_key_track_windows(int N, int T, int D, int Hd, int C, int hop, int K, const uint8_t* frames,
                          const int64_t* piece_off, const int64_t* win_off, const float* Kh, const float* bh,
                          const float* Ka, const float* ba, uint64_t seed, int64_t piece0, float* wargs, float* logp,
                          void* stream);
int clv_key_track_smooth(int N, int C, const int64_t* win_off, const float* logp, const double* log_prior,
                         const double* log_trans, double kappa, double* post, int32_t* path, double* log_evidence,
                         double* piece_post, void* stream);

int clv_graph_begin_capture(void* stream);
int clv_graph_end_capture(void* stream, void** graph_exec_out);
int clv_graph_launch(void* graph_exec, void* stream);
int clv_graph_destroy(void* graph_exec);

typedef struct clv_prof_record {
  char name[48];
  int32_t launches;
  float total_ms;
} clv_prof_record;
int clv_prof_enable(int on);
int clv_prof_collect(clv_prof_record* host_out, int cap);
int clv_prof_empty_scope(void* stream);

#ifdef __cplusplus
}
#endif
#endif
```

Measured before the change: 102.0 million timesteps/s.

## Fuse weight-norm Adam update of the tall tensor into the outer-product reduce tail

Moves the weight-normalized Adam update for the single tall parameter tensor into the epilogue of the split-K outer-product reduction kernel, so the freshly computed gradient tile is updated while still on-chip instead of being written and re-read by a separate optimizer pass. A new close kernel then merges the small-tensor Adam updates with the per-column norm rescale into a single launch. The intent is fewer kernel launches and less gradient and parameter memory traffic per step. It adds LDS reuse inside the product kernel and depends on tight shape constraints, with a fallback to the old path when they are not met.

Result: no change. 101.5 million timesteps/s, median of 2 (-0.5%).

```diff
diff --git a/classifying-vae-lstm_amd/_lib.py b/classifying-vae-lstm_amd/_lib.py
--- a/classifying-vae-lstm_amd/_lib.py
+++ b/classifying-vae-lstm_amd/_lib.py
@@ -124,6 +124,9 @@
     "clv_splitk_reduce_multi_outer_supported": (_i, [_i, _i, _i, _i, _i]),
     "clv_splitk_reduce_multi_outer": (_i, [_p, _i, _p, _p, _p, _i, _p, _p, _i,
                                            _i, _i, _i, _p, _i, _i, _p, _i, _p, _i, _p, _p, _i, _p, _p, _p]),
+    "clv_splitk_reduce_multi_outer_adam_supported": (_i, [_p, _i, _i, _i, _i, _i, _i, _i, _i, _i]),
+    "clv_splitk_reduce_multi_outer_adam": (_i, [_p, _i, _p, _p, _p, _i, _p, _p, _i,
+                                                _i, _i, _i, _p, _i, _i, _p, _i, _p, _i, _p, _p, _i, _p, _p, _p, _p]),
     "clv_lstm_wgrad_supported": (_i, [_i, _i, _i, _i, _i]),
     "clv_lstm_wgrad_workspace_bytes": (_sz, [_i, _i, _i, _i, _i, _i]),
     "clv_lstm_wgrad_pair_supported": (_i, [_p, _p]),
@@ -217,6 +220,8 @@
     "clv_adam_wn_plan_build": (_i, [_p, _i, _p]),
     "clv_adam_wn_workspace_bytes": (_sz, [_p, _i]),
     "clv_adam_wn_step": (_i, [_p, _i, _p, _p, _p, _p, _p, _p, _p, _p, _p, _i, _f, _f, _f, _f, _i, _p, _p, _sz, _p]),
+    "clv_adam_in_tail_supported": (_i, [_p, _i, _i, _i, _i]),
+    "clv_adam_wn_close": (_i, [_p, _i, _p, _p, _p, _p, _p, _p, _p, _p, _p, _i, _f, _f, _f, _f, _p, _p, _sz, _p]),
     "clv_philox_normal2": (_i, [_p, _i64, _u32, _u64, _p, _i64, _u32, _u64, _u64, _u32, _p, _p]),
     "clv_gather_rows_multi": (_i, [_i64, _p, _i64, _i, _p, _p, _p, _p, _p, _p, _p, _p, _p, _p, _p, _p]),
     "clv_philox_normal": (_i, [_p, _i64, _u64, _u32, _p, _u32, _u64, _p]),
diff --git a/classifying-vae-lstm_amd/csrc/adam_fast_body.h b/classifying-vae-lstm_amd/csrc/adam_fast_body.h
--- /dev/null
+++ b/classifying-vae-lstm_amd/csrc/adam_fast_body.h
@@ -0,0 +1,141 @@
+#pragma once
+#include "common.h"
+
+namespace clv {
+
+struct AdamHyper {
+  float lr, b1, b2, eps;
+  int weightnorm;
+  int step_t;
+  const int32_t* iterations;
+};
+
+__device__ __forceinline__ int adam_t(const AdamHyper& h) {
+  return h.iterations ? (*h.iterations + (h.step_t == CLV_STEP_ADVANCED ? 0 : 1)) : h.step_t;
+}
+__device__ __forceinline__ float adam_lr_t(const AdamHyper& h) {
+  const int t = adam_t(h);
+  return h.lr * sqrtf(1.f - powf(h.b2, (float)t)) / (1.f - powf(h.b1, (float)t));
+}
+
+#ifndef CLV_FAST_ROWS
+#define CLV_FAST_ROWS 64
+#endif
+constexpr int FAST_ROWS = CLV_FAST_ROWS;
+constexpr int FAST_NT = 1024;
+struct AdamFast {
+  int64_t offset, col_offset;
+  int rows, cols, nunits;
+  const float* gdot;
+  float* vn2;
+  float* gnew;
+  float* partC;
+};
+
+struct TailAdam {
+  int on;
+  AdamFast f;
+  float* params; float* m; float* v; float* mg; float* vg; const float* s;
+  AdamHyper h;
+  int32_t* t_out;
+};
+
+int adam_fast_layout(const clv_param_desc* host_table, int n_tensors, int tensor, const float* gdot, float* vn2, void* ws,
+                     size_t ws_bytes, AdamFast* f, int32_t** t_slot);
+
+__device__ __forceinline__ void lds_barrier() { asm volatile("s_waitcnt lgkmcnt(0)\n\ts_barrier" ::: "memory"); }
+
+#ifndef CLV_ADAM_FLAT_PT
+#define CLV_ADAM_FLAT_PT 2
+#endif
+
+template <int NT, int PT, bool G_LDS, bool LIGHT, bool MID_FIRST, class Mid>
+__device__ __forceinline__ void wn_fast_tile_flat(const AdamFast& f, int unit, float* params, const float* grads, const float* g_lds,
+                                                  float* m, float* v, float* mg, float* vg, const float* s, const AdamHyper& h,
+                                                  const float* gdot, float (*cs)[128], float* sq, int32_t* t_out, int tid, Mid mid) {
+#pragma clang fp contract(off)
+  auto barrier = [] { if (LIGHT) lds_barrier(); else __syncthreads(); };
+  const float lr_t = adam_lr_t(h);
+  if (unit == 0 && tid == 0 && t_out) *t_out = adam_t(h);
+  const int row0 = unit * FAST_ROWS, nrows = min(FAST_ROWS, f.rows - row0);
+  const int n4 = nrows * f.cols / 4;
+  const size_t o0 = f.offset + (size_t)row0 * f.cols;
+  constexpr int NTA = (FAST_ROWS * 128 / 4 + PT - 1) / PT < NT ? (FAST_ROWS * 128 / 4 + PT - 1) / PT : NT;
+  if (MID_FIRST) mid();
+  float4 pv[PT], gv[PT], mv[PT], vv[PT];
+#pragma unroll
+  for (int k = 0; k < PT; ++k) {
+    const size_t o = o0 + 4 * (size_t)min(tid + NTA * k, n4 - 1);
+    pv[k] = *reinterpret_cast<const float4*>(params + o);
+    if (!G_LDS) gv[k] = *reinterpret_cast<const float4*>(grads + o);
+    mv[k] = *reinterpret_cast<const float4*>(m + o); vv[k] = *reinterpret_cast<const float4*>(v + o);
+  }
+  if (!MID_FIRST) mid();
+  for (int c = tid; c < f.cols; c += NT) {
+    const size_t cg = f.col_offset + c;
+    const float sc = s[cg], a = f.vn2[cg];
+    const float Vn = sqrtf(a), inv_s = 1.f / sc;
+    const float grad_g = gdot[c] * inv_s / Vn;
+    cs[0][c] = inv_s; cs[1][c] = grad_g / Vn; cs[2][c] = sc;
+    if (unit == 0) {
+      const float mgn = fmaf(1.f - h.b1, grad_g, h.b1 * mg[cg]);
+      const float vgn = h.b2 * vg[cg] + ((1.f - h.b2) * grad_g) * grad_g;
+      mg[cg] = mgn; vg[cg] = vgn;
+      f.gnew[c] = sc * Vn - lr_t * mgn / (sqrtf(vgn) + h.eps);
+    }
+  }
+  barrier();
+#pragma unroll
+  for (int k = 0; k < PT; ++k) {
+    const int i = tid + NTA * k;
+    if (tid < NTA && i < n4) {
+      if (G_LDS) gv[k] = *reinterpret_cast<const float4*>(g_lds + 4 * i);
+      const int c0 = (4 * i) % f.cols;
+      const float pin[4] = {pv[k].x, pv[k].y, pv[k].z, pv[k].w}, gin[4] = {gv[k].x, gv[k].y, gv[k].z, gv[k].w};
+      const float min_[4] = {mv[k].x, mv[k].y, mv[k].z, mv[k].w}, vin[4] = {vv[k].x, vv[k].y, vv[k].z, vv[k].w};
+      const float4 c_is = *reinterpret_cast<const float4*>(&cs[0][c0]), c_gg = *reinterpret_cast<const float4*>(&cs[1][c0]),
+                   c_sc = *reinterpret_cast<const float4*>(&cs[2][c0]);
+      const float is4[4] = {c_is.x, c_is.y, c_is.z, c_is.w}, gg4[4] = {c_gg.x, c_gg.y, c_gg.z, c_gg.w}, sc4[4] = {c_sc.x, c_sc.y, c_sc.z, c_sc.w};
+      float po[4], mo[4], vo[4];
+#pragma unroll
+      for (int c = 0; c < 4; ++c) {
+        const float V = pin[c] * is4[c];
+        const float gV = sc4[c] * fmaf(-V, gg4[c], gin[c]);
+        mo[c] = fmaf(h.b1, min_[c], (1.f - h.b1) * gV);
+        vo[c] = fmaf(h.b2, vin[c], ((1.f - h.b2) * gV) * gV);
+        po[c] = V - lr_t * mo[c] / (sqrtf(vo[c]) + h.eps);
+      }
+      const size_t o = o0 + 4 * (size_t)i;
+      *reinterpret_cast<float4*>(m + o) = make_float4(mo[0], mo[1], mo[2], mo[3]);
+      *reinterpret_cast<float4*>(v + o) = make_float4(vo[0], vo[1], vo[2], vo[3]);
+      *reinterpret_cast<float4*>(params + o) = make_float4(po[0], po[1], po[2], po[3]);
+      *reinterpret_cast<float4*>(sq + 4 * i) = make_float4(po[0] * po[0], po[1] * po[1], po[2] * po[2], po[3] * po[3]);
+    }
+  }
+  barrier();
+  constexpr int VK = (8 * 128 + NT - 1) / NT;
+  float part[VK];
+#pragma unroll
+  for (int k = 0; k < VK; ++k) {
+    const int vt = tid + NT * k;
+    const int cx = vt % f.cols, rl = vt / f.cols;
+    part[k] = 0.f;
+    if (rl < 8)
+      for (int r = rl; r < nrows; r += 8) part[k] += sq[r * f.cols + cx];
+  }
+  barrier();
+#pragma unroll
+  for (int k = 0; k < VK; ++k) {
+    const int vt = tid + NT * k;
+    if (vt < 8 * f.cols) sq[vt] = part[k];
+  }
+  barrier();
+  if (tid < f.cols) {
+    float t = 0.f;
+#pragma unroll
+    for (int w = 0; w < 8; ++w) t += sq[w * f.cols + tid];
+    f.partC[(size_t)unit * f.cols + tid] = t;
+  }
+}
+
+}
diff --git a/classifying-vae-lstm_amd/csrc/optim.hip b/classifying-vae-lstm_amd/csrc/optim.hip
--- a/classifying-vae-lstm_amd/csrc/optim.hip
+++ b/classifying-vae-lstm_amd/csrc/optim.hip
@@ -1,4 +1,4 @@
-#include "common.h"
+#include "adam_fast_body.h"
 
 namespace clv {
 
@@ -24,18 +24,6 @@
   int32_t cols;
   int32_t col_local;
 };
-struct AdamHyper {
-  float lr, b1, b2, eps;
-  int weightnorm;
-  int step_t;
-  const int32_t* iterations;
-};
-
-__device__ __forceinline__ float adam_lr_t(const AdamHyper& h) {
-  const int t = h.iterations ? (*h.iterations + (h.step_t == CLV_STEP_ADVANCED ? 0 : 1)) : h.step_t;
-  return h.lr * sqrtf(1.f - powf(h.b2, (float)t)) / (1.f - powf(h.b1, (float)t));
-}
-
 __global__ __launch_bounds__(256) void wn_stats_kernel(const AdamUnit* units, const float* params, const float* grads,
                                                        const float* s, float* partA, float* partB) {
   const AdamUnit un = units[blockIdx.x];
@@ -358,20 +346,6 @@
 
 __global__ void adam_bump_kernel(int32_t* iterations) { *iterations += 1; }
 
-#ifndef CLV_FAST_ROWS
-#define CLV_FAST_ROWS 64
-#endif
-constexpr int FAST_ROWS = CLV_FAST_ROWS;
-constexpr int FAST_NT = 1024;
-struct AdamFast {
-  int64_t offset, col_offset;
-  int rows, cols, nunits;
-  const float* gdot;
-  float* vn2;
-  float* gnew;
-  float* partC;
-};
-
 __device__ __forceinline__ void wn_fast_update_body(const AdamFast& f, int unit, float* params, const float* grads, float* m,
                                                     float* v, float* mg, float* vg, const float* s, const AdamHyper& h) {
   __shared__ float cs[3][128];
@@ -462,9 +436,6 @@
   const int row0 = unit * FAST_ROWS, nrows = min(FAST_ROWS, f.rows - row0);
   const int n4 = nrows * f.cols / 4;
   const size_t o0 = f.offset + (size_t)row0 * f.cols;
-#ifndef CLV_ADAM_FLAT_PT
-#define CLV_ADAM_FLAT_PT 2
-#endif
   constexpr int PT = CLV_ADAM_FLAT_PT;
   constexpr int NTA = (FAST_ROWS * 128 / 4 + PT - 1) / PT < FAST_NT ? (FAST_ROWS * 128 / 4 + PT - 1) / PT : FAST_NT;
   float4 pv[PT], gv[PT], mv[PT], vv[PT];
@@ -534,9 +505,9 @@
   wn_fast_update_body(f, (int)blockIdx.x, params, grads, m, v, mg, vg, s, h);
 }
 
-__global__ __launch_bounds__(FAST_NT) void wn_fast_rescale_kernel(AdamFast f, float* params, float* s, int32_t* iterations) {
+__device__ __forceinline__ void wn_fast_rescale_body(const AdamFast& f, int unit, float* params, float* s, int32_t* iterations) {
   __shared__ __attribute__((aligned(16))) float2 red[16][64], snew[64];
-  const int tid = threadIdx.x, cx = tid & 63, ry = tid >> 6, unit = blockIdx.x, n2 = f.cols / 2;
+  const int tid = threadIdx.x, cx = tid & 63, ry = tid >> 6, n2 = f.cols / 2;
   if (unit == 0 && tid == 0 && iterations) *iterations += 1;
 #if CLV_ADAM_FLAT
   const bool flat = f.cols % 4 == 0 && f.offset % 4 == 0;
@@ -596,6 +567,21 @@
         *reinterpret_cast<float2*>(params + f.offset + (size_t)(row0 + ry + 16 * i) * f.cols + 2 * cx) =
             make_float2(pv[i].x * sn.x, pv[i].y * sn.y);
   }
+}
+
+__global__ __launch_bounds__(FAST_NT) void wn_fast_rescale_kernel(AdamFast f, float* params, float* s, int32_t* iterations) {
+  wn_fast_rescale_body(f, (int)blockIdx.x, params, s, iterations);
+}
+
+__global__ __launch_bounds__(FAST_NT) void wn_close_kernel(AdamFast f, int n_small, const SmallItem* items, float* params,
+                                                           const float* grads, float* m, float* v, float* mg, float* vg, float* s,
+                                                           AdamHyper h, int32_t* iterations) {
+  if ((int)blockIdx.x < n_small) {
+    if (threadIdx.x >= 256) return;
+    wn_small_body(items[blockIdx.x], params, grads, m, v, mg, vg, s, h);
+    return;
+  }
+  wn_fast_rescale_body(f, (int)blockIdx.x - n_small, params, s, iterations);
 }
 
 struct PlanCounts { int n_units, n_cols, n_part, n_small, n_big; };
@@ -674,6 +660,59 @@
   if (!host_table || n_tensors <= 0) return 0;
   PlanCounts c = plan_counts(host_table, n_tensors);
   return (size_t)(3 * c.n_part + 4 * c.n_cols + 16) * sizeof(float);
+}
+
+int clv::adam_fast_layout(const clv_param_desc* host_table, int n_tensors, int tensor, const float* gdot, float* vn2, void* ws,
+                          size_t ws_bytes, AdamFast* f, int32_t** t_slot) {
+  if (!host_table || n_tensors <= 0 || !gdot || !vn2) return CLV_EINVAL;
+  if (!clv_adam_in_tail_supported(host_table, n_tensors, tensor, CLV_OPT_ADAM_WN, 1)) return CLV_EINVAL;
+  if (!ws || ws_bytes < clv_adam_wn_workspace_bytes(host_table, n_tensors)) return CLV_EWORKSPACE;
+  const PlanCounts c = plan_counts(host_table, n_tensors);
+  const clv_param_desc& t = host_table[tensor];
+  const int nunits = (t.rows + FAST_ROWS - 1) / FAST_ROWS;
+  if ((size_t)nunits * t.cols > (size_t)c.n_part) return CLV_EWORKSPACE;
+  float* partC = (float*)ws + 2 * (size_t)c.n_part;
+  float* colscal = partC + c.n_part;
+  *f = AdamFast{t.offset, t.col_offset, t.rows, t.cols, nunits, gdot, vn2, colscal, partC};
+  *t_slot = reinterpret_cast<int32_t*>(colscal + 4 * (size_t)c.n_cols);
+  return CLV_OK;
+}
+
+extern "C" int clv_adam_in_tail_supported(const clv_param_desc* host_table, int n_tensors, int tensor, int weightnorm,
+                                          int known_sums) {
+  if (!host_table || n_tensors <= 0 || tensor < 0 || tensor >= n_tensors) return 0;
+  if (weightnorm != CLV_OPT_ADAM_WN || !known_sums) return 0;
+  for (int i = 0; i < n_tensors; ++i)
+    if (host_table[i].rows <= 0 || host_table[i].cols <= 0) return 0;
+  const PlanCounts c = plan_counts(host_table, n_tensors);
+  const clv_param_desc& t = host_table[tensor];
+  if (c.n_big != 1 || is_small(t)) return 0;
+  if (t.cols % 4 || t.cols > 128 || t.offset % 4 || t.col_offset % 2) return 0;
+  return 1;
+}
+
+extern "C" int clv_adam_wn_close(const clv_param_desc* host_table, int n_tensors, const void* plan_dev,
+                                 float* params, const float* grads, float* m, float* v, float* mg, float* vg, float* s,
+                                 int32_t* iterations_dev, int step_t, float lr, float beta1, float beta2, float eps,
+                                 const clv_adam_known_sums* known, void* ws, size_t ws_bytes, void* stream) {
+  if (!host_table || n_tensors <= 0 || !plan_dev || !params || !grads || !m || !v || !mg || !vg || !s) return CLV_EINVAL;
+  if (!known || !known->use) return CLV_EINVAL;
+  AdamFast f;
+  int32_t* t_slot = nullptr;
+  if (int e = adam_fast_layout(host_table, n_tensors, known->tensor, known->gdot, known->vnorm2, ws, ws_bytes, &f, &t_slot)) return e;
+  const PlanCounts c = plan_counts(host_table, n_tensors);
+  const char* p = (const char*)plan_dev;
+  p += align_up(sizeof(AdamUnit) * c.n_units, 16);
+  p += align_up(sizeof(AdamCol) * (c.n_cols > 0 ? c.n_cols : 1), 16);
+  p += align_up(sizeof(int32_t) * c.n_units, 16);
+  const SmallItem* small = (const SmallItem*)p;
+  AdamHyper h{lr, beta1, beta2, eps, CLV_OPT_ADAM_WN, CLV_STEP_ADVANCED, t_slot};
+  int32_t* bump = (iterations_dev && (step_t == -1 || step_t == CLV_STEP_ADVANCED)) ? nullptr : iterations_dev;
+  hipStream_t st = (hipStream_t)stream;
+  ProfScope pr("adam_wn_close", st);
+  hipLaunchKernelGGL(wn_close_kernel, dim3(c.n_small + f.nunits), dim3(FAST_NT), 0, st, f, c.n_small, small, params, grads, m, v,
+                     mg, vg, s, h, bump);
+  return launch_status();
 }
 
 extern "C" int clv_adam_wn_step(const clv_param_desc* host_table, int n_tensors, const void* plan_dev,
diff --git a/classifying-vae-lstm_amd/csrc/outer_bf16_body.h b/classifying-vae-lstm_amd/csrc/outer_bf16_body.h
--- a/classifying-vae-lstm_amd/csrc/outer_bf16_body.h
+++ b/classifying-vae-lstm_amd/csrc/outer_bf16_body.h
@@ -1,5 +1,6 @@
 #pragma once
 #include "bf16_images.h"
+#include "adam_fast_body.h"
 
 namespace clv {
 
@@ -12,6 +13,9 @@
 constexpr int OD_IMG = OD_KS * OD_P;
 constexpr int OD_BUF = 4 * OD_IMG;
 constexpr int OD_LDS = 2 * OD_BUF;
+constexpr int OD_ADAM_CS = 64 * 96 * 4, OD_ADAM_GD = OD_ADAM_CS + 3 * 128 * 4, OD_ADAM_RED = OD_ADAM_GD + 128 * 4;
+constexpr int OD_ADAM_MAX_VW = 8;
+static_assert(OD_ADAM_RED + OD_ADAM_MAX_VW * 64 * 8 <= OD_LDS, "the Adam epilogue fits the product's allocation");
 
 struct OuterBf16Args {
   int Bn, nx, N, ldx, ldg, ldo;
@@ -40,8 +44,57 @@
 
 inline int od_own_launch_waves(int nx) { return (nx + 95) / 96 >= 100 ? 6 : 3; }
 
-template <int OD_NW, bool XU8>
-__device__ __forceinline__ void dense_outer_block(const OuterBf16Args& a, char* od_lds, int blk, int vw) {
+template <int OD_NW, int GR>
+__device__ __forceinline__ void od_gdot_in_tile(const OuterBf16Args& a, float2* red, float* gd, int vw, int wave, int lane) {
+  const int n2 = a.N / 2, cl = min(lane, n2 - 1);
+  const float2 hb = make_float2(a.hbias[2 * cl], a.hbias[2 * cl + 1]);
+  const int w0 = wave, w1 = wave + OD_NW;
+  const float* gp = a.G + 2 * cl;
+  const float* hp = a.Hact + 2 * cl;
+  float2 g0 = make_float2(0.f, 0.f), g1 = make_float2(0.f, 0.f);
+  for (int base = 0; base < a.Bn; base += 8 * vw) {
+#pragma unroll
+    for (int i0 = 0; i0 < 8; i0 += GR) {
+      float2 hv0[GR], gv0[GR], hv1[GR], gv1[GR];
+#pragma unroll
+      for (int i = 0; i < GR; ++i) {
+        const int b0 = min(base + w0 + (i0 + i) * vw, a.Bn - 1), b1 = min(base + w1 + (i0 + i) * vw, a.Bn - 1);
+        gv0[i] = *reinterpret_cast<const float2*>(gp + (size_t)b0 * a.ldg);
+        hv0[i] = *reinterpret_cast<const float2*>(hp + (size_t)b0 * a.ldh);
+        gv1[i] = *reinterpret_cast<const float2*>(gp + (size_t)b1 * a.ldg);
+        hv1[i] = *reinterpret_cast<const float2*>(hp + (size_t)b1 * a.ldh);
+      }
+      if (base + w0 < a.Bn) {
+#pragma unroll
+        for (int i = 0; i < GR; ++i) {
+          const float mk = base + w0 + (i0 + i) * vw < a.Bn ? 1.f : 0.f;
+          g0.x = fmaf((hv0[i].x - hb.x) * mk, gv0[i].x, g0.x);
+          g0.y = fmaf((hv0[i].y - hb.y) * mk, gv0[i].y, g0.y);
+        }
+      }
+      if (w1 < vw && base + w1 < a.Bn) {
+#pragma unroll
+        for (int i = 0; i < GR; ++i) {
+          const float mk = base + w1 + (i0 + i) * vw < a.Bn ? 1.f : 0.f;
+          g1.x = fmaf((hv1[i].x - hb.x) * mk, gv1[i].x, g1.x);
+          g1.y = fmaf((hv1[i].y - hb.y) * mk, gv1[i].y, g1.y);
+        }
+      }
+    }
+  }
+  if (w0 < vw) red[w0 * 64 + lane] = g0;
+  if (w1 < vw) red[w1 * 64 + lane] = g1;
+  lds_barrier();
+  if (wave == 0 && lane < n2) {
+    float2 u = make_float2(0.f, 0.f);
+    for (int w = 0; w < vw; ++w) { u.x += red[w * 64 + lane].x; u.y += red[w * 64 + lane].y; }
+    gd[2 * lane] = u.x; gd[2 * lane + 1] = u.y;
+  }
+  lds_barrier();
+}
+
+template <int OD_NW, bool XU8, bool ADAM = false>
+__device__ __forceinline__ void dense_outer_block(const OuterBf16Args& a, char* od_lds, int blk, int vw, const TailAdam* ta = nullptr) {
   constexpr int OD_NT = 64 * OD_NW, OD_JT = 16 * OD_NW;
   const int tid = threadIdx.x, lane = tid & 63;
   const int wave = __builtin_amdgcn_readfirstlane(tid >> 6);
@@ -173,6 +226,25 @@
       const int j = j0 + 16 * wave + 4 * (lane >> 4) + r, c = 16 * n + (lane & 15);
       if (j < a.nx && c < a.N) a.out[(size_t)j * a.ldo + c] = acc[n][r];
     }
-}
-
-}
+  if constexpr (ADAM) {
+    static_assert(OD_JT == FAST_ROWS, "a row tile of the product is one unit of the optimizer");
+    if (!ta->on) return;
+    const int lane = (int)__builtin_amdgcn_mbcnt_hi(~0u, __builtin_amdgcn_mbcnt_lo(~0u, 0u)), tid = 64 * wave + lane;
+    float* tile = reinterpret_cast<float*>(od_lds);
+    float (*cs)[128] = reinterpret_cast<float (*)[128]>(od_lds + OD_ADAM_CS);
+    float* gd = reinterpret_cast<float*>(od_lds + OD_ADAM_GD);
+    float2* red = reinterpret_cast<float2*>(od_lds + OD_ADAM_RED);
+#pragma unroll
+    for (int n = 0; n < 6; ++n)
+#pragma unroll
+      for (int r = 0; r < 4; ++r) {
+        const int jl = 16 * wave + 4 * (lane >> 4) + r, c = 16 * n + (lane & 15);
+        if (c < a.N) tile[jl * a.N + c] = acc[n][r];
+      }
+    constexpr int PT = (FAST_ROWS * 96 / 4 + OD_NT - 1) / OD_NT;
+    wn_fast_tile_flat<OD_NT, PT, true, true, XU8>(ta->f, blk, ta->params, nullptr, tile, ta->m, ta->v, ta->mg, ta->vg, ta->s, ta->h, gd, cs,
+                                             tile, ta->t_out, tid, [&] { od_gdot_in_tile<OD_NW, 8>(a, red, gd, vw, wave, lane); });
+  }
+}
+
+}
diff --git a/classifying-vae-lstm_amd/csrc/tail_launch.hip b/classifying-vae-lstm_amd/csrc/tail_launch.hip
--- a/classifying-vae-lstm_amd/csrc/tail_launch.hip
+++ b/classifying-vae-lstm_amd/csrc/tail_launch.hip
@@ -14,18 +14,26 @@
   reduce_launch_block<true>(t, m, sr, blockIdx.x - n_outer, reinterpret_cast<float*>(tl_lds));
 }
 
+template <bool XU8>
+__global__ __launch_bounds__(64 * TL_NW, XU8 ? 4 : 3) void tail_launch_adam_kernel(ReduceTable t, MeanTerms m, SkinnyRider sr,
+                                                                     OuterBf16Args a, unsigned n_outer, int vw, TailAdam ta) {
+  extern __shared__ __attribute__((aligned(16))) char tl_lds[];
+  if (blockIdx.x < n_outer) { dense_outer_block<TL_NW, XU8, true>(a, tl_lds, (int)blockIdx.x, vw, &ta); return; }
+  reduce_launch_block<true>(t, m, sr, blockIdx.x - n_outer, reinterpret_cast<float*>(tl_lds));
+}
+
 }
 
 extern "C" int clv_splitk_reduce_multi_outer_supported(int Bn, int nx, int N, int ldx, int ldg) {
   return clv_dense_outer_bf16_supported(Bn, nx, N, ldx, ldg);
 }
 
-extern "C" int clv_splitk_reduce_multi_outer(const clv_reduce_job* jobs, int njobs, const float* const* x, const int* n,
-                                             const int* stride, int n_terms, float* means_out,
-                                             const clv_skinny_product* riders, int n_riders,
-                                             int Bn, int nx, int N, const void* X, int x_u8, int ldx, const float* G, int ldg,
-                                             float* out, int ldo, float* colsum, const float* Hact, int ldh, const float* hbias,
-                                             float* gdot, void* stream) {
+static int tail_launch(const clv_reduce_job* jobs, int njobs, const float* const* x, const int* n,
+                       const int* stride, int n_terms, float* means_out,
+                       const clv_skinny_product* riders, int n_riders,
+                       int Bn, int nx, int N, const void* X, int x_u8, int ldx, const float* G, int ldg,
+                       float* out, int ldo, float* colsum, const float* Hact, int ldh, const float* hbias,
+                       float* gdot, const clv_tail_adam* ad, void* stream) {
   using namespace clv;
   ReduceTable t;
   MeanTerms m;
@@ -42,6 +50,20 @@
     a = OuterBf16Args{Bn, nx, N, ldx, ldg, ldo, X, G, out, colsum, Hact, hbias, gdot, ldh};
     n_outer = (unsigned)((nx + 16 * TL_NW - 1) / (16 * TL_NW)) + ((colsum || gdot) ? 1u : 0u);
   }
+  TailAdam ta{};
+  if (ad) {
+    if (!product || !clv_splitk_reduce_multi_outer_adam_supported(ad->host_table, ad->n_tensors, ad->tensor, ad->weightnorm,
+                                                                  ad->known_sums, Bn, nx, N, ldx, ldg))
+      return CLV_EINVAL;
+    if (!ad->params || !ad->grads || !ad->m || !ad->v || !ad->mg || !ad->vg || !ad->s || !gdot) return CLV_EINVAL;
+    const clv_param_desc& pd = ad->host_table[ad->tensor];
+    if (out != ad->grads + pd.offset || ldo != N || od_own_launch_waves(nx) > OD_ADAM_MAX_VW) return CLV_EINVAL;
+    ta.on = 1;
+    if (int e = adam_fast_layout(ad->host_table, ad->n_tensors, ad->tensor, gdot, ad->vnorm2, ad->ws, ad->ws_bytes, &ta.f, &ta.t_out))
+      return e;
+    ta.params = ad->params; ta.m = ad->m; ta.v = ad->v; ta.mg = ad->mg; ta.vg = ad->vg; ta.s = ad->s;
+    ta.h = AdamHyper{ad->lr, ad->beta1, ad->beta2, ad->eps, CLV_OPT_ADAM_WN, ad->step_t, ad->iterations_dev};
+  }
   if (blocks + n_outer == 0) return CLV_OK;
   hipStream_t s = (hipStream_t)stream;
   const int lds = product ? OD_LDS : SR_LDS_FLOATS * 4 + reduce_pad_lds();
@@ -51,5 +73,44 @@
     hipLaunchKernelGGL(kern, dim3(n_outer + blocks), dim3(64 * TL_NW), lds, s, t, m, sr, a, n_outer, od_own_launch_waves(nx));
     return launch_status();
   };
+  if (ad) {
+    auto go_adam = [&](auto kern) -> int {
+      if (int e = allow_dynamic_lds(reinterpret_cast<const void*>(kern), OD_LDS)) return e;
+      hipLaunchKernelGGL(kern, dim3(n_outer + blocks), dim3(64 * TL_NW), lds, s, t, m, sr, a, n_outer, od_own_launch_waves(nx), ta);
+      return launch_status();
+    };
+    return x_u8 ? go_adam(tail_launch_adam_kernel<true>) : go_adam(tail_launch_adam_kernel<false>);
+  }
   return x_u8 ? go(tail_launch_kernel<true>) : go(tail_launch_kernel<false>);
 }
+
+extern "C" int clv_splitk_reduce_multi_outer(const clv_reduce_job* jobs, int njobs, const float* const* x, const int* n,
+                                             const int* stride, int n_terms, float* means_out,
+                                             const clv_skinny_product* riders, int n_riders,
+                                             int Bn, int nx, int N, const void* X, int x_u8, int ldx, const float* G, int ldg,
+                                             float* out, int ldo, float* colsum, const float* Hact, int ldh, const float* hbias,
+                                             float* gdot, void* stream) {
+  return tail_launch(jobs, njobs, x, n, stride, n_terms, means_out, riders, n_riders, Bn, nx, N, X, x_u8, ldx, G, ldg, out, ldo,
+                     colsum, Hact, ldh, hbias, gdot, nullptr, stream);
+}
+
+extern "C" int clv_splitk_reduce_multi_outer_adam_supported(const clv_param_desc* host_table, int n_tensors, int tensor,
+                                                            int weightnorm, int known_sums, int Bn, int nx, int N, int ldx,
+                                                            int ldg) {
+  if (!clv_adam_in_tail_supported(host_table, n_tensors, tensor, weightnorm, known_sums)) return 0;
+  if (!clv_dense_outer_bf16_supported(Bn, nx, N, ldx, ldg)) return 0;
+  const clv_param_desc& pd = host_table[tensor];
+  static_assert(16 * clv::TL_NW == clv::FAST_ROWS, "a 4-wave row tile is one unit");
+  return pd.rows == nx && pd.cols == N;
+}
+
+extern "C" int clv_splitk_reduce_multi_outer_adam(const clv_reduce_job* jobs, int njobs, const float* const* x, const int* n,
+                                                  const int* stride, int n_terms, float* means_out,
+                                                  const clv_skinny_product* riders, int n_riders,
+                                                  int Bn, int nx, int N, const void* X, int x_u8, int ldx, const float* G, int ldg,
+                                                  float* out, int ldo, float* colsum, const float* Hact, int ldh, const float* hbias,
+                                                  float* gdot, const clv_tail_adam* adam, void* stream) {
+  if (!adam) return CLV_EINVAL;
+  return tail_launch(jobs, njobs, x, n, stride, n_terms, means_out, riders, n_riders, Bn, nx, N, X, x_u8, ldx, G, ldg, out, ldo,
+                     colsum, Hact, ldh, hbias, gdot, adam, stream);
+}
diff --git a/classifying-vae-lstm_amd/engine.py b/classifying-vae-lstm_amd/engine.py
--- a/classifying-vae-lstm_amd/engine.py
+++ b/classifying-vae-lstm_amd/engine.py
@@ -59,6 +59,7 @@
     'frames_u8':      ('CLV_FRAMES_U8',        True,  "the large-batch step widens its byte batch to float (rounds 4-5) instead of reading bytes"),
     'front_fused':    ('CLV_FRONT_FUSED',      True,  "the frame projections as a launch of their own behind the label launch instead of workgroups of it (csrc/label_head.hip: vrnn_front_kernel)"),
     'tail_launch':    ('CLV_TAIL_LAUNCH',      True,  "the hW kernel gradient as a launch of its own in front of grads_tail() instead of workgroups of the reduction launch that ends it (csrc/tail_launch.hip)"),
+    'adam_in_tail':   ('CLV_ADAM_IN_TAIL',     False, "the hW kernel's Adam update as the epilogue of the tail launch's workgroups that form its gradient, then one closing launch, instead of two optimizer launches behind the tail launch (off until its A/B has run: PERFLOG \"Adam in the tail launch\")"),
     'fine_grid':      ('CLV_FINE_GRID',        False, "twice the workgroups, half the rows each, for the LSTM kernel gradients (what tune_dp_schedule may pick next to an all-reduce)"),
     'fuse_notes':     ('CLV_FUSE_NOTES',       False, "input projections gathered inside the pair forward from note lists (+48 us on MI355X: profiles/r03_notes_fusion_ab.txt)"),
 }
@@ -363,6 +364,10 @@
         self.tail_launch = sw('tail_launch')
         self.halves_adjacent = False
         self._hw_outer = None
+        self.adam_in_tail = sw('adam_in_tail')
+        self.tail_adam = None
+        self._hw_adam = None
+        self.adam_in_tail_done = False
         self.fuse_notes = sw('fuse_notes') and self.fuse_pair and self.sparse_inputs and D == ops.NOTE_NONE
         self.notes_valid = False
         if self.fuse_notes:
@@ -701,7 +706,9 @@
         inv_bt, inv_b = 1.0 / BT, 1.0 / B
         g, ws, off = ops.gemm, self.ws, self.off
         adjacent, self.halves_adjacent = bool(do_tail or self.halves_adjacent), False
-        self._hw_outer = None
+        tail_adam, self.tail_adam = self.tail_adam, None
+        self._hw_outer = self._hw_adam = None
+        self.adam_in_tail_done = False
         self._train_pass = bool(need_grads)
         try:
             self.forward(X, Xp, eps_W, eps_Z, w_true, nll=(inv_bt, need_grads), target=target, noise=noise, frames8=frames8)
@@ -754,6 +761,11 @@
                     and ops.reduce_outer_supported(B, T * D, D, T * D, D)):
                 self._hw_outer = dict(Bn=B, nx=T * D, N=D, X=frames, ldx=T * D, G=self.dhW, ldg=D, out=P.g('hW/kernel'),
                                       colsum=P.g('hW/bias'), gdot=gdot)
+                if self.adam_in_tail and tail_adam is not None and need_grads:
+                    ad = P.tail_adam(self.gdot, **tail_adam)
+                    if (ad is not None and P.tall_tensor()[1] == 'hW/kernel'
+                            and ops.reduce_outer_adam_supported(ad, B, T * D, D, T * D, D)):
+                        self._hw_adam = ad
             else:
                 outer(B, T * D, D, frames, T * D, self.dhW, D, P.g('hW/kernel'), colsum=P.g('hW/bias'), gdot=gdot)
             self.gdot_fresh = True
@@ -801,6 +813,8 @@
                 ops.gemm_grouped_tn_small2(wprobs('encoder_h', D), self.dzsum_enc, wprobs('decoder_h', off + L),
                                            self.dzsum_dec, 4 * H, B)
         if rq is not None:
-            rq.flush(means=getattr(self, '_loss_terms', None), out=self.scal, skinny=skinny, outer=self._hw_outer)
+            rq.flush(means=getattr(self, '_loss_terms', None), out=self.scal, skinny=skinny, outer=self._hw_outer,
+                     adam=self._hw_adam)
             self._loss_terms = None
-            self._hw_outer = None
+            self.adam_in_tail_done = self._hw_adam is not None
+            self._hw_outer = self._hw_adam = None
diff --git a/classifying-vae-lstm_amd/ops.py b/classifying-vae-lstm_amd/ops.py
--- a/classifying-vae-lstm_amd/ops.py
+++ b/classifying-vae-lstm_amd/ops.py
@@ -53,7 +53,9 @@
         self.n += 1
         return a
 
-    def flush(self, means=None, out=None, skinny=None, outer=None):
+    def flush(self, means=None, out=None, skinny=None, outer=None, adam=None):
+        if adam is not None and outer is None:
+            raise _lib.ClvError("ReduceQueue.flush: adam= needs the product it updates (outer=)")
         if means or skinny or self.n or outer is not None:
             means = means or []
             k = len(means)
@@ -73,14 +75,23 @@
                 o = outer
                 h, ldh, hb, go = o['gdot'] if o.get('gdot') is not None else (None, 0, None, None)
                 ldo = o['ldo'] if o.get('ldo') is not None else o['N']
-                check(_lib.lib().clv_splitk_reduce_multi_outer(
-                    *args, o['Bn'], o['nx'], o['N'], _ptr(o['X']), _is_u8(o['X']), o['ldx'], _ptr(o['G']), o['ldg'], _ptr(o['out']),
-                    ldo, _ptr(o.get('colsum')), _ptr(h), int(ldh), _ptr(hb), _ptr(go), _stream()), "clv_splitk_reduce_multi_outer")
+                oargs = (o['Bn'], o['nx'], o['N'], _ptr(o['X']), _is_u8(o['X']), o['ldx'], _ptr(o['G']), o['ldg'], _ptr(o['out']),
+                         ldo, _ptr(o.get('colsum')), _ptr(h), int(ldh), _ptr(hb), _ptr(go))
+                if adam is None:
+                    check(_lib.lib().clv_splitk_reduce_multi_outer(*args, *oargs, _stream()), "clv_splitk_reduce_multi_outer")
+                else:
+                    check(_lib.lib().clv_splitk_reduce_multi_outer_adam(*args, *oargs, C.byref(adam), _stream()),
+                          "clv_splitk_reduce_multi_outer_adam")
         self.n = 0
 
 
 def reduce_outer_supported(Bn, nx, N, ldx, ldg):
     return bool(_lib.lib().clv_splitk_reduce_multi_outer_supported(Bn, nx, N, ldx, ldg))
+
+
+def reduce_outer_adam_supported(adam, Bn, nx, N, ldx, ldg):
+    return bool(_lib.lib().clv_splitk_reduce_multi_outer_adam_supported(adam.host_table, adam.n_tensors, adam.tensor, adam.weightnorm,
+                                                                        adam.known_sums, Bn, nx, N, ldx, ldg))
 
 
 def gemm(A, B, C_out, M, N, K, ta=False, tb=False, lda=None, ldb=None, ldc=None, alpha=1.0, beta=0.0,
diff --git a/classifying-vae-lstm_amd/params.py b/classifying-vae-lstm_amd/params.py
--- a/classifying-vae-lstm_amd/params.py
+++ b/classifying-vae-lstm_amd/params.py
@@ -4,6 +4,13 @@
 import torch
 
 from . import _lib, ops
+
+
+class TailAdam(C.Structure):
+    _fields_ = [("host_table", C.c_void_p), ("n_tensors", C.c_int), ("tensor", C.c_int), ("weightnorm", C.c_int), ("known_sums", C.c_int),
+                ("params", C.c_void_p), ("grads", C.c_void_p), ("m", C.c_void_p), ("v", C.c_void_p), ("mg", C.c_void_p), ("vg", C.c_void_p), ("s", C.c_void_p), ("vnorm2", C.c_void_p),
+                ("iterations_dev", C.c_void_p), ("step_t", C.c_int), ("lr", C.c_float), ("beta1", C.c_float), ("beta2", C.c_float), ("eps", C.c_float),
+                ("ws", C.c_void_p), ("ws_bytes", C.c_size_t)]
 
 
 def fuse_heads(shapes, pairs):
@@ -124,6 +131,27 @@
         tall = [(i, name) for i, (name, shp) in enumerate(self.shapes) if len(shp) > 1 and int(np.prod(shp[:-1])) > 144]
         return tall[0] if len(tall) == 1 else None
 
+    def tail_adam(self, gdot, lr=1e-3, b1=0.9, b2=0.999, eps=1e-8, weightnorm=True, advance=True, advanced=False):
+        tall = self.tall_tensor()
+        if tall is None or int(weightnorm) != 1 or gdot is None or not self.norms_valid:
+            return None
+        if not _lib.lib().clv_adam_in_tail_supported(self.table, len(self.shapes), tall[0], 1, 1):
+            return None
+        p = ops._ptr
+        return TailAdam(C.cast(self.table, C.c_void_p), len(self.shapes), tall[0], 1, 1, p(self.params), p(self.grads),
+                             p(self.m), p(self.v), p(self.mg), p(self.vg), p(self.s), p(self.vn2), p(self.iterations),
+                             -2 if advanced else (0 if advance else -1), lr, b1, b2, eps, p(self.adam_ws), self.adam_ws.numel())
+
+    def adam_close(self, gdot, lr=1e-3, b1=0.9, b2=0.999, eps=1e-8, advance=True, advanced=False):
+        tall = self.tall_tensor()
+        known = _lib.AdamKnownSums(tall[0], 1, ops._ptr(gdot), ops._ptr(self.vn2))
+        _lib.check(_lib.lib().clv_adam_wn_close(
+            self.table, len(self.shapes), ops._ptr(self.plan), ops._ptr(self.params), ops._ptr(self.grads),
+            ops._ptr(self.m), ops._ptr(self.v), ops._ptr(self.mg), ops._ptr(self.vg), ops._ptr(self.s),
+            ops._ptr(self.iterations), -2 if advanced else (0 if advance else -1), lr, b1, b2, eps,
+            C.byref(known), ops._ptr(self.adam_ws), self.adam_ws.numel(), ops._stream()), "clv_adam_wn_close")
+        self.norms_valid = True
+
     def adam_step(self, lr=1e-3, b1=0.9, b2=0.999, eps=1e-8, weightnorm=True, only=None, advance=True, advanced=False,
                   gdot=None):
         table, n, plan = (self.table, len(self.shapes), self.plan) if only is None else self._subplan(only)
diff --git a/classifying-vae-lstm_amd/trainer.py b/classifying-vae-lstm_amd/trainer.py
--- a/classifying-vae-lstm_amd/trainer.py
+++ b/classifying-vae-lstm_amd/trainer.py
@@ -197,6 +197,8 @@
         if self.is_vrnn:
             if hasattr(self.eng, 'halves_adjacent'):
                 self.eng.halves_adjacent = self.ar is None
+            if hasattr(self.eng, 'tail_adam'):
+                self.eng.tail_adam = self._adam_args() if (self.ar is None and self.fast_adam and self.weightnorm == 1) else None
             self.eng.loss_and_grads(self.X, self.Xp, self.w_true, self.eps_w, self.eps_z, do_tail=False, target=self.Y,
                                     noise=self.noise_spec(), frames8=self._f8)
             return
@@ -209,7 +211,15 @@
 
     def _update(self):
         eng = self.eng
+        if getattr(eng, 'adam_in_tail_done', False):
+            eng.adam_in_tail_done = False
+            eng.gdot_fresh = False
+            eng.P.adam_close(eng.gdot, **self._adam_args())
+            return
         eng.P.adam_step(lr=self.lr, b2=self.b2, weightnorm=self.weightnorm, advanced=self._folded(), gdot=self._gdot())
+
+    def _adam_args(self):
+        return dict(lr=self.lr, b2=self.b2, advanced=self._folded())
 
     def _gdot(self):
         eng = self.eng
diff --git a/include/clvae.h b/include/clvae.h
--- a/include/clvae.h
+++ b/include/clvae.h
@@ -431,6 +431,31 @@
                         int32_t* iterations_dev, int step_t, float lr, float beta1, float beta2, float eps,
                         int weightnorm, const clv_adam_known_sums* known, void* ws, size_t ws_bytes, void* stream);
 
+typedef struct clv_tail_adam {
+  const clv_param_desc* host_table; int n_tensors;
+  int tensor;
+  int weightnorm;
+  int known_sums;
+  float* params; const float* grads; float* m; float* v; float* mg; float* vg; const float* s;
+  float* vnorm2;
+  const int32_t* iterations_dev; int step_t;
+  float lr, beta1, beta2, eps;
+  void* ws; size_t ws_bytes;
+} clv_tail_adam;
+int clv_adam_in_tail_supported(const clv_param_desc* host_table, int n_tensors, int tensor, int weightnorm, int known_sums);
+int clv_splitk_reduce_multi_outer_adam_supported(const clv_param_desc* host_table, int n_tensors, int tensor, int weightnorm,
+                                                 int known_sums, int Bn, int nx, int N, int ldx, int ldg);
+int clv_splitk_reduce_multi_outer_adam(const clv_reduce_job* jobs, int njobs, const float* const* x, const int* n,
+                                       const int* stride, int n_terms, float* means_out,
+                                       const clv_skinny_product* riders, int n_riders,
+                                       int Bn, int nx, int N, const void* X, int x_u8, int ldx, const float* G, int ldg,
+                                       float* out, int ldo, float* colsum, const float* Hact, int ldh, const float* hbias,
+                                       float* gdot, const clv_tail_adam* adam, void* stream);
+int clv_adam_wn_close(const clv_param_desc* host_table, int n_tensors, const void* plan_dev,
+                      float* params, const float* grads, float* m, float* v, float* mg, float* vg, float* s,
+                      int32_t* iterations_dev, int step_t, float lr, float beta1, float beta2, float eps,
+                      const clv_adam_known_sums* known, void* ws, size_t ws_bytes, void* stream);
+
 int clv_philox_normal(float* out, int64_t n, uint64_t seed, uint32_t step, const int32_t* step_dev,
                       uint32_t stream_id, uint64_t first_index, void* stream);
 int clv_philox_uniform(float* out, int64_t n, uint64_t seed, uint32_t step, const int32_t* step_dev,
```
